# kaegi/adaptive-sph

Hardware: AMD Instinct MI355X
Metric: particle-steps/sec (whole node), 2D dam-break N=1M DFSPH; 1/2/4/8 GPUs (higher is better)
Workload: dtype f32; 1 GPU; dam_break_1m: 2D dam-break, 1024x1024 = 1 048 576 uniform-h particles, HybridDFSPH; particles=1048576, solver=HybridDFSPH, parallelism=single GPU

## Files before the change

adaptive_sph_amd/csrc/sph_api.hip:

```cpp
#include <hip/hip_runtime.h>

#include <algorithm>
#include <chrono>
#include <cmath>
#include <cstdarg>
#include <cstdio>
#include <cstdlib>
#include <cstring>
#include <string>
#include <vector>

#include "sph_context.hpp"
#include "sph_lambda.hpp"

int Profiler::find(const char* name)
{
    for (size_t i = 0; i < recs.size(); i++)
        if (recs[i].name == name) return (int)i;
    recs.push_back(Rec{name, 0, 0, {}});
    return (int)recs.size() - 1;
}
bool Profiler::wants(const char* name) const
{
    return mode == 1 || mode == 3 || mode == 4 || (mode == 2 && (step_index & 7u) == 0u && strncmp(name, "density", 7) == 0);
// ... 43 lines not shown
}
void Profiler::end(hipStream_t s)
{
    if (--depth > 0) return;
    if (ext_open) {
        if (ext_slot >= 0) pending.push_back(Pending{cur, nullptr, nullptr, ext_slot});
        ext_open = false;
        cur = -1;
        return;
    }
    if (kev_open) {
        kev_open = false;
        if (kev_taken) pending.push_back(Pending{cur, cur_a, cur_b, -1});
        else pool.push_back(cur_a);
        cur = -1;
        return;
    }
    hipEvent_t b = get_event();
    (void)hipEventRecord(b, s);
    pending.push_back(Pending{cur, cur_a, b, -1});
    cur = -1;
}
void Profiler::collect()
{
    std::vector<unsigned long long> ts;
    if (ts_next) {
        ts.resize(2 * (size_t)ts_next);
        (void)hipMemcpy(ts.data(), ts_dev, (size_t)ts_next * sizeof(unsigned long long), hipMemcpyDeviceToHost);
        (void)hipMemcpy(ts.data() + ts_next, ts_dev + TS_RING, (size_t)ts_next * sizeof(unsigned long long), hipMemcpyDeviceToHost);
        (void)hipMemset(ts_dev, 0xff, (size_t)ts_next * sizeof(unsigned long long));
        (void)hipMemset(ts_dev + TS_RING, 0, (size_t)ts_next * sizeof(unsigned long long));
    }
    static FILE* dump = getenv("SPH_TS_DUMP") ? fopen(getenv("SPH_TS_DUMP"), "w") : nullptr;
    std::vector<Pending> later;
    for (auto& p : pending) {
        if (p.slot >= 0) {
            const unsigned long long t0 = ts[(size_t)p.slot], t1 = ts[(size_t)ts_next + (size_t)p.slot];
            if (dump) fprintf(dump, "%s %llu %llu\n", recs[p.rec].name.c_str(), t0, t1);
            if (t1 >= t0 && t0 != ~0ull) {
                const float ms = (float)((double)(t1 - t0) * 1e-5);
                recs[p.rec].launches++;
                recs[p.rec].total_ms += ms;
                recs[p.rec].samples.push_back(ms);
            }
            continue;
        }
        float ms = 0.f;
        const hipError_t e = hipEventElapsedTime(&ms, p.a, p.b);
        if (e == hipErrorNotReady) {
            later.push_back(p);
            continue;
        }
        if (e == hipSuccess) {
            recs[p.rec].launches++;
            recs[p.rec].total_ms += ms;
            recs[p.rec].samples.push_back(ms);
        }
        pool.push_back(p.a);
        pool.push_back(p.b);
    }
    pending.swap(later);
    ts_next = 0;
    if (dump) fflush(dump);
}
void Profiler::reset()
{
    collect();
    recs.clear();
}
Profiler::~Profiler()
{
    for (auto& p : pending) {
        if (p.a) (void)hipEventDestroy(p.a);
        if (p.b) (void)hipEventDestroy(p.b);
    }
    for (auto e : pool) (void)hipEventDestroy(e);
    if (ts_dev) (void)hipFree(ts_dev);
}

#define HDR_BLOCKS 256

__global__ __launch_bounds__(256) void k_header(float4* __restrict__ pm, const float2* __restrict__ vel, uint32_t n, float rest_density,
                                                 int from_mass, float* __restrict__ h2_next, HeaderOut* __restrict__ partials,
                                                 const uint8_t* __restrict__ owned)
{
    const float INF = __uint_as_float(0x7f800000u);
    float mnx = INF, mny = INF, mxx = -INF, mxy = -INF, hmx = 0.f, hmn = INF, cfl = INF;
    for (uint32_t i = blockIdx.x * 256 + threadIdx.x; i < n; i += gridDim.x * 256) {
        if (owned && !owned[i]) continue;
        float4 p = pm[i];
        if (from_mass == 1) {
            p.w = h_from_mass(p.z, rest_density);
            pm[i] = p;
        } else if (from_mass == 2) {
            const float t = p.w;
            p.w = h2_next[i];
            h2_next[i] = t;
            pm[i] = p;
        }
        float2 v = vel[i];
        mnx = fminf(mnx, p.x); mxx = fmaxf(mxx, p.x);
        mny = fminf(mny, p.y); mxy = fmaxf(mxy, p.y);
        hmx = fmaxf(hmx, p.w); hmn = fminf(hmn, p.w);
        float sr = p.w * 2.f;
        float c = sr * sr / ((v.x * v.x + v.y * v.y) + 0.01f);
        cfl = c < cfl ? c : cfl;
    }
    mnx = wave_min(mnx); mny = wave_min(mny); mxx = wave_max(mxx); mxy = wave_max(mxy);
    hmx = wave_max(hmx); hmn = wave_min(hmn); cfl = wave_min(cfl);
    __shared__ HeaderOut s[4];
    const int lane = threadIdx.x & 63, w = threadIdx.x >> 6;
    if (lane == 0) s[w] = HeaderOut{mnx, mny, mxx, mxy, hmx, hmn, cfl, 0};
    __syncthreads();
    if (threadIdx.x == 0) {
        HeaderOut o = s[0];
        for (int k = 1; k < 4; k++) {
            o.min_x = fminf(o.min_x, s[k].min_x); o.min_y = fminf(o.min_y, s[k].min_y);
            o.max_x = fmaxf(o.max_x, s[k].max_x); o.max_y = fmaxf(o.max_y, s[k].max_y);
            o.h_max = fmaxf(o.h_max, s[k].h_max); o.h_min = fminf(o.h_min, s[k].h_min);
            o.min_cfl = fminf(o.min_cfl, s[k].min_cfl);
        }
        partials[blockIdx.x] = o;
    }
}

__global__ __launch_bounds__(256) void k_header_final(const HeaderOut* __restrict__ partials, int nparts, HeaderOut* __restrict__ out, uint32_t seq)
{
    const float INF = __uint_as_float(0x7f800000u);
    HeaderOut o{INF, INF, -INF, -INF, 0.f, INF, INF, 0};
    if ((int)threadIdx.x < nparts) o = partials[threadIdx.x];
    o.min_x = wave_min(o.min_x); o.min_y = wave_min(o.min_y); o.max_x = wave_max(o.max_x); o.max_y = wave_max(o.max_y);
    o.h_max = wave_max(o.h_max); o.h_min = wave_min(o.h_min); o.min_cfl = wave_min(o.min_cfl);
    __shared__ HeaderOut s[4];
    const int lane = threadIdx.x & 63, w = threadIdx.x >> 6;
    if (lane == 0) s[w] = o;
    __syncthreads();
    if (threadIdx.x == 0) {
        HeaderOut r = s[0];
        for (int k = 1; k < 4; k++) {
            r.min_x = fminf(r.min_x, s[k].min_x); r.min_y = fminf(r.min_y, s[k].min_y);
            r.max_x = fmaxf(r.max_x, s[k].max_x); r.max_y = fmaxf(r.max_y, s[k].max_y);
            r.h_max = fmaxf(r.h_max, s[k].h_max); r.h_min = fminf(r.h_min, s[k].h_min);
            r.min_cfl = fminf(r.min_cfl, s[k].min_cfl);
        }
        r.pad = seq - 1u;
        *out = r;
        if (seq) {
            __threadfence_system();
            ((volatile HeaderOut*)out)->pad = seq;
        }
    }
}

__global__ __launch_bounds__(1024) void k_header_ahead(const HeaderOut* __restrict__ partials, uint32_t nparts, const SolverCtrl* __restrict__ ctrl,
                                                       HeaderOut* __restrict__ out, const DeviceStatus* __restrict__ status, SolverCtrl* __restrict__ h_ctrl,
                                                       DeviceStatus* __restrict__ h_status, uint32_t seq)
{
    if (ctrl->done == 0u) {
        if (h_ctrl && threadIdx.x == 0) {
            SolverCtrl v = *ctrl;
            v.seq = seq - 1u;
            *h_ctrl = v;
            *h_status = *status;
            __threadfence_system();
            ((volatile SolverCtrl*)h_ctrl)->seq = seq;
        }
        return;
    }
    const float INF = __uint_as_float(0x7f800000u);
    HeaderOut o{INF, INF, -INF, -INF, 0.f, INF, INF, 0};
    for (uint32_t k0 = threadIdx.x; k0 < nparts; k0 += 4096u) {
        HeaderOut q[4];
#pragma unroll
        for (uint32_t u = 0; u < 4u; u++) q[u] = partials[min(k0 + 1024u * u, nparts - 1u)];
#pragma unroll
        for (uint32_t u = 0; u < 4u; u++) {
            o.min_x = fminf(o.min_x, q[u].min_x); o.min_y = fminf(o.min_y, q[u].min_y);
            o.max_x = fmaxf(o.max_x, q[u].max_x); o.max_y = fmaxf(o.max_y, q[u].max_y);
            o.h_max = fmaxf(o.h_max, q[u].h_max); o.h_min = fminf(o.h_min, q[u].h_min);
            o.min_cfl = fminf(o.min_cfl, q[u].min_cfl);
        }
    }
    o.min_x = wave_min(o.min_x); o.min_y = wave_min(o.min_y); o.max_x = wave_max(o.max_x); o.max_y = wave_max(o.max_y);
    o.h_max = wave_max(o.h_max); o.h_min = wave_min(o.h_min); o.min_cfl = wave_min(o.min_cfl);
    __shared__ HeaderOut s[16];
    const int lane = threadIdx.x & 63, w = threadIdx.x >> 6;
    if (lane == 0) s[w] = o;
    __syncthreads();
    if (threadIdx.x == 0) {
        HeaderOut r = s[0];
        for (int k = 1; k < 16; k++) {
            r.min_x = fminf(r.min_x, s[k].min_x); r.min_y = fminf(r.min_y, s[k].min_y);
            r.max_x = fmaxf(r.max_x, s[k].max_x); r.max_y = fmaxf(r.max_y, s[k].max_y);
            r.h_max = fmaxf(r.h_max, s[k].h_max); r.h_min = fminf(r.h_min, s[k].h_min);
            r.min_cfl = fminf(r.min_cfl, s[k].min_cfl);
        }
        *out = r;
        if (h_ctrl) {
            SolverCtrl v = *ctrl;
            v.seq = seq - 1u;
            *h_ctrl = v;
            *h_status = *status;
            __threadfence_system();
            ((volatile SolverCtrl*)h_ctrl)->seq = seq;
        }
    }
}

__global__ __launch_bounds__(256) void k_pack_upload(uint32_t n, const float* __restrict__ mass, const float2* __restrict__ pos,
                                                      const float2* __restrict__ velin, float4* __restrict__ pm, float2* __restrict__ vel,
                                                      uint32_t* __restrict__ orig, float* __restrict__ lvl, float* __restrict__ lvlold,
                                                      float* __restrict__ h2_next)
{
    uint32_t i = blockIdx.x * 256 + threadIdx.x;
    if (i >= n) return;
    float2 p = pos[i];
    pm[i] = make_float4(p.x, p.y, mass[i], 0.f);
    h2_next[i] = h_from_mass(mass[i], 1.f);
    vel[i] = velin[i];
    orig[i] = i;
    lvl[i] = __uint_as_float(0x7fc00000u);
    lvlold[i] = 0.f;
}

__global__ void k_publish(const SolverCtrl* __restrict__ ctrl, const DeviceStatus* __restrict__ status, SolverCtrl* __restrict__ h_ctrl,
                          DeviceStatus* __restrict__ h_status, uint32_t seq)
{
    if (threadIdx.x == 0 && blockIdx.x == 0) {
        SolverCtrl v = *ctrl;
        v.seq = seq - 1u;
        *h_ctrl = v;
        *h_status = *status;
        __threadfence_system();
        ((volatile SolverCtrl*)h_ctrl)->seq = seq;
    }
}

enum { G_F32 = 0, G_F32X2 = 1, G_PM_X = 2, G_PM_M = 3, G_PM_H = 4, G_U32 = 5, G_H2NEXT = 6, G_U8 = 7, G_F32X4_ZW = 8 };

__global__ __launch_bounds__(256) void k_to_host_order(uint32_t n, int kind, const uint32_t* __restrict__ orig, const void* __restrict__ src,
                                                        void* __restrict__ dst)
{
    uint32_t i = blockIdx.x * 256 + threadIdx.x;
    if (i >= n) return;
    uint32_t o = orig ? orig[i] : i;
    switch (kind) {
    case G_F32: ((float*)dst)[o] = ((const float*)src)[i]; break;
    case G_U32: ((uint32_t*)dst)[o] = ((const uint32_t*)src)[i]; break;
    case G_U8: ((uint8_t*)dst)[o] = ((const uint8_t*)src)[i]; break;
    case G_F32X2: ((float2*)dst)[o] = ((const float2*)src)[i]; break;
    case G_PM_X: { float4 p = ((const float4*)src)[i]; ((float2*)dst)[o] = make_float2(p.x, p.y); } break;
    case G_F32X4_ZW: { float4 p = ((const float4*)src)[i]; ((float2*)dst)[o] = make_float2(p.z, p.w); } break;
    case G_PM_M: ((float*)dst)[o] = ((const float4*)src)[i].z; break;
    case G_PM_H: ((float*)dst)[o] = ((const float4*)src)[i].w; break;
    case G_H2NEXT: ((float*)dst)[o] = h_from_mass(((const float4*)src)[i].z, 1.f); break;
    }
}

__global__ __launch_bounds__(256) void k_from_host_order(uint32_t n, int kind, const uint32_t* __restrict__ orig, const void* __restrict__ src,
                                                          void* __restrict__ dst)
{
    uint32_t i = blockIdx.x * 256 + threadIdx.x;
    if (i >= n) return;
    uint32_t o = orig ? orig[i] : i;
    switch (kind) {
    case G_F32: ((float*)dst)[i] = ((const float*)src)[o]; break;
    case G_U32: ((uint32_t*)dst)[i] = ((const uint32_t*)src)[o]; break;
    case G_F32X2: ((float2*)dst)[i] = ((const float2*)src)[o]; break;
    case G_U8: ((uint8_t*)dst)[i] = ((const uint8_t*)src)[o]; break;
    case G_PM_X: { float2 p = ((const float2*)src)[o]; float4 q = ((float4*)dst)[i]; q.x = p.x; q.y = p.y; ((float4*)dst)[i] = q; } break;
    case G_PM_M: { float4 q = ((float4*)dst)[i]; q.z = ((const float*)src)[o]; ((float4*)dst)[i] = q; } break;
    case G_PM_H: { float4 q = ((float4*)dst)[i]; q.w = ((const float*)src)[o]; ((float4*)dst)[i] = q; } break;
    default: break;
    }
}

__global__ __launch_bounds__(256) void k_rows_to_slots(uint32_t n, int kind, const uint32_t* __restrict__ slot, const void* __restrict__ src, void* __restrict__ dst)
{
    const uint32_t r = blockIdx.x * 256 + threadIdx.x;
    if (r >= n) return;
    const uint32_t i = slot[r];
    switch (kind) {
    case G_F32: ((float*)dst)[i] = ((const float*)src)[r]; break;
    case G_U32: ((uint32_t*)dst)[i] = ((const uint32_t*)src)[r]; break;
    case G_F32X2: ((float2*)dst)[i] = ((const float2*)src)[r]; break;
    case G_U8: ((uint8_t*)dst)[i] = ((const uint8_t*)src)[r]; break;
    case G_PM_X: { float2 p = ((const float2*)src)[r]; float4 q = ((float4*)dst)[i]; q.x = p.x; q.y = p.y; ((float4*)dst)[i] = q; } break;
    case G_PM_M: { float4 q = ((float4*)dst)[i]; q.z = ((const float*)src)[r]; ((float4*)dst)[i] = q; } break;
    case G_PM_H: { float4 q = ((float4*)dst)[i]; q.w = ((const float*)src)[r]; ((float4*)dst)[i] = q; } break;
    default: break;
    }
}

__global__ __launch_bounds__(256) void k_cell_index_host(uint32_t n, GridP g, const uint32_t* __restrict__ orig, const float4* __restrict__ pm,
                                                          uint32_t* __restrict__ dst)
{
    uint32_t i = blockIdx.x * 256 + threadIdx.x;
    if (i >= n) return;
    float4 p = pm[i];
    int cx = (int)floorf(p.x / g.cs) - g.minx, cy = (int)floorf(p.y / g.cs) - g.miny;
    dst[orig[i]] = (uint32_t)cx + (uint32_t)cy * (uint32_t)g.sx;
}

__global__ __launch_bounds__(256) void k_ext_counts(uint32_t n, const uint4* __restrict__ nl_ext, const uint32_t* __restrict__ orig, uint32_t* __restrict__ dst)
{
    uint32_t i = blockIdx.x * 256 + threadIdx.x;
    if (i < n) dst[orig[i]] = nl_ext[i].w & 0xffffu;
}

__global__ __launch_bounds__(256) void k_fill_neighbors(uint32_t n, GridP g, TileP t, const uint32_t* __restrict__ cell_start,
                                                         const uint32_t* __restrict__ cxy, const uint32_t* __restrict__ orig,
                                                         const float4* __restrict__ pm, const uint32_t* __restrict__ offsets_host,
                                                         uint32_t* __restrict__ indices, float k, const uint32_t* __restrict__ rowmap)
{
    uint32_t i = blockIdx.x * 256 + threadIdx.x;
    if (i >= n) return;
    const uint32_t row = rowmap ? rowmap[i] : orig[i];
    if (row == 0xffffffffu) return;
    const float4 Ai = pm[i];
    const uint32_t c = cxy[i];
    const int cx = c & 0xffffu, cy = c >> 16;
    uint32_t w = offsets_host[row];
    const int R = stencil_radius(g, t, Ai.w, cx, cy, k);
    for (int dy = -R; dy <= R; dy++) {
        int yy = cy + dy;
        if (yy < 0 || yy >= g.sy) continue;
        uint32_t b = cell_start[(uint32_t)yy * g.sx + max(cx - R, 0)];
        uint32_t e = cell_start[(uint32_t)yy * g.sx + min(cx + R + 1, g.sx)];
        for (uint32_t j = b; j < e; j++) {
            const float4 Aj = pm[j];
            const float dx = Ai.x - Aj.x, dyy = Ai.y - Aj.y;
            const float r2 = dx * dx + dyy * dyy;
            const float s = ((Ai.w + Aj.w) * 0.5f) * k;
            if (r2 < s * s) indices[w++] = orig[j];
        }
    }
}

__global__ __launch_bounds__(256) void k_check_neighborhood(uint32_t n, const float4* __restrict__ pm, const uint32_t* __restrict__ ncount,
                                                             const uint32_t* __restrict__ orig, DeviceStatus* status, const uint8_t* __restrict__ owned)
{
    uint32_t i = blockIdx.x * 256 + threadIdx.x;
    if (i >= n) return;
    if (owned && !owned[i]) return;
    const float4 Ai = pm[i];
    uint32_t cnt = 0;
    for (uint32_t j = 0; j < n; j++) {
        const float4 Aj = pm[j];
        const float dx = Ai.x - Aj.x, dy = Ai.y - Aj.y;
        const float s = ((Ai.w + Aj.w) * 0.5f) * 2.f;
        cnt += (dx * dx + dy * dy < s * s) ? 1u : 0u;
    }
    if (cnt != ncount[i] && atomicCAS(&status->error, 0u, (uint32_t)SPH_ERR_CHECK_NEIGHBORHOOD) == 0u) status->info = orig[i];
}

static int alloc_particle_buffers(sph_ctx* c)
{
    const size_t n = c->cap ? c->cap : 1;
    for (int k = 0; k < 2; k++) {
        HIPCHK(c, c->pm[k].ensure(n * sizeof(float4)));
        HIPCHK(c, c->vel[k].ensure(n * sizeof(float2)));
        HIPCHK(c, c->orig[k].ensure(n * sizeof(uint32_t)));
        HIPCHK(c, c->lvl[k].ensure(n * sizeof(float)));
        HIPCHK(c, c->lvlold[k].ensure(n * sizeof(float)));
        HIPCHK(c, c->h2n[k].ensure(n * sizeof(float)));
        HIPCHK(c, c->szc[k].ensure(n));
        HIPCHK(c, c->key[k].ensure(n * sizeof(uint32_t)));
        HIPCHK(c, c->val[k].ensure(n * sizeof(uint32_t)));
    }
    HIPCHK(c, c->vel_tmp.ensure(n * sizeof(float2)));
    HIPCHK(c, c->sort_scratch.ensure(radix_sort_scratch_elems((uint32_t)n) * sizeof(uint32_t)));
    HIPCHK(c, c->cxy.ensure(n * sizeof(uint32_t)));
    DevBuf* f1[] = {&c->rho, &c->lam_sum, &c->constf, &c->aii, &c->src, &c->p0, &c->p1, &c->dens_err, &c->stat, &c->ncount,
                    &c->mrho, &c->pt0, &c->pt1};
    for (auto b : f1) HIPCHK(c, b->ensure(n * sizeof(float)));
    HIPCHK(c, c->lam_grad.ensure(n * sizeof(float2)));
    if (c->exact) {
        HIPCHK(c, c->wall_pl.ensure(n * sizeof(float2) * SPH_MAX_PLANES));
        HIPCHK(c, c->wall_cnt.ensure(n));
    }
    HIPCHK(c, c->lam_prev.ensure(n * sizeof(float)));
    HIPCHK(c, c->omega.ensure(n * sizeof(float)));
    HIPCHK(c, c->pacc.ensure(n * sizeof(float4)));
    HIPCHK(c, c->prec0.ensure(n * sizeof(float4)));
    HIPCHK(c, c->prec1.ensure(n * sizeof(float4)));
    HIPCHK(c, c->xv.ensure(n * sizeof(float4)));
    HIPCHK(c, c->scratch.ensure(n * sizeof(float4)));
    HIPCHK(c, c->nl.ensure(sweep_list_bytes((uint32_t)n)));
    HIPCHK(c, c->nl_ok.ensure(n));
    HIPCHK(c, c->red_partials.ensure(sizeof(SolverPartial) * (size_t)solver_reduce_blocks((uint32_t)n)));
    HIPCHK(c, c->hdr_ahead_partials.ensure(sizeof(HeaderOut) * (((size_t)n + 255) / 256)));
    return SPH_OK;
}

Options options_from_env()
{
    Options o;
    auto num = [](const char* name, int dflt) {
        const char* e = getenv(name);
        return e && e[0] ? atoi(e) : dflt;
    };
    auto flag = [](const char* name) { return getenv(name) != nullptr ? 1 : 0; };
    o.exact = num("SPH_HIP_EXACT", 0) == 1 ? 1 : 0;
    o.overlap = num("SPH_OVERLAP", -1);
    o.loopback_sync = num("SPH_LOOPBACK_SYNC", 0) != 0 ? 1 : 0;
    o.force_slab_mode = flag("SPH_FORCE_SLAB_MODE");
    o.event_wait = flag("SPH_EVENT_WAIT");
    o.debug_sync = num("SPH_DEBUG_SYNC", 0);
    o.debug_counts = flag("SPH_DEBUG_COUNTS");
    o.comm_delay_us = num("SPH_DEBUG_COMM_DELAY_US", 0);
    o.hip_trace = num("SPH_HIP_TRACE", 0) == 1 ? 1 : 0;
#ifdef SPH_LAB
    o.paced = num("SPH_PACED", 1) != 0 ? 1 : 0;
    o.pace_lead = num("SPH_PACE_LEAD", 0);
    o.pace_pred = num("SPH_PACE_PRED", 0xffff);
    o.chain = num("SPH_CHAIN", -1);
    o.accel_generic = flag("SPH_ACCEL_GENERIC");
    o.jacobi_generic = flag("SPH_JACOBI_GENERIC");
    o.source_generic = flag("SPH_SOURCE_GENERIC");
    o.slab_general = flag("SPH_SLAB_GENERAL");
    o.slab_level_plain = flag("SPH_SLAB_LEVEL_PLAIN");
    o.level_serial = flag("SPH_LEVEL_SERIAL");
    o.level_batch8 = flag("SPH_LEVEL_BATCH8");
    o.level_queue = num("SPH_LEVEL_QUEUE", 1) != 0 ? 1 : 0;
    o.offset_lists = num("SPH_OFFSET_LISTS", 1) != 0 ? 1 : 0;
    o.no_fuse = flag("SPH_NO_FUSE");
    o.side_stream_normal = flag("SPH_SIDE_STREAM_NORMAL");
    o.tile = num("SPH_TILE", 0);
    o.ahead_build = num("SPH_AHEAD_BUILD", 1) != 0 ? 1 : 0;
    o.inc_sort = num("SPH_INC_SORT", 1);
    o.slab_paced = num("SPH_SLAB_PACED", 1) != 0 ? 1 : 0;
    o.slab_records = num("SPH_SLAB_RECORDS", 1) != 0 ? 1 : 0;
    o.side_cus = num("SPH_SIDE_CUS", 0);
    o.main_exclude = num("SPH_MAIN_EXCLUDE", 0) != 0 ? 1 : 0;
    o.ipc_fuse_max_bytes = std::max(num("SPH_IPC_FUSE_MAX_BYTES", 64 << 10), 0);
    o.ipc_copy_min_bytes = std::max(num("SPH_IPC_COPY_MIN_BYTES", 256 << 10), 0);
    o.search_block = std::min(std::max(num("SPH_SEARCH_BLOCK", 1024) / 64 * 64, 64), 1024);
#else
    static const char* const lab_only[] = {"SPH_PACED", "SPH_PACE_LEAD", "SPH_PACE_PRED", "SPH_CHAIN", "SPH_ACCEL_GENERIC", "SPH_JACOBI_GENERIC", "SPH_SOURCE_GENERIC",
                                           "SPH_SLAB_GENERAL", "SPH_SLAB_LEVEL_PLAIN", "SPH_LEVEL_SERIAL", "SPH_LEVEL_BATCH8", "SPH_LEVEL_QUEUE", "SPH_OFFSET_LISTS",
                                           "SPH_NO_FUSE", "SPH_SIDE_STREAM_NORMAL", "SPH_TILE", "SPH_AHEAD_BUILD", "SPH_INC_SORT", "SPH_SLAB_PACED", "SPH_SLAB_RECORDS",
                                           "SPH_SIDE_CUS", "SPH_MAIN_EXCLUDE", "SPH_IPC_FUSE_MAX_BYTES", "SPH_IPC_COPY_MIN_BYTES"};
    static bool warned = false;
    if (!warned)
        for (const char* name : lab_only)
            if (getenv(name)) {
                fprintf(stderr, "libsph_hip: %s is a laboratory switch and is IGNORED by the product library (use SPH_HIP_LIBRARY=libsph_lab.so, scripts/README.md)\n", name);
                warned = true;
            }
#endif
    return o;
}

extern "C" int sph_create(uint64_t n_capacity, int device_id, const sph_plane* planes, int n_planes, sph_ctx** out)
{
    if (!out || n_planes < 0 || n_planes > SPH_MAX_PLANES || (n_planes > 0 && !planes)) return SPH_ERR_INVALID_ARGUMENT;
    if (n_capacity >= (1ull << 31)) return SPH_ERR_CAPACITY;
    int ndev = 0;
    if (hipGetDeviceCount(&ndev) != hipSuccess || ndev <= 0 || device_id < 0 || device_id >= ndev) return SPH_ERR_DEVICE;
    if (hipSetDevice(device_id) != hipSuccess) return SPH_ERR_DEVICE;
    sph_ctx* c = new sph_ctx();
    c->device = device_id;
    c->cap = n_capacity;
    c->n_planes = n_planes;
    for (int k = 0; k < n_planes; k++) c->bnd_h.planes[k] = PlaneP{planes[k].dir_x, planes[k].dir_y, planes[k].delta};
    c->opt = options_from_env();
    c->exact = c->opt.exact;
    auto bail = [&](int code) {
        sph_destroy(c);
        return code;
    };
    uint32_t side_mask[8] = {0, 0, 0, 0, 0, 0, 0, 0}, main_mask[8];
    for (int b = 0; b < 8 * c->opt.side_cus && b < 256; b++) side_mask[b >> 5] |= 1u << (b & 31);
    for (int w = 0; w < 8; w++) main_mask[w] = ~side_mask[w];
    if (c->opt.side_cus > 0 && c->opt.main_exclude) {
        if (hipExtStreamCreateWithCUMask(&c->stream, 8, main_mask) != hipSuccess) return bail(SPH_ERR_DEVICE);
    } else if (hipStreamCreateWithFlags(&c->stream, hipStreamNonBlocking) != hipSuccess) return bail(SPH_ERR_DEVICE);
    if (c->opt.side_cus > 0) {
        if (hipExtStreamCreateWithCUMask(&c->stream2, 8, side_mask) != hipSuccess) return bail(SPH_ERR_DEVICE);
    } else
    {
        int lo = 0, hi = 0;
        (void)hipDeviceGetStreamPriorityRange(&lo, &hi);
        if (c->opt.side_stream_normal || hipStreamCreateWithPriority(&c->stream2, hipStreamNonBlocking, hi) != hipSuccess)
            if (hipStreamCreateWithFlags(&c->stream2, hipStreamNonBlocking) != hipSuccess) return bail(SPH_ERR_DEVICE);
    }
    if (hipEventCreateWithFlags(&c->ev_fork, hipEventDisableTiming) != hipSuccess) return bail(SPH_ERR_DEVICE);
    for (auto& e : c->ev)
        if (hipEventCreate(&e) != hipSuccess) return bail(SPH_ERR_DEVICE);
    if (alloc_particle_buffers(c) != SPH_OK) return bail(SPH_ERR_DEVICE);
    bool ok = c->planes_d.ensure(sizeof(BoundaryP)) == hipSuccess && c->lam_lut.ensure(10001 * 4) == hipSuccess &&
              c->dlam_lut.ensure(10001 * 4) == hipSuccess && c->hdr_partials.ensure(sizeof(HeaderOut) * HDR_BLOCKS) == hipSuccess &&
              c->hdr_out.ensure(sizeof(HeaderOut)) == hipSuccess && c->ctrl.ensure(3 * sizeof(SolverCtrl)) == hipSuccess &&
              c->status.ensure(sizeof(DeviceStatus)) == hipSuccess && c->n_tiles.ensure(16) == hipSuccess;
    if (!ok) return bail(SPH_ERR_DEVICE);
    if (hipHostMalloc((void**)&c->hdr_host, sizeof(HeaderOut), hipHostMallocMapped) != hipSuccess) return bail(SPH_ERR_DEVICE);
    if (hipHostMalloc((void**)&c->ctrl_host, 3 * sizeof(SolverCtrl), hipHostMallocMapped) != hipSuccess) return bail(SPH_ERR_DEVICE);
    if (hipHostMalloc((void**)&c->status_host, sizeof(DeviceStatus), hipHostMallocMapped) != hipSuccess) return bail(SPH_ERR_DEVICE);
    if (hipHostMalloc((void**)&c->lvl_changed, 64 * sizeof(uint32_t), hipHostMallocMapped) != hipSuccess) return bail(SPH_ERR_DEVICE);
    if (hipHostGetDevicePointer((void**)&c->lvl_changed_dev, c->lvl_changed, 0) != hipSuccess) return bail(SPH_ERR_DEVICE);
    memset(c->lvl_changed, 0, 64 * sizeof(uint32_t));
    if (hipHostGetDevicePointer((void**)&c->hdr_host_dev, c->hdr_host, 0) != hipSuccess) return bail(SPH_ERR_DEVICE);
    if (hipHostGetDevicePointer((void**)&c->ctrl_host_dev, c->ctrl_host, 0) != hipSuccess) return bail(SPH_ERR_DEVICE);
    if (hipHostGetDevicePointer((void**)&c->status_host_dev, c->status_host, 0) != hipSuccess) return bail(SPH_ERR_DEVICE);
    if (hipEventCreateWithFlags(&c->ev_sync, hipEventDisableTiming) != hipSuccess) return bail(SPH_ERR_DEVICE);
    memset(c->status_host, 0, sizeof(DeviceStatus));
    memset((void*)c->ctrl_host, 0, 3 * sizeof(SolverCtrl));
    c->prog_host = (volatile uint32_t*)(c->ctrl_host + 2);
    c->prog_host_dev = (uint32_t*)(c->ctrl_host_dev + 2);
    c->movers_host = c->prog_host + 1;
    std::vector<float> lam, dlam;
    sph_lambda::build_luts(lam, dlam);
    if (hipMemcpy(c->lam_lut.p, lam.data(), lam.size() * 4, hipMemcpyHostToDevice) != hipSuccess ||
        hipMemcpy(c->dlam_lut.p, dlam.data(), dlam.size() * 4, hipMemcpyHostToDevice) != hipSuccess ||
        hipMemcpy(c->planes_d.p, &c->bnd_h, sizeof(BoundaryP), hipMemcpyHostToDevice) != hipSuccess ||
        hipMemset(c->status.p, 0, sizeof(DeviceStatus)) != hipSuccess || hipMemset(c->ctrl.p, 0, sizeof(SolverCtrl)) != hipSuccess ||
        hipDeviceSynchronize() != hipSuccess)
        return bail(SPH_ERR_DEVICE);
    *out = c;
    return SPH_OK;
}

extern "C" int sph_set_boundary_polygon(sph_ctx* c, const float* pts, int n)
{
    if (!c || !pts || n < 3 || n > SPH_MAX_POLYGON_POINTS) return SPH_ERR_INVALID_ARGUMENT;
    HIPCHK(c, hipSetDevice(c->device));
    BoundaryP b = c->bnd_h;
    for (int i = 0; i < n; i++) {
        b.px[i] = pts[2 * i];
        b.py[i] = pts[2 * i + 1];
    }
    for (int i = 0; i < n; i++) {
        const int i1 = (i + 1) % n;
        const float dx = b.px[i1] - b.px[i], dy = b.py[i1] - b.py[i];
        const float n2 = dx * dx + dy * dy;
        if (!(n2 > 0.00001f)) return c->fail(SPH_ERR_INVALID_ARGUMENT, "assertion failed: line_dir.norm_squared() > 0.00001");
        const float nn = sqrtf(n2);
        b.dx[i] = dx / nn;
        b.dy[i] = dy / nn;
    }
    for (int i = 0; i < n; i++) {
        const int pi = i == 0 ? n - 1 : i - 1;
        const float px = -b.dy[pi] + -b.dy[i], py = b.dx[pi] + b.dx[i];
        if (!(px * px + py * py > 0.00001f)) return c->fail(SPH_ERR_INVALID_ARGUMENT, "assertion failed: pseudo_normal.norm_squared() > 0.00001");
        b.nx[i] = px;
        b.ny[i] = py;
    }
    b.poly_n = n;
    c->bnd_h = b;
    c->n_planes = 1;
    HIPCHK(c, hipStreamSynchronize(c->stream));
    HIPCHK(c, hipMemcpy(c->planes_d.p, &c->bnd_h, sizeof(BoundaryP), hipMemcpyHostToDevice));
    return SPH_OK;
}

extern "C" void sph_destroy(sph_ctx* c)
{
    if (!c) return;
    (void)hipSetDevice(c->device);
    if (c->stream) (void)hipStreamSynchronize(c->stream);
    if (c->stream2) (void)hipStreamSynchronize(c->stream2);
    dist_release(c);
    DevBuf* all[] = {&c->pm[0], &c->pm[1], &c->vel[0], &c->vel[1], &c->orig[0], &c->orig[1], &c->lvl[0], &c->lvl[1], &c->lvlold[0],
                     &c->lvlold[1], &c->vel_tmp, &c->key[0], &c->key[1], &c->val[0], &c->val[1], &c->sort_scratch, &c->cxy, &c->cell_start,
                     &c->cs_scratch, &c->hdr_ahead_partials, &c->h2n[0], &c->h2n[1], &c->lam_prev, &c->nl, &c->nlx, &c->tile_raw, &c->tile_h, &c->tile_h_ext, &c->lvl_changed_d, &c->lvl_tmp, &c->lvl_nrm, &c->lvl_state, &c->lvl_when, &c->lvl_mark, &c->lvl_queue, &c->nloff, &c->nlh, &c->flag_surface,
                     &c->flag_insufficient, &c->con_thr, &c->con_consumed, &c->con_h, &c->flag_reduced, &c->szc[0], &c->szc[1], &c->omega, &c->stash, &c->nl_ext, &c->nlx_ext, &c->nl_ok, &c->mrho, &c->pt0, &c->pt1, &c->prec0, &c->prec1, &c->xv, &c->rho, &c->lam_sum, &c->lam_grad, &c->wall_pl, &c->wall_cnt, &c->constf, &c->aii, &c->src, &c->p0, &c->p1, &c->pacc, &c->dens_err,
                     &c->stat, &c->ncount, &c->planes_d, &c->lam_lut, &c->dlam_lut, &c->hdr_partials, &c->hdr_out, &c->ctrl, &c->status,
                     &c->n_tiles, &c->red_partials, &c->scratch, &c->split_patterns, &c->akey[0], &c->akey[1], &c->aval[0], &c->aval[1], &c->acxy, &c->acell_start, &c->pm2,
                     &c->atile_raw, &c->atile_h, &c->inc_head, &c->inc_next, &c->inc_bsum, &c->inc_movers, &c->cand_red, &c->rnd_rec, &c->rnd_keys, &c->rnd_out, &c->rnd_max, &c->rnd_prev, &c->rnd_layer, &c->rnd_band, &c->rnd_words, &c->rnd_stage};
    for (auto b : all) b->release();
    for (DevBuf* b : c->export_bufs()) b->release();
    for (DevBuf* b : c->prob_bufs()) b->release();
    for (DevBuf* b : c->slab_bufs()) b->release();
    if (c->hdr_host) (void)hipHostFree(c->hdr_host);
    if (c->ctrl_host) (void)hipHostFree(c->ctrl_host);
    if (c->status_host) (void)hipHostFree(c->status_host);
    if (c->lvl_changed) (void)hipHostFree(c->lvl_changed);
    for (auto& e : c->ev)
        if (e) (void)hipEventDestroy(e);
    if (c->ev_sync) (void)hipEventDestroy(c->ev_sync);
    if (c->stream) (void)hipStreamDestroy(c->stream);
    if (c->stream2) (void)hipStreamDestroy(c->stream2);
    if (c->ev_fork) (void)hipEventDestroy(c->ev_fork);
    delete c;
}

extern "C" const char* sph_last_error(const sph_ctx* c) { return c ? c->err.c_str() : "null context"; }
extern "C" uint64_t sph_num_particles(const sph_ctx* c) { return c ? c->n : 0; }
extern "C" float sph_time(const sph_ctx* c) { return c ? c->time : 0.f; }
extern "C" int sph_set_time(sph_ctx* c, float t, uint64_t step)
{
    if (!c) return SPH_ERR_INVALID_ARGUMENT;
    c->time = t;
    c->step_number = step;
    return SPH_OK;
}

extern "C" int sph_set_math_policy(sph_ctx* c, int policy)
{
    if (!c || (policy != SPH_MATH_FAST && policy != SPH_MATH_EXACT)) return SPH_ERR_INVALID_ARGUMENT;
    if (c->poisoned) return c->fail(SPH_ERR_POISONED, "sph_set_math_policy: the context is poisoned until sph_upload");
    if (policy == c->exact) return SPH_OK;
    HIPCHK(c, hipSetDevice(c->device));
    if (int rc = wait_stream(c)) return rc;
    c->exact = policy;
    if (c->exact) {
        size_t n = c->cap ? c->cap : 1;
        HIPCHK(c, c->wall_pl.ensure(n * sizeof(float2) * SPH_MAX_PLANES));
        HIPCHK(c, c->wall_cnt.ensure(n));
    }
    c->drop(DROPS_POLICY);
    return SPH_OK;
}
extern "C" int sph_get_math_policy(const sph_ctx* c) { return c ? c->exact : -1; }

extern "C" int sph_upload(sph_ctx* c, uint64_t n, const float* mass, const float* pos, const float* vel)
{
    if (!c || (n && (!mass || !pos || !vel))) return SPH_ERR_INVALID_ARGUMENT;
    if (n > c->cap) return c->fail(SPH_ERR_CAPACITY, "n=%llu exceeds capacity %llu", (unsigned long long)n, (unsigned long long)c->cap);
    HIPCHK(c, hipSetDevice(c->device));
    hipStream_t s = c->stream;
    c->n = n;
    c->cur = 0;
    c->pcur = 0;
    c->poisoned = false;
    c->dist.n_tot = (uint32_t)n;
    c->drop(DROPS_UPLOAD);
    for (DevBuf* b : c->export_bufs()) b->release();
    for (DevBuf* b : c->slab_bufs()) b->release();
    for (DevBuf* b : c->prob_bufs()) b->release();
    if (n == 0) return SPH_OK;
    HIPCHK(c, hipMemcpyAsync(c->key[1].p, mass, n * sizeof(float), hipMemcpyHostToDevice, s));
    HIPCHK(c, hipMemcpyAsync(c->scratch.p, pos, n * sizeof(float2), hipMemcpyHostToDevice, s));
    HIPCHK(c, hipMemcpyAsync(c->vel_tmp.p, vel, n * sizeof(float2), hipMemcpyHostToDevice, s));
    hipLaunchKernelGGL(k_pack_upload, dim3((n + 255) / 256), dim3(256), 0, s, (uint32_t)n, c->key[1].as<float>(), c->scratch.as<float2>(),
                       c->vel_tmp.as<float2>(), c->pm[0].as<float4>(), c->vel[0].as<float2>(), c->orig[0].as<uint32_t>(),
                       c->lvl[0].as<float>(), c->lvlold[0].as<float>(), c->h2n[0].as<float>());
    HIPCHK(c, hipMemsetAsync(c->szc[0].p, 2, n, s));
    DevBuf* zero[] = {&c->rho, &c->lam_sum, &c->constf, &c->aii, &c->src, &c->p0, &c->p1, &c->dens_err, &c->ncount};
    for (auto b : zero) HIPCHK(c, hipMemsetAsync(b->p, 0, n * sizeof(float), s));
    HIPCHK(c, hipMemsetAsync(c->lam_grad.p, 0, n * sizeof(float2), s));
    HIPCHK(c, hipMemsetAsync(c->pacc.p, 0, n * sizeof(float4), s));
    c->pressure_cur = 0;
    HIPCHK(c, hipStreamSynchronize(s));
    return SPH_OK;
}

struct FieldRef {
    int kind;
    const void* src;
    size_t elem;
    bool uploadable;
};

static bool field_ref(sph_ctx* c, int field, FieldRef* r)
{
    const int k = c->cur;
    switch (field) {
    case SPH_F_MASS: *r = {G_PM_M, c->pm[c->pcur].p, 4, true}; return true;
    case SPH_F_POSITION: *r = {G_PM_X, c->pm[c->pcur].p, 8, true}; return true;
    case SPH_F_VELOCITY: *r = {G_F32X2, c->vel[k].p, 8, true}; return true;
    case SPH_F_PRESSURE_ACCEL: *r = {G_F32X4_ZW, c->pacc.p, 8, false}; return true;
    case SPH_F_DENSITY: *r = {G_F32, c->rho.p, 4, false}; return true;
    case SPH_F_PPE_SOURCE_TERM: *r = {G_F32, c->src.p, 4, false}; return true;
    case SPH_F_PRESSURE: *r = {G_F32, c->pressure_cur ? c->p1.p : c->p0.p, 4, false}; return true;
    case SPH_F_AII: *r = {G_F32, c->aii.p, 4, false}; return true;
    case SPH_F_DENSITY_ERROR: *r = {G_F32, c->dens_err.p, 4, false}; return true;
    case SPH_F_H2: *r = {G_PM_H, c->pm[c->pcur].p, 4, true}; return true;
    case SPH_F_H2_NEXT: *r = {G_F32, c->h2n[k].p, 4, true}; return true;
    case SPH_F_CONSTANT_FIELD: *r = {G_F32, c->constf.p, 4, false}; return true;
    case SPH_F_NEIGHBOR_COUNT: *r = {G_U32, c->ncount.p, 4, false}; return true;
    case SPH_F_LEVEL_ESTIMATION: *r = {G_F32, c->lvl[k].p, 4, true}; return true;
    case SPH_F_LEVEL_OLD: *r = {G_F32, c->lvlold[k].p, 4, true}; return true;
    case SPH_F_PARTICLE_SIZE_CLASS: *r = {G_U8, c->szc[k].p, 1, true}; return true;
    case SPH_F_LAMBDA_SUM: *r = {G_F32, c->lam_sum.p, 4, false}; return true;
    case SPH_F_LAMBDA_GRAD_SUM: *r = {G_F32X2, c->lam_grad.p, 8, false}; return true;
    default: return false;
    }
}

static int download_slab(sph_ctx* c, int kind, const void* src, size_t elem, void* dst, uint64_t bytes)
{
    hipStream_t s = c->stream;
    const uint32_t nt = c->have_flags ? c->dist.n_tot : (uint32_t)c->n;
    if (bytes != (uint64_t)c->n * elem) return c->fail(SPH_ERR_INVALID_ARGUMENT, "size mismatch (slab holds %llu particles)", (unsigned long long)c->n);
    if (nt == 0) return SPH_OK;
    std::vector<uint8_t> raw((size_t)nt * elem), flags(nt, 1);
    hipLaunchKernelGGL(k_to_host_order, dim3((nt + 255) / 256), dim3(256), 0, s, nt, kind, (const uint32_t*)nullptr, src, c->scratch.p);
    HIPCHK(c, hipMemcpyAsync(raw.data(), c->scratch.p, raw.size(), hipMemcpyDeviceToHost, s));
    if (c->have_flags) HIPCHK(c, hipMemcpyAsync(flags.data(), c->dist.owned.p, nt, hipMemcpyDeviceToHost, s));
    HIPCHK(c, hipStreamSynchronize(s));
    size_t w = 0;
    for (uint32_t i = 0; i < nt; i++)
        if (flags[i]) {
            if (w >= c->n) return c->fail(SPH_ERR_DEVICE, "owned-particle count mismatch");
            memcpy((uint8_t*)dst + w * elem, raw.data() + (size_t)i * elem, elem);
            w++;
        }
    return SPH_OK;
}

extern "C" int sph_download(sph_ctx* c, int field, void* dst, uint64_t bytes)
{
    if (!c || !dst) return SPH_ERR_INVALID_ARGUMENT;
    HIPCHK(c, hipSetDevice(c->device));
    hipStream_t s = c->stream;
    const uint32_t n = (uint32_t)c->n;
    const int k = c->cur;
    if (field == SPH_F_PARTICLE_ID) {
        if (c->dist.on) return download_slab(c, G_U32, c->orig[k].p, 4, dst, bytes);
        if (bytes != (uint64_t)n * 4) return c->fail(SPH_ERR_INVALID_ARGUMENT, "field %d: size mismatch", field);
        for (uint32_t i = 0; i < n; i++) ((uint32_t*)dst)[i] = i;
        return SPH_OK;
    }
    if (field == SPH_F_CELL_INDEX) {
        if (!c->grid_valid) return c->fail(SPH_ERR_INVALID_ARGUMENT, "no grid yet: run a step first");
        if (c->dist.on) return download_slab(c, G_U32, c->key[0].p, 4, dst, bytes);
        if (bytes != (uint64_t)n * 4) return c->fail(SPH_ERR_INVALID_ARGUMENT, "field %d: size mismatch", field);
        if (n == 0) return SPH_OK;
        const bool same_grid = c->fgrid.minx == c->grid.minx && c->fgrid.miny == c->grid.miny && c->fgrid.sx == c->grid.sx && c->fgrid.sy == c->grid.sy;
        if (c->uniform_h && same_grid) {
            hipLaunchKernelGGL(k_to_host_order, dim3((n + 255) / 256), dim3(256), 0, s, n, (int)G_U32, c->orig[k].as<uint32_t>(),
// ... 597 lines not shown
    if (!ext)
        hipLaunchKernelGGL(k_fill_neighbors, dim3((n + 255) / 256), dim3(256), 0, s, n, c->fgrid,
                           TileP{c->tile_ts, c->tile_tsx, c->tile_tsy, c->tile_h.as<uint32_t>(), 0.f}, c->cell_start.as<uint32_t>(), c->cxy.as<uint32_t>(),
                           c->orig[c->cur].as<uint32_t>(), c->pm[c->pcur ^ 1].as<float4>(), d_off.as<uint32_t>(), d_idx.as<uint32_t>(), 2.f, (const uint32_t*)nullptr);
    else
        hipLaunchKernelGGL(k_fill_neighbors, dim3((n + 255) / 256), dim3(256), 0, s, n, c->fgrid,
                           TileP{c->tile_ts, c->tile_tsx, c->tile_tsy, c->tile_h_ext.as<uint32_t>(), c->lists_after_slack}, c->cell_start.as<uint32_t>(),
                           c->cxy.as<uint32_t>(), c->orig[c->cur].as<uint32_t>(), c->pm[c->pcur].as<float4>(), d_off.as<uint32_t>(), d_idx.as<uint32_t>(),
                           c->lists_after_k, (const uint32_t*)nullptr);
    HIPCHK(c, hipMemcpyAsync(indices, d_idx.p, (size_t)tot * 4, hipMemcpyDeviceToHost, s));
    HIPCHK(c, hipStreamSynchronize(s));
    c->export_built();
    c->export_tot = tot;
    return SPH_OK;
}

int export_lists_on_device(sph_ctx* c)
{
    const uint32_t n = (uint32_t)c->n;
    hipStream_t s = c->stream;
    DevBuf &d_off = c->export_d_off, &d_idx = c->export_d_idx;
    c->drop(CARRY_EXPORT);
    HIPCHK(c, d_off.ensure(((size_t)n + 1) * 4));
    HIPCHK(c, c->scratch.ensure((size_t)n * 4 + 4));
    HIPCHK(c, c->cand_scan.ensure(((size_t)n / 2048 + 4) * 4));
    const bool ext = c->lists_after;
    const dim3 grid((n + 255) / 256), blk(256);
    if (n) {
        if (!ext) hipLaunchKernelGGL(k_to_host_order, grid, blk, 0, s, n, (int)G_U32, c->orig[c->cur].as<uint32_t>(), (const void*)c->ncount.p, c->scratch.p);
        else hipLaunchKernelGGL(k_ext_counts, grid, blk, 0, s, n, c->nl_ext.as<uint4>(), c->orig[c->cur].as<uint32_t>(), c->scratch.as<uint32_t>());
    }
    device_exclusive_scan_u32(s, c->scratch.as<uint32_t>(), d_off.as<uint32_t>(), n, c->cand_scan.as<uint32_t>(), d_off.as<uint32_t>() + n);
    uint32_t tot = 0;
    HIPCHK(c, hipMemcpyAsync(&tot, d_off.as<uint32_t>() + n, 4, hipMemcpyDeviceToHost, s));
    HIPCHK(c, hipStreamSynchronize(s));
    HIPCHK(c, d_idx.ensure((size_t)tot * 4));
    if (n && tot) {
        if (!ext)
            hipLaunchKernelGGL(k_fill_neighbors, grid, blk, 0, s, n, c->fgrid, TileP{c->tile_ts, c->tile_tsx, c->tile_tsy, c->tile_h.as<uint32_t>(), 0.f},
                               c->cell_start.as<uint32_t>(), c->cxy.as<uint32_t>(), c->orig[c->cur].as<uint32_t>(), c->pm[c->pcur ^ 1].as<float4>(),
                               d_off.as<uint32_t>(), d_idx.as<uint32_t>(), 2.f, (const uint32_t*)nullptr);
        else
            hipLaunchKernelGGL(k_fill_neighbors, grid, blk, 0, s, n, c->fgrid,
                               TileP{c->tile_ts, c->tile_tsx, c->tile_tsy, c->tile_h_ext.as<uint32_t>(), c->lists_after_slack}, c->cell_start.as<uint32_t>(),
                               c->cxy.as<uint32_t>(), c->orig[c->cur].as<uint32_t>(), c->pm[c->pcur].as<float4>(), d_off.as<uint32_t>(), d_idx.as<uint32_t>(),
                               c->lists_after_k, (const uint32_t*)nullptr);
    }
    c->export_built();
    c->export_tot = tot;
    return SPH_OK;
}

__global__ __launch_bounds__(256) void k_slab_owned_flags(uint32_t nt, const uint8_t* __restrict__ owned, uint32_t* __restrict__ flag, uint32_t* __restrict__ iota)
{
    const uint32_t s = blockIdx.x * 256 + threadIdx.x;
    if (s >= nt) return;
    flag[s] = owned[s] ? 1u : 0u;
    iota[s] = s;
}
__global__ __launch_bounds__(256) void k_slab_rowmap(uint32_t nt, uint32_t n_rows, const uint8_t* __restrict__ owned, uint32_t* __restrict__ pos,
                                                      const uint32_t* __restrict__ ncount, const uint4* __restrict__ nl_ext, uint32_t* __restrict__ row_slot,
                                                      uint32_t* __restrict__ cnt, unsigned long long* __restrict__ total64)
{
    const uint32_t s = blockIdx.x * 256 + threadIdx.x;
    unsigned long long c = 0;
    if (s < nt) {
        const uint32_t r = pos[s];
        if (!owned[s] || r >= n_rows) pos[s] = 0xffffffffu;
        else {
            row_slot[r] = s;
            c = nl_ext ? (nl_ext[s].w & 0xffffu) : ncount[s];
            cnt[r] = (uint32_t)c;
        }
    }
    for (int o = 32; o > 0; o >>= 1) c += __shfl_down(c, o, 64);
    if ((threadIdx.x & 63) == 0 && c) atomicAdd(total64, c);
}
int slab_lists_on_device(sph_ctx* c)
{
    const uint32_t n = (uint32_t)c->n, nt = c->dist.n_tot;
    hipStream_t s = c->stream;
    c->drop(CARRY_SLAB_LISTS);
    TmpBuf d_iota, d_cnt, d_tot64;
    HIPCHK(c, d_tot64.ensure(8));
    HIPCHK(c, hipMemsetAsync(d_tot64.p, 0, 8, s));
    DevBuf& d_map = c->slab_slot_row;
    HIPCHK(c, d_map.ensure((size_t)nt * 4 + 4));
    HIPCHK(c, d_iota.ensure((size_t)nt * 4 + 4));
    HIPCHK(c, d_cnt.ensure((size_t)n * 4 + 4));
    HIPCHK(c, c->slab_row_slot.ensure((size_t)n * 4 + 4));
    HIPCHK(c, c->slab_off.ensure(((size_t)n + 1) * 4));
    HIPCHK(c, c->scratch.ensure((size_t)nt * 4 + 4));
    HIPCHK(c, c->cand_scan.ensure(((size_t)nt / 2048 + 4) * 4));
    const bool ext = c->lists_after;
    uint32_t* off = c->slab_off.as<uint32_t>();
    uint32_t tot[2] = {0, 0};
    if (nt) {
        const dim3 grid((nt + 255) / 256), blk(256);
        hipLaunchKernelGGL(k_slab_owned_flags, grid, blk, 0, s, nt, c->dist.owned.as<uint8_t>(), c->scratch.as<uint32_t>(), d_iota.as<uint32_t>());
        device_exclusive_scan_u32(s, c->scratch.as<uint32_t>(), d_map.as<uint32_t>(), nt, c->cand_scan.as<uint32_t>(), d_map.as<uint32_t>() + nt);
        HIPCHK(c, hipMemcpyAsync(&tot[0], d_map.as<uint32_t>() + nt, 4, hipMemcpyDeviceToHost, s));
        hipLaunchKernelGGL(k_slab_rowmap, grid, blk, 0, s, nt, n, c->dist.owned.as<uint8_t>(), d_map.as<uint32_t>(), c->ncount.as<uint32_t>(),
                           ext ? c->nl_ext.as<uint4>() : (const uint4*)nullptr, c->slab_row_slot.as<uint32_t>(), d_cnt.as<uint32_t>(), d_tot64.as<unsigned long long>());
    }
    unsigned long long tot64 = 0;
    HIPCHK(c, hipMemcpyAsync(&tot64, d_tot64.p, 8, hipMemcpyDeviceToHost, s));
    device_exclusive_scan_u32(s, d_cnt.as<uint32_t>(), off, n, c->cand_scan.as<uint32_t>(), off + n);
    HIPCHK(c, hipMemcpyAsync(&tot[1], off + n, 4, hipMemcpyDeviceToHost, s));
    HIPCHK(c, hipStreamSynchronize(s));
    if (tot[0] != n) return c->fail(SPH_ERR_DEVICE, "owned-particle count mismatch");
    if (tot64 >= (1ull << 32) || tot64 != tot[1])
        return c->fail(SPH_ERR_CAPACITY, "%llu neighbour-list entries on rank %d do not fit the 32-bit CSR offsets", tot64, c->dist.rank);
    HIPCHK(c, c->slab_idx.ensure((size_t)tot[1] * 4 + 4));
    if (nt && tot[1]) {
        const dim3 grid((nt + 255) / 256), blk(256);
        if (!ext)
            hipLaunchKernelGGL(k_fill_neighbors, grid, blk, 0, s, nt, c->fgrid, TileP{c->tile_ts, c->tile_tsx, c->tile_tsy, c->tile_h.as<uint32_t>(), 0.f},
                               c->cell_start.as<uint32_t>(), c->cxy.as<uint32_t>(), (const uint32_t*)d_iota.as<uint32_t>(), c->pm[c->pcur ^ 1].as<float4>(), off,
                               c->slab_idx.as<uint32_t>(), 2.f, (const uint32_t*)d_map.as<uint32_t>());
        else
            hipLaunchKernelGGL(k_fill_neighbors, grid, blk, 0, s, nt, c->fgrid,
                               TileP{c->tile_ts, c->tile_tsx, c->tile_tsy, c->tile_h_ext.as<uint32_t>(), c->lists_after_slack}, c->cell_start.as<uint32_t>(),
                               c->cxy.as<uint32_t>(), (const uint32_t*)d_iota.as<uint32_t>(), c->pm[c->pcur].as<float4>(), off, c->slab_idx.as<uint32_t>(),
                               c->lists_after_k, (const uint32_t*)d_map.as<uint32_t>());
        HIPCHK(c, hipStreamSynchronize(s));
    }
    c->slab_lists_valid = true;
    c->slab_lists_rows = n;
    c->slab_lists_tot = tot[1];
    return SPH_OK;
}


void launch_header(sph_ctx* c, uint32_t n, float rest_density, int from_mass , HeaderOut* out_dev,
                   const uint8_t* owned)
{
    hipStream_t s = c->stream;
    ProfScope ps(&c->prof, "header", s);
    int nb = (int)((n + 255) / 256);
    if (nb > HDR_BLOCKS) nb = HDR_BLOCKS;
    if (nb < 1) nb = 1;
    hipLaunchKernelGGL(k_header, dim3(nb), dim3(256), 0, s, c->pm[c->pcur].as<float4>(), c->vel[c->cur].as<float2>(), n, rest_density, from_mass,
                       c->h2n[c->cur].as<float>(), c->hdr_partials.as<HeaderOut>(), owned);
    c->publish_seq++;
    if (c->publish_seq == 0u) c->publish_seq = 1u;
    const bool mapped = out_dev == c->hdr_host_dev;
    hipLaunchKernelGGL(k_header_final, dim3(1), dim3(256), 0, s, c->hdr_partials.as<HeaderOut>(), nb, out_dev, mapped ? c->publish_seq : 0u);
    if (mapped) {
        c->hint_word = &((volatile HeaderOut*)c->hdr_host)->pad;
        c->hint_seq = c->publish_seq;
    }
}

void launch_header_ahead(sph_ctx* c, uint32_t nblocks, HeaderOut* out_dev, bool publish)
{
    ProfScope ps(&c->prof, "header_ahead", c->stream);
    uint32_t seq = 0;
    if (publish) {
        c->publish_seq++;
        if (c->publish_seq == 0u) c->publish_seq = 1u;
        seq = c->publish_seq;
        c->publish_folded = true;
    }
    hipLaunchKernelGGL(k_header_ahead, dim3(1), dim3(1024), 0, c->stream, c->hdr_ahead_partials.as<HeaderOut>(), nblocks, c->ctrl.as<SolverCtrl>(), out_dev,
                       c->status.as<DeviceStatus>(), publish ? c->ctrl_host_dev : (SolverCtrl*)nullptr, publish ? c->status_host_dev : (DeviceStatus*)nullptr, seq);
}

void launch_publish(sph_ctx* c)
{
    if (c->publish_folded) {
        c->publish_folded = false;
        return;
    }
    c->publish_seq++;
    if (c->publish_seq == 0u) c->publish_seq = 1u;
    hipLaunchKernelGGL(k_publish, dim3(1), dim3(64), 0, c->stream, c->ctrl.as<SolverCtrl>(), c->status.as<DeviceStatus>(), c->ctrl_host_dev,
                       c->status_host_dev, c->publish_seq);
}

void launch_check_neighborhood(sph_ctx* c, const SweepArgs& a)
{
    ProfScope ps(&c->prof, "check_neighborhood", c->stream);
    hipLaunchKernelGGL(k_check_neighborhood, dim3((a.n + 255) / 256), dim3(256), 0, c->stream, a.n, a.pm, a.ncount, a.orig, a.status, a.owned);
}
```

adaptive_sph_amd/csrc/sph_context.hpp:

```cpp
#pragma once

#include <hip/hip_runtime.h>

#include <array>
#include <chrono>
#include <cstdarg>
#include <cstdio>
#include <string>
#include <vector>

#include "sph_carry.hpp"
#include "sph_internal.hpp"

struct DevBuf {
    void* p = nullptr;
    size_t bytes = 0;
    hipError_t ensure(size_t need)
    {
        if (need <= bytes) return hipSuccess;
        if (p) (void)hipFree(p);
        p = nullptr;
        bytes = 0;
        size_t grow = need + need / 4 + 256;
        hipError_t e = hipMalloc(&p, grow);
        if (e == hipSuccess) bytes = grow;
        return e;
    }
    void release()
    {
        if (p) (void)hipFree(p);
        p = nullptr;
        bytes = 0;
    }
    template <class T>
    T* as() const { return (T*)p; }
};

struct TmpBuf : DevBuf {
    TmpBuf() = default;
    TmpBuf(const TmpBuf&) = delete;
    TmpBuf& operator=(const TmpBuf&) = delete;
    ~TmpBuf() { release(); }
};

struct Options {
    int exact = 0;
    int paced = 1;
    int pace_lead = 0;
    int pace_pred = 0xffff;
    int chain = -1;
    int overlap = -1;
    int accel_generic = 0;
    int jacobi_generic = 0;
    int source_generic = 0;
    int slab_general = 0;
    int slab_level_plain = 0;
    int level_serial = 0;
    int level_batch8 = 0;
    int offset_lists = 1;
    int level_queue = 1;
    int no_fuse = 0;
    int event_wait = 0;
    int loopback_sync = 0;
    int side_stream_normal = 0;
    int force_slab_mode = 0;
    int tile = 0;
    int ahead_build = 1;
    int inc_sort = 1;
    int slab_paced = 1;
    int slab_records = 1;
    int debug_sync = 0;
    int debug_counts = 0;
    int comm_delay_us = 0;
    int hip_trace = 0;
    int side_cus = 0;
    int main_exclude = 0;
    int ipc_fuse_max_bytes = 64 << 10;
    int ipc_copy_min_bytes = 256 << 10;
    int search_block = 1024;
};
Options options_from_env();

struct sph_ctx : Carry {
    int device = 0;
    Options opt;
    uint64_t cap = 0, n = 0;
    hipStream_t stream = nullptr;
    hipStream_t stream2 = nullptr;
    hipEvent_t ev_fork = nullptr;
    uint32_t level_seq = 0;
    int n_planes = 0;
    BoundaryP bnd_h{};
    float time = 0.f;
    uint64_t step_number = 0;
    uint64_t n_waits = 0;
    bool poisoned = false;
    std::string err;
    Profiler prof;
    int exact = 0;
    std::vector<uint32_t> export_cnt, export_off;
    DevBuf export_d_off, export_d_idx;

    uint64_t export_tot = 0;
    DevBuf cand_rec, cand_cls, cand_cnt, cand_off, cand_idx, cand_scan, cand_red;
    std::array<DevBuf*, 8> export_bufs() { return {&export_d_off, &export_d_idx, &cand_rec, &cand_cls, &cand_cnt, &cand_off, &cand_idx, &cand_scan}; }
    int prob_kind = 0;
    uint32_t prob_k = 0;
    DevBuf prob_flag, prob_rank, prob_lvl, prob_ids, prob_cls, prob_mass, prob_level, prob_pos, prob_h2, prob_off, prob_idx;
    uint64_t prob_serial = 0, sol_serial = 0;
    DevBuf sol_partner, sol_counter, ps_w, ps_words, ps_state, ps_rec;
    std::array<DevBuf*, 17> prob_bufs() { return {&prob_flag, &prob_rank, &prob_lvl, &prob_ids, &prob_cls, &prob_mass, &prob_level, &prob_pos, &prob_h2, &prob_off, &prob_idx,
                                                  &sol_partner, &sol_counter, &ps_w, &ps_words, &ps_state, &ps_rec}; }
    uint32_t slab_lists_rows = 0, slab_rows_n = 0;
    uint64_t slab_lists_tot = 0, slab_rows_tot = 0;
    DevBuf slab_row_slot, slab_slot_row, slab_off, slab_idx;
    uint32_t slab_prob_k = 0, slab_prob_ko = 0;
    DevBuf slab_prob_flag, slab_prob_rank, slab_prob_ids, slab_prob_cls, slab_prob_mass, slab_prob_level, slab_prob_pos, slab_prob_h2, slab_prob_off;
    std::array<DevBuf*, 13> slab_bufs() { return {&slab_row_slot, &slab_slot_row, &slab_off, &slab_idx, &slab_prob_flag, &slab_prob_rank, &slab_prob_ids, &slab_prob_cls,
                                                  &slab_prob_mass, &slab_prob_level, &slab_prob_pos, &slab_prob_h2, &slab_prob_off}; }

    DevBuf pm[2], vel[2], orig[2], lvl[2], lvlold[2];
    int cur = 0;
    int pcur = 0;
    DevBuf vel_tmp;
    DevBuf key[2], val[2], sort_scratch, cxy, cell_start, cs_scratch, nl, nl_ok, mrho, pt0, pt1, prec0, prec1, xv;
    bool uniform_h = false;
    float h_uniform = 0.f;
    DevBuf wall_pl, wall_cnt;
    DevBuf rho, lam_sum, lam_grad, constf, aii, src, p0, p1, pacc, dens_err, stat, ncount;
    DevBuf planes_d, lam_lut, dlam_lut, hdr_partials, hdr_out, ctrl, status, n_tiles, red_partials, scratch;
    HeaderOut* hdr_host = nullptr;
    volatile uint32_t* hint_word = nullptr;
    uint32_t hint_seq = 0;
    uint32_t publish_seq = 0;
    bool publish_folded = false;
    SolverCtrl* ctrl_host = nullptr;
    DeviceStatus* status_host = nullptr;
    HeaderOut* hdr_host_dev = nullptr;
    SolverCtrl* ctrl_host_dev = nullptr;
    DeviceStatus* status_host_dev = nullptr;
    volatile uint32_t* prog_host = nullptr;
    uint32_t* prog_host_dev = nullptr;
    uint32_t solve_epoch = 0;
    bool paced_step = false;
    hipEvent_t ev_sync = nullptr;

    struct Dist {
        bool on = false;
        int rank = 0, nranks = 1;
        float cut_lo = 0.f, cut_hi = 0.f;
        uint32_t n_tot = 0;
        uint32_t n_halo[2] = {0, 0}, n_ghost[2] = {0, 0};
        float hcut[2] = {0.f, 0.f};
        float halo_w[2] = {0.f, 0.f};
        DevBuf owned;
        DevBuf cls, blk;
        int overlap_env = -1;
        bool pre = false;
        uint32_t pre_n = 0;
        uint32_t pre_cls_n = 0;
        uint32_t pre_own = 0;
        DevBuf tot_table;
        DevBuf ring1, ring1_src;
        DevBuf halo_idx, halo_pos, halo_src, ghost_dst;
        DevBuf send[2], recv[2];
        DevBuf counts;
        DevBuf solver_tot;
        uint32_t* counts_host = nullptr;
        uint32_t* counts_host_dev = nullptr;
        void* nccl = nullptr;
        DevBuf edge;
        hipStream_t xstream = nullptr;
        hipEvent_t ev_x[3] = {nullptr, nullptr, nullptr};
        hipEvent_t ev_pack = nullptr, ev_copied = nullptr, ev_tot = nullptr;
        double* gtot = nullptr;
        uint32_t gtot_seq = 0;
        bool ghosts_ok = true;
        void* tgroup = nullptr;
        void* ipc = nullptr;
        void* shm = nullptr;
        size_t shm_bytes = 0;
        std::string shm_name;
        int rebalance_every = 0;
        DevBuf hist;
        uint32_t rebalances = 0;
        uint64_t stat_exchanges = 0, stat_bytes_sent = 0, stat_bytes_recv = 0, stat_allreduces = 0, stat_step0 = 0;
    } dist;

    GridP grid{};
    GridP fgrid{};
    int tile_ts = 0, tile_tsx = 0, tile_tsy = 0;
    DevBuf tile_raw, tile_h, tile_h_ext, nlx;
    DevBuf nloff, nlh;
    DevBuf akey[2], aval[2], acxy, acell_start, pm2;
    DevBuf atile_raw, atile_h;
    DevBuf inc_head, inc_next, inc_bsum, inc_movers;
    uint32_t inc_epoch = 0;
    int inc_radix_streak = 0;
    struct Ahead {
        GridP g{};
        float h_max = 0.f, h_min = 0.f, rest_density = 0.f;
        int tile_ts = 0, tile_tsx = 0, tile_tsy = 0;
        uint64_t n = 0;
    } ahead;
    DevBuf hdr_ahead_partials;
    float hdr_ahead_rest_density = 0.f;
    DevBuf h2n[2];
    DevBuf lam_prev;
    DevBuf lvl_queue;
    DevBuf lvl_tmp, lvl_nrm, lvl_state, lvl_when, lvl_mark, flag_surface, flag_insufficient, stash, nl_ext, nlx_ext;
    DevBuf con_thr, con_consumed, con_h, flag_reduced;
    float lists_after_k = 0.f, lists_after_slack = 0.f;
    float h_max_step = 0.f;
    float last_dmax = 0.f;
    float slab_slack_w = 0.f;
    DevBuf szc[2];
    DevBuf omega;
    DevBuf split_patterns;
    uint32_t n_split_patterns = 0;
    DevBuf lvl_changed_d;
    uint32_t* lvl_changed = nullptr;
    uint32_t last_level_sweeps = 0;
    uint32_t* lvl_changed_dev = nullptr;
    uint32_t pressure_cur = 0;
    uint32_t last_div_iters = 2, last_dens_iters = 2;
    uint32_t prev_dens_iters = 0;
    uint32_t prev_div_iters = 0;
    DevBuf rnd_rec, rnd_keys, rnd_out, rnd_max, rnd_prev;
    uint64_t rnd_prev_n = 0;
    DevBuf rnd_layer, rnd_band, rnd_words, rnd_stage;
    bool rnd_have_layer = false;
    int rnd_layer_sx0 = 0, rnd_layer_sx1 = 0, rnd_layer_hs = 0;
    hipEvent_t ev[8];

    int fail(int code, const char* fmt, ...)
    {
        char buf[512];
        va_list ap;
        va_start(ap, fmt);
        vsnprintf(buf, sizeof buf, fmt, ap);
        va_end(ap);
        err = buf;
        return code;
    }
    int refuse_poisoned() { return fail(SPH_ERR_POISONED, "an earlier step failed inside the step: the particle state is undefined until sph_upload"); }
};

#define HIPCHK(ctx, call)                                                                                  \
    do {                                                                                                   \
        hipError_t e_ = (call);                                                                            \
        if (e_ != hipSuccess) return (ctx)->fail(SPH_ERR_DEVICE, "%s failed: %s", #call, hipGetErrorString(e_)); \
    } while (0)


int wait_stream(sph_ctx* c);
const char* status_message(uint32_t code);
SweepArgs make_args(sph_ctx* c, const StepP& sp);

void launch_header(sph_ctx* c, uint32_t n, float rest_density, int from_mass, HeaderOut* out_dev, const uint8_t* owned = nullptr);
void launch_publish(sph_ctx* c);
void launch_profile_calibration(sph_ctx* c);
void launch_check_neighborhood(sph_ctx* c, const SweepArgs& a);
int export_lists_on_device(sph_ctx* c);
int slab_lists_on_device(sph_ctx* c);
void dist_release(sph_ctx* c);
```

adaptive_sph_amd/csrc/sph_internal.hpp:

```cpp
#pragma once

#include <hip/hip_runtime.h>
#include <hip/hip_ext.h>
#include <stdint.h>

#include <string>
#include <vector>

#include "sph_device.h"
#include "sph_ffi.h"

struct Profiler {
    int mode = 0;
    uint64_t step_index = 0;
    struct Rec {
        std::string name;
        uint64_t launches = 0;
        double total_ms = 0;
        std::vector<float> samples;
    };
    struct Pending {
        int rec;
        hipEvent_t a, b;
        int slot;
    };
    std::vector<Rec> recs;
    std::vector<Pending> pending;
    std::vector<hipEvent_t> pool;

    int find(const char* name);
    bool wants(const char* name) const;
    hipEvent_t get_event();
    void begin(const char* name, hipStream_t s, bool single_launch = false);
    void end(hipStream_t s);
    unsigned long long* take_slot();
    bool take_events(hipEvent_t* a, hipEvent_t* b);
    enum { TS_RING = 1 << 16 };
    unsigned long long* ts_dev = nullptr;
    uint32_t ts_next = 0;
    void collect();
    void reset();
    ~Profiler();
    int cur = -1;
    int depth = 0;
    hipEvent_t cur_a = nullptr, cur_b = nullptr;
    bool ext_open = false;
    int ext_slot = -1;
    bool kev_open = false, kev_taken = false;
};

struct ProfScope {
    Profiler* p;
    hipStream_t s;
    bool on;
    ProfScope(Profiler* p_, const char* name, hipStream_t s_, bool single_launch = false)
        : p(p_), s(s_), on(p_ && p_->mode && p_->wants(name) && (p_->mode != 3 || single_launch))
    {
        if (on) p->begin(name, s, single_launch);
    }
    ~ProfScope()
    {
        if (on) p->end(s);
    }
};

struct HeaderOut {
    float min_x, min_y, max_x, max_y, h_max, h_min, min_cfl;
    uint32_t pad;
};

struct SolverCtrl {
    uint32_t done;
    uint32_t iters;
    uint32_t cur;
    uint32_t peer_error;
    uint32_t normal, singular, negative;
    float sum_err, max_err;
    uint32_t slot_done[2];
    uint32_t seq;
};

struct DeviceStatus {
    uint32_t error;
    uint32_t info;
};

struct CellKeyGen {
    const float4* pm;
    GridP g;
    const uint8_t* gone;
    uint32_t n_gone, gone_from;
    int clamp = 0;
};
int radix_sort_pairs(hipStream_t s, Profiler* prof, uint32_t* keyA, uint32_t* valA, uint32_t* keyB, uint32_t* valB,
                     uint32_t n, int bits, uint32_t* hist_scratch , const CellKeyGen* keygen = nullptr);
size_t radix_sort_scratch_elems(uint32_t n);
struct ReorderIO {
    const float4* pm_in;
    const float2* vel_in;
    const uint32_t* orig_in;
    const float *lvl_in, *lvlold_in;
    float4* pm_out;
    float2* vel_out;
    uint32_t* orig_out;
    float *lvl_out, *lvlold_out;
    uint32_t* cxy_out;
    const float* h2n_in;
    float* h2n_out;
    const float* lam_in;
    float* lam_prev_out;
    const uint8_t* szc_in;
    uint8_t* szc_out;
};
size_t incremental_sort_block_sums(uint32_t ncells);
void incremental_cell_sort_reorder(hipStream_t s, Profiler* prof, uint32_t n, const float4* pm_new, const IncClassifyP& q, bool classified,
                                   const uint32_t* cell_start_cur, uint32_t* key_out, uint32_t* cell_start_out, const ReorderIO& io, uint32_t* bsum, uint32_t* movers,
                                   uint32_t* movers_host);

void incremental_cell_sort_perm(hipStream_t s, Profiler* prof, uint32_t n, uint32_t n_prev, const CellKeyGen& kg, const IncClassifyP& q, const uint32_t* cell_start_cur,
                                uint32_t* key_out, uint32_t* perm_out, uint32_t* cell_start_out, uint32_t* bsum, uint32_t* movers, uint32_t* movers_host);

void launch_reorder(hipStream_t s, Profiler* prof, uint32_t n, GridP g, const uint32_t* sorted_key, const uint32_t* perm, const ReorderIO& io,
                    void* cell_start_scratch);
size_t cell_start_scratch_bytes();
void launch_cell_start(hipStream_t s, Profiler* prof, const uint32_t* sorted_key, uint32_t n, uint32_t ncells,
                       uint32_t* cell_start , void* scratch ,
                       bool count_zeroed = false );
void launch_tile_hmax(hipStream_t s, Profiler* prof, uint32_t n, const float4* pm, GridP g, int ts, int tsx, int tsy, uint32_t* raw,
                      uint32_t* out , uint32_t* out_ext = nullptr , int d_ext = 2);

struct SweepArgs {
    GridP g;
    StepP sp;
    uint32_t n;
    int exact;
    int uniform_h;
    float h_uniform;
    const uint32_t* cell_start;
    const uint32_t* orig;
    const float4* pm;
    float2* vel;
    float2* vel_tmp;
    float* rho;
    float* lam_sum;
    float2* lam_grad;
    float2* wall_pl = nullptr;
    uint8_t* wall_cnt = nullptr;
    float* constf;
    float* aii;
    float* src;
    float* p0;
    float* p1;
    float4* pacc;
    float* dens_err;
    float* stat;
    uint32_t* ncount;
    uint4* nl;
    uint4* nlx;
    HeaderOut* hdr_partials;
    IncClassifyP inc;
    int h_mode;
    int sp_check_aii;
    float* h2_next;
    float* omega;
    const uint8_t* size_class;
    const float* lam_prev;
    const uint2* nloff = nullptr;
    const uint8_t* nlh = nullptr;
    uint2* nloff_out = nullptr;
    uint8_t* nlh_out = nullptr;
    uint4* nl_ext;
    uint4* nlx_ext;
    TileP t;
    TileP t_ext;
    float* partials;
    const uint8_t* owned;
    const uint8_t* ring1;
    const uint8_t* edge = nullptr;
    const uint32_t* elist_a = nullptr;
    const uint32_t* elist_b = nullptr;
    uint32_t n_ea = 0, n_eb = 0;
    int part = 0;
    double* solver_tot;
    const double* tot_table = nullptr;
    int tot_nr = 0, tot_self = 0;
    float* mrho;
    float* pt0;
    float* pt1;
    float4* rec0 = nullptr;
    float4* rec1 = nullptr;
    float4* xv = nullptr;
    bool xv_ok = false;
    const BoundaryP* planes;
    const float* lam_lut;
    const float* dlam_lut;
    SolverCtrl* ctrl;
    const uint32_t* gate = nullptr;
    DeviceStatus* status;
    uint32_t* prog_host = nullptr;
    uint32_t prog_epoch = 0;
    int opt_tile = 0, opt_jacobi_generic = 0;
    Profiler* prof = nullptr;
};

bool sweep_a_on_records(const SweepArgs& a);
bool source_term_on_records(const SweepArgs& a);
size_t sweep_list_bytes(uint32_t n);
size_t sweep_index_list_bytes(uint32_t n);
size_t sweep_offset_list_bytes(uint32_t n);
bool sweeps_want_offset_lists(const SweepArgs& a);
bool sweep_forces_index_lists();
uint32_t solver_reduce_blocks(uint32_t n);
void launch_density(hipStream_t s, Profiler* prof, const SweepArgs& a);
void launch_density_replay(hipStream_t s, Profiler* prof, const SweepArgs& a);
void launch_constrain_init(hipStream_t s, Profiler* prof, const SweepArgs& a, uint32_t target, float* thr, uint32_t* consumed, float* h_new, uint8_t* flag);
void launch_constrain_pass(hipStream_t s, Profiler* prof, const SweepArgs& a, uint32_t target, float* thr, uint32_t* consumed, float* h_new, uint32_t* pending);
void launch_constrain_apply(hipStream_t s, Profiler* prof, const SweepArgs& a, float4* pm, const float* h_new, float* h2_next);
void launch_aii_const(hipStream_t s, Profiler* prof, const SweepArgs& a);
void launch_aii_const_non_pressure(hipStream_t s, Profiler* prof, const SweepArgs& a);
void launch_non_pressure(hipStream_t s, Profiler* prof, const SweepArgs& a);
void launch_source_term(hipStream_t s, Profiler* prof, const SweepArgs& a, int kind, int residual_density);
void launch_pressure_accel(hipStream_t s, Profiler* prof, const SweepArgs& a, int iter, int residual_density, float max_avg_error, uint32_t max_iters, int multi,
                           int part = 0);
void launch_solver_totals(hipStream_t s, Profiler* prof, const SweepArgs& a, int iter, int residual_density, float max_avg_error, uint32_t max_iters);
void launch_pack_and_totals(hipStream_t s, Profiler* prof, const SweepArgs& a, int iter, int residual_density, float max_avg_error, uint32_t max_iters,
                            const uint32_t* src_idx, uint32_t cnt0, uint32_t cnt1, int words, int stride, int off, const float* field, float* out0, float* out1);
void launch_ctrl_reset(hipStream_t s, SolverCtrl* ctrl, const uint32_t* gate);
void launch_solver_progress(hipStream_t s, Profiler* prof, const SweepArgs& a, int iter, int residual_density, float max_avg_error, uint32_t max_iters);
void launch_solver_handoff(hipStream_t s, Profiler* prof, SolverCtrl* ctrl, SolverCtrl* saved_host, uint32_t* gate);
void launch_solver_tail(hipStream_t s, Profiler* prof, const SweepArgs& a, int tail, float4* pm_out, int decide_iter = -1, int residual_density = 0,
                        float max_avg_error = 0.f, uint32_t max_iters = 0, SolverCtrl* handoff_host = nullptr, uint32_t* gate_out = nullptr);
void launch_jacobi_update(hipStream_t s, Profiler* prof, const SweepArgs& a, int iter, int residual_density, float max_avg_error, uint32_t max_iters, int multi);
void launch_solver_decide(hipStream_t s, Profiler* prof, const SweepArgs& a, int iter, int residual_density, float max_avg_error,
                          uint32_t max_iters);
struct LevelArgs {
    float k;
    float threshold;
    float max_surface_distance;
    int boundary_is_fluid_surface;
    float2* nrm;
    uint8_t* state;
    uint8_t* flag_surface;
    uint8_t* flag_insufficient;
    float maximum_range;
    uint8_t* size_class;
    float* level;
    uint32_t* when;
    uint32_t* mark;
    uint8_t* fmap = nullptr;
    uint32_t fmap_lg_s = 0;
    float* level_old;
    float* stash_first;
    int center_diff;
    int plain_propagate;
    const uint8_t* edge;
    int replay_step_lists;
    const float4* pm_cell;
};
void launch_max_disp(hipStream_t s, Profiler* prof, uint32_t n, const float4* pm_old, const float4* pm_new, uint32_t* out);
void launch_tile_redilate(hipStream_t s, Profiler* prof, int tsx, int tsy, int d, const uint32_t* raw, uint32_t* out);
void launch_level_detect(hipStream_t s, Profiler* prof, const SweepArgs& a, const LevelArgs& l);
void launch_level_propagate(hipStream_t s, Profiler* prof, const SweepArgs& a, const LevelArgs& l, uint32_t t, uint32_t* changed);
void launch_fill_stash(hipStream_t s, Profiler* prof, const SweepArgs& a, const LevelArgs& l, float* stash);
void launch_level_smooth(hipStream_t s, Profiler* prof, const SweepArgs& a, const LevelArgs& l, const float4* pm_new, const float* in, float* out);
void launch_classify(hipStream_t s, Profiler* prof, uint32_t n, const float4* pm, const float* level, uint8_t* size_class, const uint8_t* owned,
                     const uint32_t* orig, DeviceStatus* status, const sph_params* p);
void launch_header_ahead(sph_ctx* c, uint32_t nblocks, HeaderOut* out_dev, bool publish = false);
void launch_iisph2_scale(hipStream_t s, Profiler* prof, const SweepArgs& a);
void launch_check_aii(hipStream_t s, Profiler* prof, const SweepArgs& a);
void launch_vel_add_pacc(hipStream_t s, Profiler* prof, const SweepArgs& a);
void launch_integrate(hipStream_t s, Profiler* prof, const SweepArgs& a, float4* pm_out, int mode);

struct EditSrc {
    uint32_t obj;
    uint32_t set_idx;
};
struct EditSet {
    uint32_t fields;
    float mass, px, py, vx, vy, h2, h2_next, lvl, lvlold;
};
struct sph_ctx;
int regather_host_order(sph_ctx* c, uint32_t n_new, const EditSrc* d_src, const EditSet* d_sets);
void device_exclusive_scan_u32(hipStream_t s, const uint32_t* in, uint32_t* out, uint32_t n, uint32_t* scratch, uint32_t* total);
int transfer_on_device(struct sph_ctx* c, const struct sph_params* p, const struct sph_adapt_params* ap, const uint32_t* d_partner, const uint16_t* d_counter,
                       int merging);
```

adaptive_sph_amd/csrc/sph_sort.hip:

```cpp
#include "sph_internal.hpp"

#define RS_ITEMS 32
#define RS_TILE (64 * RS_ITEMS)

template <int NB>
__device__ __forceinline__ uint64_t rs_peers(uint32_t d, bool valid)
{
    uint64_t peers = __ballot(valid);
#pragma unroll
    for (int b = 0; b < NB; b++) {
        const bool bit = (d >> b) & 1u;
        const uint64_t m = __ballot(bit);
        peers &= bit ? m : ~m;
    }
    return peers;
}

__device__ __forceinline__ uint32_t cell_key_of(const CellKeyGen& kg, uint32_t i)
{
    if (kg.gone && i < kg.n_gone && kg.gone[i] >= kg.gone_from) return kg.g.ncells;
    const float4 p = kg.pm[i];
    if (kg.clamp) return cell_key_clamped(kg.g, p.x, p.y);
    const int cx = (int)floorf(p.x / kg.g.cs) - kg.g.minx;
    const int cy = (int)floorf(p.y / kg.g.cs) - kg.g.miny;
// ... 77 lines not shown
    constexpr int DIG = 1 << NB, PER = DIG / 256;
    __shared__ uint32_t wcount[4][DIG];
    __shared__ uint32_t gbase[DIG];
    __shared__ uint32_t wsum[4];
    const int tid = threadIdx.x, lane = tid & 63, w = tid >> 6;
    for (int k = 0; k < 4; k++)
        for (int q = 0; q < PER; q++) wcount[k][tid * PER + q] = 0;
    {
        uint32_t t[PER], sum = 0;
        for (int q = 0; q < PER; q++) {
            t[q] = totals[tid * PER + q];
            sum += t[q];
        }
        uint32_t x = sum;
#pragma unroll
        for (int o = 1; o < 64; o <<= 1) {
            const uint32_t y = __shfl_up(x, o, 64);
            if (lane >= o) x += y;
        }
        if (lane == 63) wsum[w] = x;
        __syncthreads();
        uint32_t off = x - sum;
        for (int k = 0; k < w; k++) off += wsum[k];
        for (int q = 0; q < PER; q++) {
            gbase[tid * PER + q] = off + hist[(size_t)(tid * PER + q) * nblocks + blockIdx.x];
            off += t[q];
        }
    }
    const uint32_t base = blockIdx.x * RS_TILE + w * (RS_TILE / 4);
    const uint64_t lt = (1ull << lane) - 1ull;
    uint32_t k_[RS_ITEMS / 4], v_[RS_ITEMS / 4], d_[RS_ITEMS / 4], rank_[RS_ITEMS / 4];
    bool ok_[RS_ITEMS / 4];
    __syncthreads();
#pragma unroll
    for (int r = 0; r < RS_ITEMS / 4; r++) {
        const uint32_t idx = base + r * 64 + lane;
        ok_[r] = idx < n;
        k_[r] = ok_[r] ? key_in[idx] : 0u;
        v_[r] = ok_[r] ? val_in[idx] : 0u;
        d_[r] = (k_[r] >> shift) & (uint32_t)(DIG - 1);
        const uint64_t peers = rs_peers<NB>(d_[r], ok_[r]);
        const uint32_t before = wcount[w][d_[r]];
        rank_[r] = before + (uint32_t)__popcll(peers & lt);
        __builtin_amdgcn_wave_barrier();
        if (ok_[r] && (peers & lt) == 0ull) wcount[w][d_[r]] = before + (uint32_t)__popcll(peers);
        __builtin_amdgcn_wave_barrier();
    }
    __syncthreads();
    for (int q = 0; q < PER; q++) {
        const int d = tid * PER + q;
        uint32_t run = gbase[d];
        for (int k = 0; k < 4; k++) {
            const uint32_t c = wcount[k][d];
            wcount[k][d] = run;
            run += c;
        }
    }
    __syncthreads();
#pragma unroll
    for (int r = 0; r < RS_ITEMS / 4; r++) {
        if (ok_[r]) {
            const uint32_t dst = wcount[w][d_[r]] + rank_[r];
            key_out[dst] = k_[r];
            val_out[dst] = v_[r];
        }
    }
}

#define RS_MAX_DIGITS 1024

size_t radix_sort_scratch_elems(uint32_t n)
{
    size_t nblocks = ((size_t)n + RS_TILE - 1) / RS_TILE;
    return RS_MAX_DIGITS * (nblocks ? nblocks : 1) + RS_MAX_DIGITS;
}

template <int NB>
static void radix_pass(hipStream_t s, Profiler* prof, uint32_t* ki, uint32_t* vi, uint32_t* ko, uint32_t* vo, uint32_t n, int shift,
                       uint32_t nblocks, uint32_t* hist, uint32_t* totals, const CellKeyGen* kg)
{
    {
        ProfScope ps(prof, "sort_hist", s);
        if (kg) hipLaunchKernelGGL((k_rs_hist<NB, true>), dim3(nblocks), dim3(256), 0, s, ki, vi, n, shift, nblocks, hist, *kg);
        else hipLaunchKernelGGL((k_rs_hist<NB, false>), dim3(nblocks), dim3(256), 0, s, ki, vi, n, shift, nblocks, hist, CellKeyGen{});
    }
    {
        ProfScope ps(prof, "sort_rowscan", s);
        hipLaunchKernelGGL(k_rs_rowscan, dim3(1 << NB), dim3(256), 0, s, hist, nblocks, totals);
    }
    {
        ProfScope ps(prof, "sort_scatter", s);
        hipLaunchKernelGGL(k_rs_scatter<NB>, dim3(nblocks), dim3(256), 0, s, ki, vi, ko, vo, n, shift, nblocks, hist, totals);
    }
}

int radix_sort_pairs(hipStream_t s, Profiler* prof, uint32_t* keyA, uint32_t* valA, uint32_t* keyB, uint32_t* valB, uint32_t n,
                     int bits, uint32_t* scratch, const CellKeyGen* keygen)
{
    if (n == 0) return 0;
    uint32_t nblocks = (n + RS_TILE - 1) / RS_TILE;
    uint32_t* hist = scratch;
    uint32_t* totals = scratch + (size_t)RS_MAX_DIGITS * nblocks;
    if (bits < 1) bits = 1;
    const int passes = (bits + 9) / 10;
    int nb = (bits + passes - 1) / passes;
    if (nb < 8) nb = 8;
    int cur = 0;
    for (int p = 0; p < passes; p++) {
        uint32_t *ki = cur ? keyB : keyA, *vi = cur ? valB : valA, *ko = cur ? keyA : keyB, *vo = cur ? valA : valB;
        const CellKeyGen* kg = p == 0 ? keygen : nullptr;
        if (nb == 8) radix_pass<8>(s, prof, ki, vi, ko, vo, n, p * nb, nblocks, hist, totals, kg);
        else if (nb == 9) radix_pass<9>(s, prof, ki, vi, ko, vo, n, p * nb, nblocks, hist, totals, kg);
        else radix_pass<10>(s, prof, ki, vi, ko, vo, n, p * nb, nblocks, hist, totals, kg);
        cur ^= 1;
    }
    return cur;
}

struct IncGrid {
    GridP cur, nxt;
};
__device__ __forceinline__ void inc_cur_range(const IncGrid& G, uint32_t c, const uint32_t* __restrict__ cell_start_cur, uint32_t& b, uint32_t& e)
{
    const uint32_t cy = c / (uint32_t)G.nxt.sx, cx = c - cy * (uint32_t)G.nxt.sx;
    const int ox = (int)cx + G.nxt.minx - G.cur.minx, oy = (int)cy + G.nxt.miny - G.cur.miny;
    b = e = 0u;
    if (ox >= 0 && ox < G.cur.sx && oy >= 0 && oy < G.cur.sy) {
        const uint32_t k = (uint32_t)ox + (uint32_t)oy * (uint32_t)G.cur.sx;
        b = cell_start_cur[k];
        e = cell_start_cur[k + 1];
    }
}

__global__ __launch_bounds__(256) void k_inc_classify(uint32_t n, const float4* __restrict__ pm, IncClassifyP q)
{
    const uint32_t i = blockIdx.x * 256 + threadIdx.x;
    if (i >= n) return;
    const float4 p = pm[i];
    inc_classify_particle(q, i, p.x, p.y);
}

__global__ __launch_bounds__(256) void k_inc_classify_slab(uint32_t n, uint32_t n_prev, CellKeyGen kg, IncClassifyP q)
{
    const uint32_t i = blockIdx.x * 256 + threadIdx.x;
    if (i >= n) return;
    if (kg.gone && i < kg.n_gone && kg.gone[i] >= kg.gone_from) {
        q.mv[i] = 2;
        return;
    }
    const uint32_t k = cell_key_of(kg, i);
    inc_register(q, i, k, i >= n_prev || k != inc_key_of_cur_cell(q.cur, q.nxt, q.cxy_cur[i]));
}

#define INC_CELLS 1024
__global__ __launch_bounds__(INC_CELLS) void k_inc_count(IncGrid G, const uint32_t* __restrict__ cell_start_cur, const uint8_t* __restrict__ mv,
                                                          const uint32_t* __restrict__ next, const unsigned long long* __restrict__ head, uint32_t epoch,
                                                          uint32_t* __restrict__ count , uint32_t* __restrict__ bsum,
                                                          uint32_t* __restrict__ movers)
{
    __shared__ uint32_t ws[INC_CELLS / 64], wm[INC_CELLS / 64];
    const uint32_t c = blockIdx.x * (uint32_t)INC_CELLS + threadIdx.x;
    uint32_t cnt = 0, listed = 0;
    if (c < G.nxt.ncells) {
        uint32_t b, e;
        inc_cur_range(G, c, cell_start_cur, b, e);
        const unsigned long long h = head[c];
        for (uint32_t j = b; j < e; j++) cnt += mv[j] ? 0u : 1u;
        if ((uint32_t)(h >> 32) == epoch)
            for (uint32_t m = (uint32_t)h; m; m = next[m - 1u]) listed++;
        cnt += listed;
        count[c] = cnt;
    }
    uint32_t x = cnt, y = listed;
    for (int o = 32; o > 0; o >>= 1) {
        x += (uint32_t)__shfl_xor((int)x, o, 64);
        y += (uint32_t)__shfl_xor((int)y, o, 64);
    }
    if ((threadIdx.x & 63) == 0) {
        ws[threadIdx.x >> 6] = x;
        wm[threadIdx.x >> 6] = y;
    }
    __syncthreads();
    if (threadIdx.x == 0) {
        uint32_t t = 0, m = 0;
        for (int k = 0; k < INC_CELLS / 64; k++) {
            t += ws[k];
            m += wm[k];
        }
        bsum[blockIdx.x] = t;
        if (m) atomicAdd(movers, m);
    }
}

__global__ __launch_bounds__(256) void k_inc_scan(uint32_t ncells, uint32_t* __restrict__ cell_start, const uint32_t* __restrict__ bsum, uint32_t* __restrict__ movers,
                                                   uint32_t* __restrict__ movers_host)
{
    __shared__ uint32_t ws[4], base_s;
    const int tid = threadIdx.x, lane = tid & 63, w = tid >> 6;
    uint32_t pre = 0;
    for (uint32_t k = tid; k < blockIdx.x; k += 256) pre += bsum[k];
    for (int o = 32; o > 0; o >>= 1) pre += (uint32_t)__shfl_xor((int)pre, o, 64);
    if (lane == 0) ws[w] = pre;
    __syncthreads();
    if (tid == 0) base_s = ws[0] + ws[1] + ws[2] + ws[3];
    __syncthreads();
    const uint32_t c0 = blockIdx.x * (uint32_t)INC_CELLS + 4u * (uint32_t)tid;
    uint32_t v[4];
#pragma unroll
    for (uint32_t u = 0; u < 4u; u++) v[u] = c0 + u < ncells ? cell_start[c0 + u] : 0u;
    const uint32_t own = v[0] + v[1] + v[2] + v[3];
    uint32_t x = own;
#pragma unroll
    for (int o = 1; o < 64; o <<= 1) {
        const uint32_t y = __shfl_up(x, o, 64);
        if (lane >= o) x += y;
    }
    if (lane == 63) ws[w] = x;
    __syncthreads();
    uint32_t run = base_s + x - own;
    for (int k = 0; k < w; k++) run += ws[k];
#pragma unroll
    for (uint32_t u = 0; u < 4u; u++) {
        if (c0 + u < ncells) cell_start[c0 + u] = run;
        run += v[u];
        if (c0 + u + 1u == ncells) cell_start[ncells] = run;
    }
    if (blockIdx.x == 0 && tid == 0) {
        *movers_host = *movers;
        *movers = 0u;
    }
}

template <bool PERM>
__global__ __launch_bounds__(256) void k_inc_place_reorder(uint32_t n, IncGrid G, const uint32_t* __restrict__ cell_start_cur, const uint32_t* __restrict__ cell_start_nxt,
                                                            const uint32_t* __restrict__ nk, const uint8_t* __restrict__ mv, const uint32_t* __restrict__ next,
                                                            const unsigned long long* __restrict__ head, uint32_t epoch, const uint32_t* __restrict__ cxy_cur,
                                                            uint32_t* __restrict__ key_out, ReorderIO io, uint32_t* __restrict__ perm_out)
{
    const uint32_t i = blockIdx.x * 256 + threadIdx.x;
    if (i >= n) return;
    const uint32_t flag = mv[i];
    if (PERM && flag == 2u) return;
    const uint32_t c = nk[i];
    const bool mover = flag != 0u;
    const uint32_t own = mover ? 0u : cxy_cur[i];
    float4 pm;
    float2 vel;
    uint32_t orig = 0;
    float lvl = 0.f, lvlold = 0.f;
    if (!PERM) {
        pm = io.pm_in[i];
        vel = io.vel_in[i];
        orig = io.orig_in[i];
        lvl = io.lvl_in[i];
        lvlold = io.lvlold_in[i];
    }
    const unsigned long long h = head[c];
    const uint32_t first = cell_start_nxt[c];
    uint32_t b, e, r = 0;
    if (!mover) {
        const uint32_t k = (own & 0xffffu) + (own >> 16) * (uint32_t)G.cur.sx;
        b = cell_start_cur[k];
        e = i;
    } else {
        uint32_t eb;
        inc_cur_range(G, c, cell_start_cur, b, eb);
        e = i >= eb ? eb : b;
    }
    for (uint32_t j = b; j < e; j++) r += mv[j] ? 0u : 1u;
    if ((uint32_t)(h >> 32) == epoch)
        for (uint32_t m = (uint32_t)h; m; m = next[m - 1u]) r += (m - 1u < i) ? 1u : 0u;
    const uint32_t dst = first + r;
    key_out[dst] = c;
    if (PERM) {
        perm_out[dst] = i;
        return;
    }
    io.pm_out[dst] = pm;
    io.vel_out[dst] = vel;
    io.orig_out[dst] = orig;
    io.lvl_out[dst] = lvl;
    io.lvlold_out[dst] = lvlold;
    if (io.h2n_in) io.h2n_out[dst] = io.h2n_in[i];
    if (io.lam_in) io.lam_prev_out[dst] = io.lam_in[i];
    if (io.szc_in) io.szc_out[dst] = io.szc_in[i];
    const uint32_t cy = c / (uint32_t)G.nxt.sx;
    io.cxy_out[dst] = (c - cy * (uint32_t)G.nxt.sx) | (cy << 16);
}

size_t incremental_sort_block_sums(uint32_t ncells) { return ((size_t)ncells + INC_CELLS - 1) / INC_CELLS; }

void incremental_cell_sort_reorder(hipStream_t s, Profiler* prof, uint32_t n, const float4* pm_new, const IncClassifyP& q, bool classified,
                                   const uint32_t* cell_start_cur, uint32_t* key_out, uint32_t* cell_start_out, const ReorderIO& io, uint32_t* bsum, uint32_t* movers,
                                   uint32_t* movers_host)
{
    const IncGrid G{q.cur, q.nxt};
    const uint32_t ncells = q.nxt.ncells, cblocks = (uint32_t)incremental_sort_block_sums(ncells);
    if (!classified) {
        ProfScope ps(prof, "inc_classify", s);
        hipLaunchKernelGGL(k_inc_classify, dim3((n + 255) / 256), dim3(256), 0, s, n, pm_new, q);
    }
    {
        ProfScope ps(prof, "inc_count", s);
        hipLaunchKernelGGL(k_inc_count, dim3(cblocks), dim3(INC_CELLS), 0, s, G, cell_start_cur, q.mv, q.next, q.head, q.epoch, cell_start_out, bsum, movers);
    }
    {
        ProfScope ps(prof, "inc_scan", s);
        hipLaunchKernelGGL(k_inc_scan, dim3(cblocks), dim3(256), 0, s, ncells, cell_start_out, bsum, movers, movers_host);
    }
    {
        ProfScope ps(prof, "inc_reorder", s);
        hipLaunchKernelGGL(k_inc_place_reorder<false>, dim3((n + 255) / 256), dim3(256), 0, s, n, G, cell_start_cur, cell_start_out, q.nk, q.mv, q.next, q.head,
                           q.epoch, q.cxy_cur, key_out, io, (uint32_t*)nullptr);
    }
}

void incremental_cell_sort_perm(hipStream_t s, Profiler* prof, uint32_t n, uint32_t n_prev, const CellKeyGen& kg, const IncClassifyP& q, const uint32_t* cell_start_cur,
                                uint32_t* key_out, uint32_t* perm_out, uint32_t* cell_start_out, uint32_t* bsum, uint32_t* movers, uint32_t* movers_host)
{
    const IncGrid G{q.cur, q.nxt};
    const uint32_t ncells = q.nxt.ncells, cblocks = (uint32_t)incremental_sort_block_sums(ncells);
    {
        ProfScope ps(prof, "inc_classify", s);
        hipLaunchKernelGGL(k_inc_classify_slab, dim3((n + 255) / 256), dim3(256), 0, s, n, n_prev, kg, q);
    }
    {
        ProfScope ps(prof, "inc_count", s);
        hipLaunchKernelGGL(k_inc_count, dim3(cblocks), dim3(INC_CELLS), 0, s, G, cell_start_cur, q.mv, q.next, q.head, q.epoch, cell_start_out, bsum, movers);
    }
    {
        ProfScope ps(prof, "inc_scan", s);
        hipLaunchKernelGGL(k_inc_scan, dim3(cblocks), dim3(256), 0, s, ncells, cell_start_out, bsum, movers, movers_host);
    }
    {
        ProfScope ps(prof, "inc_place", s);
        hipLaunchKernelGGL(k_inc_place_reorder<true>, dim3((n + 255) / 256), dim3(256), 0, s, n, G, cell_start_cur, cell_start_out, q.nk, q.mv, q.next, q.head, q.epoch,
                           q.cxy_cur, key_out, ReorderIO{}, perm_out);
    }
}

__global__ __launch_bounds__(256) void k_reorder(uint32_t n, GridP g, const uint32_t* __restrict__ sorted_key,
                                                  const uint32_t* __restrict__ perm, const float4* __restrict__ pm_in,
                                                  const float2* __restrict__ vel_in, const uint32_t* __restrict__ orig_in,
                                                  const float* __restrict__ lvl_in, const float* __restrict__ lvlold_in,
                                                  float4* __restrict__ pm_out, float2* __restrict__ vel_out,
                                                  uint32_t* __restrict__ orig_out, float* __restrict__ lvl_out,
                                                  float* __restrict__ lvlold_out, uint32_t* __restrict__ cxy,
                                                  const float* __restrict__ h2n_in, float* __restrict__ h2n_out,
                                                  const float* __restrict__ lam_in, float* __restrict__ lam_prev_out,
                                                  uint32_t* __restrict__ zero_word, const uint8_t* __restrict__ szc_in,
                                                  uint8_t* __restrict__ szc_out)
{
    uint32_t i = blockIdx.x * 256 + threadIdx.x;
    if (i == 0 && zero_word) *zero_word = 0u;
    if (i >= n) return;
    uint32_t src = perm[i];
    if (h2n_in) h2n_out[i] = h2n_in[src];
    if (lam_in) lam_prev_out[i] = lam_in[src];
    if (szc_in) szc_out[i] = szc_in[src];
    pm_out[i] = pm_in[src];
    vel_out[i] = vel_in[src];
    orig_out[i] = orig_in[src];
    lvl_out[i] = lvl_in[src];
    lvlold_out[i] = lvlold_in[src];
    uint32_t k = sorted_key[i];
    uint32_t cy = k / (uint32_t)g.sx;
    uint32_t cx = k - cy * (uint32_t)g.sx;
    cxy[i] = cx | (cy << 16);
}

void launch_reorder(hipStream_t s, Profiler* prof, uint32_t n, GridP g, const uint32_t* sorted_key, const uint32_t* perm, const ReorderIO& io,
                    void* cell_start_scratch)
{
    ProfScope ps(prof, "reorder", s);
    hipLaunchKernelGGL(k_reorder, dim3((n + 255) / 256), dim3(256), 0, s, n, g, sorted_key, perm, io.pm_in, io.vel_in, io.orig_in, io.lvl_in,
                       io.lvlold_in, io.pm_out, io.vel_out, io.orig_out, io.lvl_out, io.lvlold_out, io.cxy_out, io.h2n_in, io.h2n_out, io.lam_in,
                       io.lam_prev_out, (uint32_t*)cell_start_scratch, io.szc_in, io.szc_out);
}

#define CS_INLINE 64u
#define CS_WORK_CAP 65536u

struct CellGap {
    uint32_t lo, hi, val;
};

__global__ __launch_bounds__(256) void k_cell_start(const uint32_t* __restrict__ key, uint32_t n, uint32_t ncells,
                                                     uint32_t* __restrict__ cell_start, CellGap* __restrict__ work,
                                                     uint32_t* __restrict__ work_count)
{
    uint32_t i = blockIdx.x * 256 + threadIdx.x;
    if (i > n) return;
    uint32_t lo, hi;
    if (i == 0) {
        lo = 0;
        hi = n ? key[0] : ncells;
    } else if (i == n) {
        lo = key[n - 1] + 1;
        hi = ncells;
    } else {
        uint32_t a = key[i - 1], b = key[i];
        if (a == b) return;
        lo = a + 1;
        hi = b;
    }
    if (hi - lo >= CS_INLINE) {
        uint32_t slot = atomicAdd(work_count, 1u);
        if (slot < CS_WORK_CAP) {
            work[slot] = CellGap{lo, hi, i};
            return;
        }
    }
    for (uint32_t c = lo; c <= hi; c++) cell_start[c] = i;
}

__global__ __launch_bounds__(256) void k_cell_fill(const CellGap* __restrict__ work, const uint32_t* __restrict__ work_count,
                                                    uint32_t* __restrict__ cell_start)
{
    const uint32_t cnt = min(*work_count, CS_WORK_CAP);
    for (uint32_t e = blockIdx.x; e < cnt; e += gridDim.x) {
        const CellGap g = work[e];
        for (uint32_t c = g.lo + threadIdx.x; c <= g.hi; c += 256) cell_start[c] = g.val;
    }
}

size_t cell_start_scratch_bytes() { return (size_t)CS_WORK_CAP * sizeof(CellGap) + 16; }

void launch_cell_start(hipStream_t s, Profiler* prof, const uint32_t* sorted_key, uint32_t n, uint32_t ncells, uint32_t* cell_start,
                       void* scratch, bool count_zeroed)
{
    ProfScope ps(prof, "cell_start", s);
    uint32_t* count = (uint32_t*)scratch;
    CellGap* work = (CellGap*)((char*)scratch + 16);
    if (!count_zeroed) (void)hipMemsetAsync(count, 0, sizeof(uint32_t), s);
    hipLaunchKernelGGL(k_cell_start, dim3((n + 1 + 255) / 256), dim3(256), 0, s, sorted_key, n, ncells, cell_start, work, count);
    hipLaunchKernelGGL(k_cell_fill, dim3(512), dim3(256), 0, s, work, count, cell_start);
}

__global__ __launch_bounds__(256) void k_tile_hmax(uint32_t n, const float4* __restrict__ pm, GridP g, int ts, int tsx, uint32_t* __restrict__ raw)
{
    const uint32_t i = blockIdx.x * 256 + threadIdx.x;
    uint32_t tile = 0xffffffffu, hb = 0u;
    if (i < n) {
        const float4 p = pm[i];
        int cx = (int)floorf(p.x / g.cs) - g.minx, cy = (int)floorf(p.y / g.cs) - g.miny;
        cx = min(max(cx, 0), g.sx - 1);
        cy = min(max(cy, 0), g.sy - 1);
        tile = (uint32_t)(cy / ts) * (uint32_t)tsx + (uint32_t)(cx / ts);
        hb = __float_as_uint(p.w);
    }
    const int lane = threadIdx.x & 63;
    for (int o = 1; o < 64; o <<= 1) {
        const uint32_t ot = (uint32_t)__shfl_down((int)tile, o, 64), oh = (uint32_t)__shfl_down((int)hb, o, 64);
        if (lane + o < 64 && ot == tile) hb = max(hb, oh);
    }
    const uint32_t prev = (uint32_t)__shfl_up((int)tile, 1, 64);
    if (i < n && (lane == 0 || prev != tile)) atomicMax(&raw[tile], hb);
}
__global__ __launch_bounds__(256) void k_tile_dilate(int tsx, int tsy, int D, const uint32_t* __restrict__ raw, uint32_t* __restrict__ out)
{
    const uint32_t t = blockIdx.x * 256 + threadIdx.x;
    if (t >= (uint32_t)tsx * (uint32_t)tsy) return;
    const int tx = (int)(t % (uint32_t)tsx), ty = (int)(t / (uint32_t)tsx);
    uint32_t m = 0;
    for (int dy = -D; dy <= D; dy++)
        for (int dx = -D; dx <= D; dx++) {
            const int x = tx + dx, y = ty + dy;
            if (x >= 0 && x < tsx && y >= 0 && y < tsy) m = max(m, raw[(uint32_t)y * (uint32_t)tsx + (uint32_t)x]);
        }
    out[t] = m;
}

void launch_tile_hmax(hipStream_t s, Profiler* prof, uint32_t n, const float4* pm, GridP g, int ts, int tsx, int tsy, uint32_t* raw, uint32_t* out,
                      uint32_t* out_ext, int d_ext)
{
    ProfScope ps(prof, "tile_hmax", s);
    const uint32_t nt = (uint32_t)tsx * (uint32_t)tsy;
    (void)hipMemsetAsync(raw, 0, (size_t)nt * 4, s);
    if (n) hipLaunchKernelGGL(k_tile_hmax, dim3((n + 255) / 256), dim3(256), 0, s, n, pm, g, ts, tsx, raw);
    hipLaunchKernelGGL(k_tile_dilate, dim3((nt + 255) / 256), dim3(256), 0, s, tsx, tsy, 1, raw, out);
    if (out_ext) hipLaunchKernelGGL(k_tile_dilate, dim3((nt + 255) / 256), dim3(256), 0, s, tsx, tsy, d_ext, raw, out_ext);
}

void launch_tile_redilate(hipStream_t s, Profiler* prof, int tsx, int tsy, int d, const uint32_t* raw, uint32_t* out)
{
    ProfScope ps(prof, "tile_hmax", s);
    const uint32_t nt = (uint32_t)tsx * (uint32_t)tsy;
    hipLaunchKernelGGL(k_tile_dilate, dim3((nt + 255) / 256), dim3(256), 0, s, tsx, tsy, d, raw, out);
}
```

adaptive_sph_amd/csrc/sph_step.hip:

```cpp
#include <atomic>
#include <hip/hip_runtime.h>
#include <rccl/rccl.h>

#include <array>
#include <cmath>
#include <cstdlib>
#include <cstring>
#include <condition_variable>
#include <functional>
#include <memory>
#include <mutex>
#include <vector>

#include "sph_dist.hpp"

SweepArgs make_args(sph_ctx* c, const StepP& sp)
{
    SweepArgs a{};
    const int k = c->cur;
    a.g = c->fgrid;
    a.sp = sp;
    a.n = c->dist.on ? c->dist.n_tot : (uint32_t)c->n;
    a.exact = c->exact;
    a.cell_start = c->cell_start.as<uint32_t>();
// ... 131 lines not shown
{
    c->hint_word = nullptr;
    return wait_word(c, &((volatile SolverCtrl*)c->ctrl_host)->seq, c->publish_seq);
}

__global__ void k_publish_words(const uint32_t* __restrict__ src, uint32_t n, uint32_t* __restrict__ dst_host, uint32_t* __restrict__ seq_host,
                                uint32_t seq)
{
    if (threadIdx.x == 0 && blockIdx.x == 0) {
        for (uint32_t k = 0; k < n; k++) dst_host[k] = src[k];
        __threadfence_system();
        *(volatile uint32_t*)seq_host = seq;
    }
}
int publish_and_wait(sph_ctx* c, const void* dev_words, uint32_t n_words)
{
    c->publish_seq++;
    if (c->publish_seq == 0u) c->publish_seq = 1u;
    hipLaunchKernelGGL(k_publish_words, dim3(1), dim3(64), 0, c->stream, (const uint32_t*)dev_words, n_words, c->dist.counts_host_dev + 16,
                       c->dist.counts_host_dev + 63, c->publish_seq);
    return wait_word(c, (volatile uint32_t*)c->dist.counts_host + 63, c->publish_seq);
}

__global__ void k_publish_count(const uint32_t* __restrict__ flags, uint32_t n, uint32_t* __restrict__ dst_host, uint32_t seq_slot, uint32_t seq)
{
    uint32_t v = 0;
    for (uint32_t k = threadIdx.x; k < n; k += 64) v += flags[k] ? 1u : 0u;
    v = wave_sum_u32(v);
    if (threadIdx.x == 0 && blockIdx.x == 0) {
        dst_host[0] = v;
        __threadfence_system();
        ((volatile uint32_t*)dst_host)[seq_slot] = seq;
    }
}

static int ilog2_ceil(uint32_t v)
{
    int b = 0;
    while ((1ull << b) < (uint64_t)v) b++;
    return b;
}

struct HostTrace {
    bool on = false;
    std::chrono::steady_clock::time_point t0;
    double acc[8] = {0};
    int steps = 0;
    void start(bool enabled)
    {
        on = enabled;
        if (on) t0 = std::chrono::steady_clock::now();
    }
    void mark(int k)
    {
        if (!on) return;
        auto t1 = std::chrono::steady_clock::now();
        acc[k] += std::chrono::duration<double, std::micro>(t1 - t0).count();
        t0 = t1;
    }
    void end_step()
    {
        if (!on) return;
        if (++steps % 20 == 0)
            fprintf(stderr, "[sph trace] per step us: decomposition %.1f | header %.1f | neighbourhood launches %.1f | first sweeps %.1f | div solve %.1f | dens solve %.1f\n",
                    acc[0] / steps, acc[1] / steps, acc[2] / steps, acc[3] / steps, acc[4] / steps, acc[5] / steps);
    }
};
static thread_local HostTrace g_trace;

void dbg_sync(sph_ctx* c, const char* what, int id)
{
    if (!(c->opt.debug_sync & (1 << id))) return;
    (void)hipSetDevice(c->device);
    const hipError_t e = hipStreamSynchronize(c->stream);
    fprintf(stderr, "[sph debug] rank %d step %llu: %s -> %s\n", c->dist.rank, (unsigned long long)c->step_number, what, hipGetErrorString(e));
}

int wait_all_hinted(Group& G)
{
    for (auto c : G.m) {
        int rc = wait_hinted(c);
        if (rc) return rc;
    }
    return SPH_OK;
}
int wait_all(Group& G)
{
    for (auto c : G.m) {
        int rc = wait_stream(c);
        if (rc) return rc;
    }
    return SPH_OK;
}

int agree(Group& G, int local_rc)
{
    if (!G.multi()) return local_rc;
    std::vector<int> v(G.m.size(), local_rc);
    int rc = G.comm->allreduce_max_i32(G, v);
    if (rc) return rc;
    if (local_rc) return local_rc;
    if (v[0]) return G.m[0]->fail(v[0], "another rank of the slab decomposition reported status %d", v[0]);
    return SPH_OK;
}

int sync_ctrl(Group& G, int mode)
{
    int rc = SPH_OK;
    if (!G.multi()) mode = SYNC_AGREE;
    for (auto c : G.m) {
        (void)hipSetDevice(c->device);
        launch_publish(c);
    }
    uint32_t peer = 0;
    for (auto c : G.m) {
        int r = wait_publish(c);
        if (r && !rc) rc = r;
        if (mode == SYNC_DEFER) continue;
        if (!r && c->status_host->error) {
            uint32_t code = c->status_host->error, info = c->status_host->info;
            (void)hipMemsetAsync(c->status.p, 0, sizeof(DeviceStatus), c->stream);
            c->status_host->error = 0;
            r = c->fail((int)code, "%s (particle i=%u)", status_message(code), info);
            if (!rc) rc = r;
        }
        if (!r && c->ctrl_host->peer_error > peer) peer = c->ctrl_host->peer_error;
    }
    if (mode == SYNC_FINAL) {
        if (!rc && peer) rc = G.m[0]->fail(peer > 1 ? (int)peer : SPH_ERR_DEVICE, "another rank of the slab decomposition reported status %u", peer);
        return rc;
    }
    if (mode == SYNC_DEFER) return rc;
    return agree(G, rc);
}

static float* sel_rho(Member& m) { return m.a.rho; }
static float* sel_vel(Member& m) { return (float*)m.a.vel; }
static float* sel_pt0(Member& m) { return m.a.pt0; }
static float* sel_pt1(Member& m) { return m.a.pt1; }
static float* sel_rec0(Member& m) { return (float*)m.a.rec0; }
static float* sel_rec1(Member& m) { return (float*)m.a.rec1; }
static float* sel_lv_level(Member& m) { return m.lv_level; }
static float* sel_lv_when(Member& m) { return m.lv_when; }
static float* sel_lv_pmnew(Member& m) { return m.lv_pmnew; }

struct SolveQ {
    float max_avg_error;
    int residual_density;
    uint32_t max_iters;
    int tail;
    bool density_solver;
    int tot_slot = 0;
    uint32_t k = 1, upto = 2;
    void extend() { upto = k + std::max(1u, k / 4u); }
};
static int solve_sweep_a(Group& G, std::vector<Member>& M, const SolveQ& q, uint32_t k)
{
    const int multi = G.multi() ? 1 : 0;
    for (auto& m : M) {
        (void)hipSetDevice(m.c->device);
        if (m.n) launch_pressure_accel(m.c->stream, &m.c->prof, m.a, (int)k, q.residual_density, q.max_avg_error, q.max_iters, multi);
        else if (!multi) {
            SolverCtrl z{};
            z.done = 1u;
            z.slot_done[0] = z.slot_done[1] = 1u;
            z.cur = k & 1u;
            (void)hipMemcpyAsync(m.c->ctrl.p, &z, sizeof z, hipMemcpyHostToDevice, m.c->stream);
        } else (void)hipMemsetAsync(m.c->dist.solver_tot.as<double>() + 8 * q.tot_slot, 0, 48, m.c->stream);
    }
    if (multi) return G.comm->allreduce_solver(G, q.tot_slot);
    return SPH_OK;
}
#ifndef SPLIT_MIN_PARTICLES
#define SPLIT_MIN_PARTICLES 786432u
#endif
static bool split_sweep_a(const Group& G, const std::vector<Member>& M)
{
    const int env = G.m[0]->dist.overlap_env;
    if (env == 0 || G.comm == nullptr || G.m[0]->dist.nranks <= 1 || G.m[0]->dist.xstream == nullptr) return false;
    if (env > 0) return true;
    uint32_t n_max = 0;
    for (auto& m : M) n_max = std::max(n_max, m.n);
    return n_max >= SPLIT_MIN_PARTICLES;
}
static int exchange_and_sweep_a(Group& G, std::vector<Member>& M, const SolveQ& q, uint32_t ka)
{
    int rc;
    const bool recs = sweep_a_on_records(M[0].a);
    float* (*sel)(Member&) = recs ? ((ka & 1u) ? sel_rec1 : sel_rec0) : ((ka & 1u) ? sel_pt1 : sel_pt0);
    const int stride = recs ? 4 : 1, off = recs ? 2 : 0;
    const TotalsJob job{(int)ka - 1, q.residual_density, q.max_avg_error, q.max_iters};
    if (!split_sweep_a(G, M)) {
        if (!G.multi()) return solve_sweep_a(G, M, q, ka);
        for (auto& m : M) {
            sph_ctx* c = m.c;
            (void)hipSetDevice(c->device);
            if (!m.n) HIPCHK(c, hipMemsetAsync(c->dist.solver_tot.as<double>() + 8 * q.tot_slot, 0, 48, c->stream));
        }
        if ((rc = refresh_ghosts(G, M, sel, 1, "pt", q.tot_slot, nullptr, stride, off, &job))) return rc;
        for (auto& m : M) {
            (void)hipSetDevice(m.c->device);
            if (m.n) launch_pressure_accel(m.c->stream, &m.c->prof, m.a, (int)ka, q.residual_density, q.max_avg_error, q.max_iters, 2);
            else launch_solver_progress(m.c->stream, &m.c->prof, m.a, (int)ka - 1, q.residual_density, q.max_avg_error, q.max_iters);
        }
        return SPH_OK;
    }
    for (auto& m : M) {
        sph_ctx* c = m.c;
        auto& d = c->dist;
        (void)hipSetDevice(c->device);
        HIPCHK(c, hipEventRecord(d.ev_x[0], c->stream));
        HIPCHK(c, hipStreamWaitEvent(d.xstream, d.ev_x[0], 0));
        if (m.n) launch_pressure_accel(d.xstream, &c->prof, m.a, (int)ka, q.residual_density, q.max_avg_error, q.max_iters, 1, 1);
        HIPCHK(c, hipEventRecord(d.ev_x[1], d.xstream));
        if (!m.n) HIPCHK(c, hipMemsetAsync(c->dist.solver_tot.as<double>() + 8 * q.tot_slot, 0, 48, c->stream));
    }
    if ((rc = refresh_ghosts(G, M, sel, 1, "pt", q.tot_slot, nullptr, stride, off, &job))) return rc;
    for (auto& m : M) {
        sph_ctx* c = m.c;
        (void)hipSetDevice(c->device);
        launch_solver_progress(c->stream, &c->prof, m.a, (int)ka - 1, q.residual_density, q.max_avg_error, q.max_iters);
        HIPCHK(c, hipStreamWaitEvent(c->stream, c->dist.ev_x[1], 0));
        if (m.n) launch_pressure_accel(c->stream, &c->prof, m.a, (int)ka, q.residual_density, q.max_avg_error, q.max_iters, 1, 2);
    }
    return SPH_OK;
}
static int solve_begin(Group& G, std::vector<Member>& M, SolveQ& q, uint32_t predicted_iters)
{
    int rc;
    if ((rc = exchange_and_sweep_a(G, M, q, 1))) return rc;
    q.k = 1;
    q.upto = predicted_iters > 2 ? predicted_iters : 2;
    return SPH_OK;
}
static int solve_queue(Group& G, std::vector<Member>& M, SolveQ& q, bool handoff = false, bool publish_next = false)
{
    int rc;
    const int multi = G.multi() ? 1 : 0;
    for (; q.k <= q.upto && q.k <= q.max_iters; q.k++) {
        const uint32_t k = q.k;
        for (auto& m : M) {
            (void)hipSetDevice(m.c->device);
            if (m.n) launch_jacobi_update(m.c->stream, &m.c->prof, m.a, (int)k, q.residual_density, q.max_avg_error, q.max_iters, multi);
        }
        if ((rc = exchange_and_sweep_a(G, M, q, k + 1))) return rc;
    }
    for (auto& m : M) {
        (void)hipSetDevice(m.c->device);
        SolverCtrl* hand_host = handoff ? m.c->ctrl_host_dev + 1 : nullptr;
        uint32_t* gate_out = handoff ? (uint32_t*)(m.c->ctrl.as<SolverCtrl>() + 2) : nullptr;
        if (!m.n || q.tail == 0 ) {
            if (handoff) launch_solver_handoff(m.c->stream, &m.c->prof, m.c->ctrl.as<SolverCtrl>(), hand_host, gate_out);
            continue;
        }
        launch_solver_tail(m.c->stream, &m.c->prof, m.a, q.tail, m.c->pm[m.c->pcur ^ 1].as<float4>(), -1, q.residual_density,
                           q.max_avg_error, q.max_iters, hand_host, gate_out);
        if (q.tail == 1  && source_term_on_records(m.a)) m.a.xv_ok = true;
        if (q.tail >= 2  && m.a.hdr_partials) launch_header_ahead(m.c, (m.n + 255u) / 256u, m.c->hdr_host_dev, publish_next && !multi);
    }
    return SPH_OK;
}
static void solve_stats(Member& m, const SolveQ& q, const SolverCtrl& h)
{
    m.c->pressure_cur = h.cur;
    sph_solver_stats* st = q.density_solver ? &m.st.density_solver : &m.st.div_solver;
    st->iters = h.iters;
    st->converged = 1;
    st->normal_count = h.normal;
    st->singular_count = h.singular;
    st->negative_count = h.negative;
    st->avg_error = h.normal > 0 ? h.sum_err / (float)h.normal : NAN;
    st->max_error = h.max_err;
}


static uint32_t pace_lead(const sph_ctx* c, uint32_t n)
{
    if (c->opt.pace_lead > 0) return (uint32_t)c->opt.pace_lead;
    return std::min(8u, std::max(1u, (450000u + n - 1u) / std::max(n, 1u)));
}
static uint32_t pace_prediction(const sph_ctx* c, uint32_t n, uint32_t last, uint32_t prev)
{
    const int mode = c->opt.pace_pred;
    const int md = mode == 0xffff ? (n >= 450000u ? 0 : 1) : mode;
    if (md == 0) return 2u;
    if (md == 2 || prev == 0u) return last;
    return std::min(last, prev);
}
static int solve_paced(Group& G, std::vector<Member>& M, SolveQ& q, uint32_t predicted_iters)
{
    const bool multi = G.multi();
    size_t lead_member = 0;
    while (lead_member + 1 < M.size() && M[lead_member].n == 0) lead_member++;
    Member& m = M[lead_member];
    sph_ctx* c = m.c;
    const uint32_t lead = multi ? 1u : pace_lead(c, m.n);
    int rc;
    sph_ctx* c0 = M[0].c;
    c0->solve_epoch = c0->solve_epoch >= 0xffffu ? 1u : c0->solve_epoch + 1u;
    const uint32_t epoch = c0->solve_epoch;
    for (auto& mm : M) {
        mm.c->solve_epoch = epoch;
        mm.a.prog_host = mm.c->prog_host_dev;
        mm.a.prog_epoch = epoch;
    }
    if ((rc = solve_begin(G, M, q, multi ? 2u : predicted_iters))) return rc;
    auto iteration = [&](uint32_t k) -> int {
        for (auto& mm : M) {
            (void)hipSetDevice(mm.c->device);
            if (mm.n) launch_jacobi_update(mm.c->stream, &mm.c->prof, mm.a, (int)k, q.residual_density, q.max_avg_error, q.max_iters, multi ? 1 : 0);
        }
        return exchange_and_sweep_a(G, M, q, k + 1);
    };
    for (; q.k <= q.upto && q.k <= q.max_iters; q.k++)
        if ((rc = iteration(q.k))) return rc;
    auto t0 = std::chrono::steady_clock::now();
    int last_seen = -2;
    for (uint64_t spins = 0;; spins++) {
        const uint32_t w = *c->prog_host;
        const bool seen = (w >> 16) == epoch;
        if (seen && (w & 0x8000u)) break;
        const int decided = seen ? (int)(w & 0x7fffu) : -1;
        if (q.k <= q.max_iters && (int)q.k - 1 - decided < (int)lead) {
            if ((rc = iteration(q.k))) return rc;
            q.k++;
            continue;
        }
        if (decided != last_seen) {
            last_seen = decided;
            t0 = std::chrono::steady_clock::now();
        } else if ((spins & 0xffffu) == 0xffffu && std::chrono::duration<double>(std::chrono::steady_clock::now() - t0).count() > 2.0) {
            if ((rc = wait_stream(c))) return rc;
            const uint32_t w2 = *c->prog_host;
            if ((w2 >> 16) == epoch && (w2 & 0x8000u)) break;
            if ((w2 >> 16) == epoch && (int)(w2 & 0x7fffu) != decided) continue;
            return c->fail(SPH_ERR_DEVICE, "pressure solve: the device finished its queue without a stop decision (iteration %u queued)", q.k - 1);
        }
    }
    q.upto = q.k - 1;
    for (auto& mm : M) mm.a.prog_host = nullptr;
    return SPH_OK;
}

static int pressure_iterations(Group& G, std::vector<Member>& M, float max_avg_error, int residual_density, uint32_t max_iters,
                               uint32_t predicted_iters, int tail, bool density_solver, bool final_solve,
                               const std::function<int()>* behind_tail = nullptr )
{
    int rc;
    const int multi = G.multi() ? 1 : 0;
    SolveQ q{max_avg_error, residual_density, max_iters, tail, density_solver};
    if ((multi || M[0].n > 0) && M[0].c->paced_step) {
        sph_ctx* c0 = M[0].c;
        const uint32_t head = density_solver ? pace_prediction(c0, M[0].n, c0->last_dens_iters, c0->prev_dens_iters) : pace_prediction(c0, M[0].n, c0->last_div_iters, c0->prev_div_iters);
        if ((rc = solve_paced(G, M, q, head))) return rc;
        if ((rc = solve_queue(G, M, q, false, true))) return rc;
        if (behind_tail && (rc = (*behind_tail)())) return rc;
        if (multi && final_solve && (rc = G.comm->agree_guards_queued(G))) return rc;
        if ((rc = sync_ctrl(G, multi ? (final_solve ? SYNC_FINAL : SYNC_DEFER) : SYNC_AGREE))) return rc;
        for (auto& m : M) solve_stats(m, q, *m.c->ctrl_host);
        return SPH_OK;
    }
    if ((rc = solve_begin(G, M, q, predicted_iters))) return rc;
    for (;;) {
        if ((rc = solve_queue(G, M, q, false, true))) return rc;
        if (multi && final_solve && (rc = G.comm->agree_guards_queued(G))) return rc;
        if ((rc = sync_ctrl(G, multi ? (final_solve ? SYNC_FINAL : SYNC_DEFER) : SYNC_AGREE))) return rc;
        if (M[0].c->ctrl_host->done) break;
        if (q.k > max_iters) break;
        q.extend();
    }
    for (auto& m : M) solve_stats(m, q, *m.c->ctrl_host);
    return SPH_OK;
}

ReorderIO reorder_io(sph_ctx* c, const float4* pm_in, float4* pm_out, uint32_t* cxy, bool lam)
{
    const int k = c->cur;
    return ReorderIO{pm_in, c->vel[k].as<float2>(), c->orig[k].as<uint32_t>(), c->lvl[k].as<float>(), c->lvlold[k].as<float>(), pm_out, c->vel[k ^ 1].as<float2>(),
                     c->orig[k ^ 1].as<uint32_t>(), c->lvl[k ^ 1].as<float>(), c->lvlold[k ^ 1].as<float>(), cxy, c->h2n[k].as<float>(), c->h2n[k ^ 1].as<float>(),
                     lam ? c->lam_sum.as<float>() : nullptr, lam ? c->lam_prev.as<float>() : nullptr, c->szc[k].as<uint8_t>(), c->szc[k ^ 1].as<uint8_t>()};
}

struct CellSortBufs {
    DevBuf *key, *val;
    DevBuf* cell_start;
};
static void radix_cell_build(sph_ctx* c, const CellSortBufs& v, const CellKeyGen& kg, uint32_t n_sort, int bits, uint32_t n, const ReorderIO& io)
{
    if (n_sort && radix_sort_pairs(c->stream, &c->prof, v.key[0].as<uint32_t>(), v.val[0].as<uint32_t>(), v.key[1].as<uint32_t>(), v.val[1].as<uint32_t>(), n_sort, bits,
                                   c->sort_scratch.as<uint32_t>(), &kg) == 1) {
        std::swap(v.key[0], v.key[1]);
        std::swap(v.val[0], v.val[1]);
    }
    if (n) launch_reorder(c->stream, &c->prof, n, kg.g, v.key[0].as<uint32_t>(), v.val[0].as<uint32_t>(), io, c->cs_scratch.p);
    launch_cell_start(c->stream, &c->prof, v.key[0].as<uint32_t>(), n, kg.g.ncells, v.cell_start->as<uint32_t>(), c->cs_scratch.p, n > 0);
}

static int ensure_inc_sort_scratch(sph_ctx* c, uint32_t ncells)
{
    const size_t head_before = c->inc_head.bytes;
    HIPCHK(c, c->inc_head.ensure((size_t)ncells * 8));
    if (c->inc_head.bytes != head_before) HIPCHK(c, hipMemsetAsync(c->inc_head.p, 0, c->inc_head.bytes, c->stream));
    HIPCHK(c, c->inc_next.ensure((size_t)c->cap * 4));
    HIPCHK(c, c->inc_bsum.ensure(incremental_sort_block_sums(ncells) * 4));
    if (!c->inc_movers.p) {
        HIPCHK(c, c->inc_movers.ensure(4));
        HIPCHK(c, hipMemsetAsync(c->inc_movers.p, 0, 4, c->stream));
    }
    if (++c->inc_epoch == 0u) c->inc_epoch = 1u;
    return SPH_OK;
}

static int level_setup(Member& m, const sph_params* p, bool after, LevelArgs& l)
{
    sph_ctx* c = m.c;
    const size_t n = m.n ? m.n : 1;
    HIPCHK(c, c->lvl_tmp.ensure((c->cap ? c->cap : 1) * 4));
    HIPCHK(c, c->lvl_nrm.ensure(n * 8));
    HIPCHK(c, c->lvl_when.ensure(n * 4));
    HIPCHK(c, c->lvl_mark.ensure(n * 8));
    HIPCHK(c, c->stash.ensure(n * 4));
    for (DevBuf* b : {&c->lvl_state, &c->flag_surface, &c->flag_insufficient}) HIPCHK(c, b->ensure(n));
    HIPCHK(c, c->nl_ext.ensure(sweep_list_bytes((uint32_t)n)));
    HIPCHK(c, c->nlx_ext.ensure(sweep_index_list_bytes((uint32_t)n)));
    HIPCHK(c, c->lvl_changed_d.ensure(1024 * sizeof(uint32_t)));
    if (!after) {
        m.a = make_args(c, m.sp);
        m.a.h_mode = p->support_length_estimation;
        m.a.sp_check_aii = p->check_aii;
    }
    l = LevelArgs{};
    l.k = p->level_estimation_range / SPH_ETA;
    l.threshold = cosf(50.f * (SPH_PI_F / 180.f));
    l.max_surface_distance = p->maximum_surface_distance;
    l.boundary_is_fluid_surface = p->boundary_is_fluid_surface;
    l.maximum_range = (p->support_length_estimation == SPH_H_FROM_DISTRIBUTION || p->support_length_estimation == SPH_H_FROM_DISTRIBUTION2)
                          ? p->maximum_range : -1.f;
    l.nrm = c->lvl_nrm.as<float2>();
    l.state = c->lvl_state.as<uint8_t>();
    l.flag_surface = c->flag_surface.as<uint8_t>();
    l.flag_insufficient = c->flag_insufficient.as<uint8_t>();
    l.size_class = c->szc[c->cur].as<uint8_t>();
    l.level = c->lvl[c->cur].as<float>();
    l.when = c->lvl_when.as<uint32_t>();
    l.mark = c->lvl_mark.as<uint32_t>();
    l.level_old = c->lvlold[c->cur].as<float>();
    l.stash_first = p->fill_stash_with == SPH_STASH_SURFACE_DISTANCE_FIRST ? c->stash.as<float>() : nullptr;
    l.center_diff = p->level_estimation_method == SPH_LEVEL_CENTER_DIFF;
    l.replay_step_lists = after && !p->use_extended_range_for_level_estimation;
    m.a.nl_ext = l.replay_step_lists ? m.a.nl : c->nl_ext.as<uint4>();
    m.a.nlx_ext = l.replay_step_lists ? m.a.nlx : c->nlx_ext.as<uint4>();
    return SPH_OK;
}

static void redilate_tiles_for_slack(sph_ctx* c, hipStream_t s, float k, float slack)
{
    const float tile_side = (float)c->tile_ts * c->fgrid.cs;
    const int d = (int)ceilf((k * c->h_max_step + slack) / tile_side);
    launch_tile_redilate(s, &c->prof, c->tile_tsx, c->tile_tsy, d < 1 ? 1 : d, c->tile_raw.as<uint32_t>(), c->tile_h_ext.as<uint32_t>());
}

struct LevelBatches {
    uint32_t t = 1, effective = 0;
    int B = 8;
};
static void level_queue_batch(sph_ctx* c, hipStream_t ls, const SweepArgs& al, const LevelArgs& lv, bool stash_middle, LevelBatches& st)
{
    uint32_t* chg = c->lvl_changed_d.as<uint32_t>();
    (void)hipMemsetAsync(chg, 0, (size_t)st.B * sizeof(uint32_t), ls);
    for (int b = 0; b < st.B; b++, st.t++) {
        launch_level_propagate(ls, &c->prof, al, lv, st.t, chg + b);
        if (st.t == 1u && stash_middle) launch_fill_stash(ls, &c->prof, al, lv, c->stash.as<float>());
    }
    c->level_seq++;
    if (c->level_seq == 0u) c->level_seq = 1u;
    hipLaunchKernelGGL(k_publish_count, dim3(1), dim3(64), 0, ls, chg, (uint32_t)st.B, c->lvl_changed_dev, 63u, c->level_seq);
}
static int level_collect_batches(sph_ctx* c, hipStream_t ls, const SweepArgs& al, const LevelArgs& lv, bool stash_middle, LevelBatches& st)
{
    for (;; level_queue_batch(c, ls, al, lv, stash_middle, st)) {
        if (int rc = wait_word(c, (volatile uint32_t*)c->lvl_changed + 63, c->level_seq)) return rc;
        const uint32_t changed = c->lvl_changed[0];
        st.effective += changed;
        if (changed < (uint32_t)st.B) break;
        st.B = 8;
    }
    c->last_level_sweeps = st.effective;
    return SPH_OK;
}

static int group_step_inner(Group& G, const sph_params* p, sph_step_stats* outs, bool* started)
{
    int rc = SPH_OK;
    g_trace.start(G.m[0]->opt.hip_trace != 0);
    std::vector<Member> M(G.m.size());
    for (size_t i = 0; i < G.m.size(); i++) {
        M[i].c = G.m[i];
        M[i].n = (uint32_t)G.m[i]->n;
        memset(&M[i].st, 0, sizeof(sph_step_stats));
        M[i].wall0 = std::chrono::steady_clock::now();
    }
    sph_ctx* c0 = G.m[0];
    if (c0->n_planes == 0) return c0->fail(SPH_ERR_NO_BOUNDARY, "not implemented: NoBoundaryHandler::iisph_aii");
    const bool h_from_mass_mode = p->support_length_estimation == SPH_H_FROM_MASS;
    const bool level_on = p->level_estimation_method != SPH_LEVEL_NONE;
    const bool level_after = level_on && p->level_estimation_after_advection;
    if (level_on && !level_after && p->level_estimation_method == SPH_LEVEL_CENTER_DIFF)
        return c0->fail(SPH_ERR_INVALID_ARGUMENT, "center diff level estimation method needs density values");
    if (!p->level_estimation_after_advection && !p->use_extended_range_for_level_estimation)
        return c0->fail(SPH_ERR_INVALID_ARGUMENT, "assertion failed: simulation_params.use_extended_range_for_level_estimation");
    if (!G.multi() && c0->n == 0) return c0->fail(SPH_ERR_INVALID_ARGUMENT, "called `Option::unwrap()` on a `None` value (no particles)");
    if (!p->level_estimation_after_advection && !(p->level_estimation_range / SPH_ETA >= 2.f))
        return c0->fail(SPH_ERR_UNSUPPORTED, "level_estimation_range / 1.9 = %g < 2: the reference then steps on lists narrower than the SPH support, which this build does not cover",
                        (double)(p->level_estimation_range / SPH_ETA));
    for (auto c : G.m)
        if (c->poisoned) return c->refuse_poisoned();
    *started = true;
    const bool no_records = c0->opt.accel_generic != 0;
    const bool paced = c0->opt.paced != 0 && p->max_iters <= 0x7fffu && (!G.multi() || c0->opt.slab_paced != 0);
    for (auto c : G.m) c->paced_step = paced;
    for (auto c : G.m) c->dist.overlap_env = c0->opt.overlap;
    for (auto c : G.m) c->publish_folded = false;

    const bool tev = c0->prof.mode == 1;
    for (auto& m : M) {
        (void)hipSetDevice(m.c->device);
        if (tev) (void)hipEventRecord(m.c->ev[0], m.c->stream);
    }

    std::vector<std::vector<float>> red(M.size(), std::vector<float>(8));
    int hdr_rc = SPH_OK, setup_rc = SPH_OK;
    bool slab_fused = false;
    const float slab_slack_k = (level_on && p->level_estimation_after_advection && G.multi())
                                   ? fmaxf(2.f, c0->h_max_step > 0.f ? 4.f * c0->last_dmax / c0->h_max_step : 0.f) : 0.f;
    const float halo_base_k = fmaxf(4.f, level_on ? p->level_estimation_range / SPH_ETA : 0.f);
    auto header_ready = [&](sph_ctx* c) { return h_from_mass_mode && c->hdr_ahead && c->hdr_ahead_rest_density == p->rest_density; };
    const bool ahead_usable = !G.multi() && header_ready(c0);
    auto fill_red = [&]() {
        for (size_t i = 0; i < M.size(); i++) {
            const HeaderOut h = *M[i].c->hdr_host;
            const bool any = M[i].c->n > 0;
            red[i][0] = any ? -h.h_max : 0.f;
            red[i][1] = any ? h.h_min : INFINITY;
            red[i][2] = any ? h.min_cfl : INFINITY;
            red[i][3] = -(float)hdr_rc;
            red[i][4] = any ? h.min_x : INFINITY;
            red[i][5] = any ? -h.max_x : INFINITY;
            red[i][6] = any ? h.min_y : INFINITY;
            red[i][7] = any ? -h.max_y : INFINITY;
            M[i].c->hdr_ahead = false;
        }
    };
    if (G.multi()) {
        bool rebalanced = false;
        const int every = c0->dist.rebalance_every;
        if (every > 0 && c0->step_number > 0 && c0->step_number % (uint64_t)every == 0 && c0->h_max_step > 0.f)
            if ((rc = rebalance_cuts(G, M, &rebalanced))) return rc;
        bool launched = false;
        for (auto& m : M) {
            sph_ctx* c = m.c;
// ... 375 lines not shown
            done = last[0] < B;
        }
        for (auto& m : M) {
            m.c->have_level = true;
            m.st.ms_level_estimation += std::chrono::duration<double, std::milli>(std::chrono::steady_clock::now() - t_lvl0).count();
        }
        return SPH_OK;
    };
    if (level_on && G.multi() && !level_after) {
        if ((rc = level_estimation_slabs(false))) return rc;
        for (auto& m : M) dbg_sync(m.c, "level estimation (slabs)", 4);
    } else if (level_on && !level_after) {
        if ((rc = level_estimation(nullptr, nullptr, !c0->opt.level_serial))) return rc;
    } else if (!level_on) {
        for (auto& m : M) m.c->have_level = false;
    }

    for (auto& m : M) {
        (void)hipSetDevice(m.c->device);
        m.a.nloff = nullptr;
        m.a.nlh = nullptr;
        const bool offsets = m.n && m.c->opt.offset_lists && sweeps_want_offset_lists(m.a);
        if (offsets) {
            HIPCHK(m.c, m.c->nloff.ensure(sweep_offset_list_bytes(m.a.n ? m.a.n : 1u)));
            HIPCHK(m.c, m.c->nlh.ensure((size_t)(m.a.n ? m.a.n : 1u)));
            m.a.nloff_out = m.c->nloff.as<uint2>();
            m.a.nlh_out = m.c->nlh.as<uint8_t>();
        }
        if (m.n) launch_density(m.c->stream, &m.c->prof, m.a);
        m.a.nloff_out = nullptr;
        m.a.nlh_out = nullptr;
        if (offsets) {
            m.a.nloff = m.c->nloff.as<uint2>();
            m.a.nlh = m.c->nlh.as<uint8_t>();
        }
        if (m.n) launch_profile_calibration(m.c);
        if (p->check_neighborhood && m.n) launch_check_neighborhood(m.c, m.a);
    }
    for (auto& m : M) m.c->have_reduced = false;
    float dt_step = dt;
    if (p->constrain_neighborhood_count) {
        const float onn = (SPH_ETA * 2.f) * (SPH_ETA * 2.f);
        const uint32_t target = (uint32_t)onn + 5u;
        for (auto& m : M) {
            sph_ctx* c = m.c;
            (void)hipSetDevice(c->device);
            const size_t n = m.n ? m.n : 1;
            HIPCHK(c, c->con_thr.ensure(n * 4));
            HIPCHK(c, c->con_consumed.ensure(n * 4));
            HIPCHK(c, c->con_h.ensure(n * 4));
            HIPCHK(c, c->flag_reduced.ensure(n));
            HIPCHK(c, c->lvl_changed_d.ensure(64 * sizeof(uint32_t)));
            launch_constrain_init(c->stream, &c->prof, m.a, target, c->con_thr.as<float>(), c->con_consumed.as<uint32_t>(), c->con_h.as<float>(),
                                  c->flag_reduced.as<uint8_t>());
        }
        bool any = false;
        for (auto& m : M) any = any || m.n > 0;
        for (bool done = !any && !G.multi(); !done;) {
            const int B = 4;
            for (auto& m : M) {
                sph_ctx* c = m.c;
                (void)hipSetDevice(c->device);
                uint32_t* pend = c->lvl_changed_d.as<uint32_t>();
                (void)hipMemsetAsync(pend, 0, B * sizeof(uint32_t), c->stream);
                for (int b = 0; b < B && m.n; b++)
                    launch_constrain_pass(c->stream, &c->prof, m.a, target, c->con_thr.as<float>(), c->con_consumed.as<uint32_t>(), c->con_h.as<float>(), pend + b);
                HIPCHK(c, hipMemcpyAsync(c->lvl_changed, pend, B * sizeof(uint32_t), hipMemcpyDeviceToHost, c->stream));
            }
            if ((rc = sync_ctrl(G))) return rc;
            std::vector<int> pending(M.size(), 0);
            for (size_t i = 0; i < M.size(); i++) pending[i] = M[i].c->lvl_changed[B - 1] ? 1 : 0;
            if (G.multi() && (rc = G.comm->allreduce_max_i32(G, pending))) return rc;
            done = true;
            for (int v : pending) done = done && !v;
        }
        for (auto& m : M) {
            sph_ctx* c = m.c;
            (void)hipSetDevice(c->device);
            if (m.n) launch_constrain_apply(c->stream, &c->prof, m.a, c->pm[c->pcur].as<float4>(), c->con_h.as<float>(), m.a.h2_next);
            m.lv_pmnew = (float*)c->pm[c->pcur].as<float4>();
        }
        if ((rc = refresh_ghosts(G, M, sel_lv_pmnew, 4, "pm"))) return rc;
        std::vector<std::vector<float>> cfl(M.size(), std::vector<float>(1, INFINITY));
        for (auto& m : M) {
            sph_ctx* c = m.c;
            (void)hipSetDevice(c->device);
            if (m.n) launch_header(c, m.n, p->rest_density, 0, c->hdr_host_dev, c->dist.on && c->have_flags ? c->dist.owned.as<uint8_t>() : nullptr);
        }
        if ((rc = sync_ctrl(G))) return rc;
        for (size_t i = 0; i < M.size(); i++)
            if (M[i].n && M[i].c->n > 0) cfl[i][0] = M[i].c->hdr_host->min_cfl;
        if (G.multi() && (rc = G.comm->allreduce_min_f32(G, cfl))) return rc;
        if (!G.multi())
            for (size_t i = 1; i < M.size(); i++) cfl[0][0] = fminf(cfl[0][0], cfl[i][0]);
        dt_step = fminf(p->max_dt, p->cfl_factor * sqrtf(cfl[0][0]));
        for (auto& m : M) {
            sph_ctx* c = m.c;
            (void)hipSetDevice(c->device);
            m.sp.dt = dt_step;
            m.sp.hyb_vfactor = fminf(dt_step * p->hybrid_dfsph_factor, 1.f);
            m.a.sp = m.sp;
            m.st.dt = dt_step;
            if (m.n) launch_density_replay(c->stream, &c->prof, m.a);
            c->have_reduced = true;
        }
    }
    if ((rc = refresh_ghosts(G, M, sel_rho, 1, "rho"))) return rc;
    if (G.multi())
        for (auto& m : M) {
            sph_ctx* c = m.c;
            (void)hipSetDevice(c->device);
            slab_ghost_mrho(c, m.a);
        }
    const bool np_first = p->pressure_solver_method != SPH_SOLVER_HYBRID_DFSPH || p->hybrid_dfsph_non_pressure_accel_before_divergence_free;
    const bool np_fused = np_first && !p->check_aii && !c0->opt.no_fuse;
    for (auto& m : M) {
        (void)hipSetDevice(m.c->device);
        if (m.n && np_fused) {
            launch_aii_const_non_pressure(m.c->stream, &m.c->prof, m.a);
            continue;
        }
        if (m.n) launch_aii_const(m.c->stream, &m.c->prof, m.a);
        if (m.n && p->check_aii) launch_check_aii(m.c->stream, &m.c->prof, m.a);
    }
    auto non_pressure = [&]() -> int {
        for (auto& m : M) {
            sph_ctx* c = m.c;
            (void)hipSetDevice(c->device);
            if (m.n && !np_fused) launch_non_pressure(c->stream, &c->prof, m.a);
            std::swap(c->vel[c->cur], c->vel_tmp);
            m.a.vel = c->vel[c->cur].as<float2>();
            m.a.vel_tmp = c->vel_tmp.as<float2>();
            m.a.xv_ok = m.n && source_term_on_records(m.a);
        }
        return refresh_ghosts(G, M, sel_vel, 2, "vel");
    };
    auto begin_solve = [&](int kind, int residual_density) {
        for (auto& m : M) {
            (void)hipSetDevice(m.c->device);
            if (!m.n) launch_ctrl_reset(m.c->stream, m.c->ctrl.as<SolverCtrl>(), m.a.gate);
            if (m.n) launch_source_term(m.c->stream, &m.c->prof, m.a, kind, residual_density);
        }
    };
    auto rec = [&](int e) {
        if (tev)
            for (auto& m : M) {
                (void)hipSetDevice(m.c->device);
                (void)hipEventRecord(m.c->ev[e], m.c->stream);
            }
    };
    enum { T_NONE = 0, T_VEL = 1, T_VX = 2, T_HYBRID = 3 };
    g_trace.mark(3);
    struct AheadPlan {
        bool on = false, incremental = false;
        GridP g{};
        int tile_ts = 0, tile_tsx = 0, tile_tsy = 0;
        IncClassifyP q{};
    } plan;
    auto plan_ahead_build = [&]() -> int {
        sph_ctx* c = c0;
        plan = AheadPlan{};
        if (G.multi() || !paced || !c->opt.ahead_build || !h_from_mass_mode || p->constrain_neighborhood_count || (!c->uniform_h && c->tile_ts <= 0) ||
            (c->uniform_h && c->tile_ts != 0) || c->exact || M[0].n == 0)
            return SPH_OK;
        const uint32_t n = M[0].n;
        const float cs = c->fgrid.cs;
        const int ts = c->tile_ts, margin = 2 * (ts > 0 ? ts : 1);
        GridP g;
        if (!plan_grid(boxes[0], cs, margin, g)) return SPH_OK;
        if (ts > 0) {
            plan.tile_ts = ts;
            plan.tile_tsx = tiles_across(g.sx, ts);
            plan.tile_tsy = tiles_across(g.sy, ts);
            const size_t nt = (size_t)plan.tile_tsx * (size_t)plan.tile_tsy;
            HIPCHK(c, c->atile_raw.ensure(nt * 4));
            HIPCHK(c, c->atile_h.ensure(nt * 4));
        }
        for (int q = 0; q < 2; q++) {
            HIPCHK(c, c->akey[q].ensure((size_t)c->cap * 4));
            HIPCHK(c, c->aval[q].ensure((size_t)c->cap * 4));
        }
        HIPCHK(c, c->acxy.ensure((size_t)c->cap * 4));
        HIPCHK(c, c->pm2.ensure((size_t)c->cap * sizeof(float4)));
        HIPCHK(c, c->acell_start.ensure(((size_t)g.ncells + 1) * 4));
        plan.on = true;
        plan.g = g;
        if (!(c->opt.inc_sort && c->grid_valid && c->fgrid.cs == cs && c->fgrid.ncells > 0 && inc_sort_fits(g.ncells, n) &&
              inc_sort_worthwhile(c->inc_count_valid, *c->movers_host, inc_sort_mover_limit(n, c->opt.inc_sort), c->inc_radix_streak)))
            return SPH_OK;
        if ((rc = ensure_inc_sort_scratch(c, g.ncells))) return rc;
        plan.incremental = true;
        plan.q = IncClassifyP{c->fgrid, g, c->cxy.as<uint32_t>(), c->akey[1].as<uint32_t>(), c->aval[1].as<uint8_t>(), c->inc_next.as<uint32_t>(),
                              c->inc_head.as<unsigned long long>(), c->inc_epoch};
        M[0].a.inc = plan.q;
        return SPH_OK;
    };
    bool ahead_deferred = level_on;
    const std::function<int()> queue_ahead_build = [&]() -> int {
        sph_ctx* c = c0;
        if (ahead_deferred) return SPH_OK;
        c->ahead_valid = false;
        if (!plan.on) return SPH_OK;
        const uint32_t n = M[0].n;
        const GridP g = plan.g;
        hipStream_t s = c->stream;
        const float4* integrated = c->pm[c->pcur ^ 1].as<float4>();
        if (plan.incremental) {
            incremental_cell_sort_reorder(s, &c->prof, n, integrated, plan.q,  true, c->cell_start.as<uint32_t>(), c->akey[0].as<uint32_t>(),
                                          c->acell_start.as<uint32_t>(), reorder_io(c, integrated, c->pm2.as<float4>(), c->acxy.as<uint32_t>(), false),
                                          c->inc_bsum.as<uint32_t>(), c->inc_movers.as<uint32_t>(), (uint32_t*)(c->ctrl_host_dev + 2) + 1);
            c->inc_count_valid = true;
        } else {
            const CellKeyGen kg{integrated, g, nullptr, 0u, (uint32_t)SC_GONE_FROM, 1};
            radix_cell_build(c, CellSortBufs{c->akey, c->aval, &c->acell_start}, kg, n, ilog2_ceil(g.ncells), n,
                             reorder_io(c, integrated, c->pm2.as<float4>(), c->acxy.as<uint32_t>(), true));
        }
        if (plan.tile_ts > 0)
            launch_tile_hmax(s, &c->prof, n, c->pm2.as<float4>(), g, plan.tile_ts, plan.tile_tsx, plan.tile_tsy, c->atile_raw.as<uint32_t>(), c->atile_h.as<uint32_t>(),
                             nullptr, 1);
        c->ahead_valid = true;
        c->ahead.g = g;
        c->ahead.h_max = h_max_g;
        c->ahead.h_min = h_min_g;
        c->ahead.tile_ts = plan.tile_ts;
        c->ahead.tile_tsx = plan.tile_tsx;
        c->ahead.tile_tsy = plan.tile_tsy;
        c->ahead.rest_density = p->rest_density;
        c->ahead.n = c->n;
        return SPH_OK;
    };

    switch (p->pressure_solver_method) {
    case SPH_SOLVER_IISPH:
        if ((rc = non_pressure())) return rc;
        rec(4);
        begin_solve(1, 1);
        if ((rc = plan_ahead_build())) return rc;
        if ((rc = pressure_iterations(G, M, p->iisph_max_avg_density_error, 1, p->max_iters, c0->last_dens_iters, T_VX, true, !level_on, &queue_ahead_build))) return rc;
        rec(5);
        break;
    case SPH_SOLVER_IISPH2:
        if ((rc = non_pressure())) return rc;
        rec(4);
        begin_solve(3, 1);
        if ((rc = pressure_iterations(G, M, p->iisph_max_avg_density_error, 1, p->max_iters, c0->last_dens_iters, T_NONE, true, false))) return rc;
        for (auto& m : M) {
            (void)hipSetDevice(m.c->device);
            if (m.n) launch_iisph2_scale(m.c->stream, &m.c->prof, m.a);
        }
        if ((rc = refresh_ghosts(G, M, M[0].c->pressure_cur ? sel_pt1 : sel_pt0, 1, "pt"))) return rc;
        for (auto& m : M) {
            (void)hipSetDevice(m.c->device);
            if (!m.n) continue;
            launch_pressure_accel(m.c->stream, &m.c->prof, m.a, -1, 1, 0.f, 0u, G.multi() ? 1 : 0);
            launch_solver_tail(m.c->stream, &m.c->prof, m.a, T_VX, m.c->pm[m.c->pcur ^ 1].as<float4>());
            if (m.a.hdr_partials) launch_header_ahead(m.c, (m.n + 255u) / 256u, m.c->hdr_host_dev);
        }
        if (G.multi() && !level_on && (rc = G.comm->agree_guards_queued(G))) return rc;
        if ((rc = sync_ctrl(G, G.multi() ? (level_on ? SYNC_DEFER : SYNC_FINAL) : SYNC_AGREE))) return rc;
        rec(5);
        break;
    case SPH_SOLVER_ONLY_DIVERGENCE:
        if ((rc = non_pressure())) return rc;
        rec(2);
        begin_solve(0, 0);
        if ((rc = plan_ahead_build())) return rc;
        if ((rc = pressure_iterations(G, M, p->hybrid_dfsph_max_avg_divergence_error, 0, p->max_iters, c0->last_div_iters, T_VX, false, !level_on, &queue_ahead_build))) return rc;
        rec(3);
        break;
    default: {
        if (p->hybrid_dfsph_non_pressure_accel_before_divergence_free)
            if ((rc = non_pressure())) return rc;
        rec(2);
        begin_solve(0, 0);
        if (paced && (G.multi() || M[0].n > 0)) {
            const bool multi = G.multi();
            SolveQ qd{p->hybrid_dfsph_max_avg_divergence_error, 0, p->max_iters, T_VEL, false};
            SolveQ qs{p->hybrid_dfsph_max_avg_density_error, 1, p->max_iters, T_HYBRID, true};
            if ((rc = solve_paced(G, M, qd, pace_prediction(c0, M[0].n, c0->last_div_iters, c0->prev_div_iters)))) return rc;
            if ((rc = solve_queue(G, M, qd, true))) return rc;
            g_trace.mark(4);
            rec(3);
            if (multi && (rc = refresh_ghosts(G, M, sel_vel, 2, "vel"))) return rc;
            if (!p->hybrid_dfsph_non_pressure_accel_before_divergence_free)
                if ((rc = non_pressure())) return rc;
            rec(4);
            begin_solve(p->hybrid_dfsph_density_source_term == SPH_ONLY_DENSITY ? 2 : 1, 1);
            if ((rc = plan_ahead_build())) return rc;
            if ((rc = solve_paced(G, M, qs, pace_prediction(c0, M[0].n, c0->last_dens_iters, c0->prev_dens_iters)))) return rc;
            if ((rc = solve_queue(G, M, qs, false, true))) return rc;
            if ((rc = queue_ahead_build())) return rc;
            const bool final_solve = !level_on;
            if (multi && final_solve && (rc = G.comm->agree_guards_queued(G))) return rc;
            if ((rc = sync_ctrl(G, multi ? (final_solve ? SYNC_FINAL : SYNC_DEFER) : SYNC_AGREE))) return rc;
            for (auto& m : M) {
                solve_stats(m, qd, m.c->ctrl_host[1]);
                solve_stats(m, qs, *m.c->ctrl_host);
            }
            g_trace.mark(5);
            rec(5);
            break;
        }
        const bool chain_wanted = c0->opt.chain >= 0 ? c0->opt.chain == 1 : c0->last_div_iters == c0->prev_div_iters;
        const bool chain = (G.multi() || M[0].n > 0) && p->hybrid_dfsph_non_pressure_accel_before_divergence_free && chain_wanted;
        if (chain) {
            const int multi = G.multi() ? 1 : 0;
            const bool final_solve = !level_on;
            SolveQ qd{p->hybrid_dfsph_max_avg_divergence_error, 0, p->max_iters, T_VEL, false};
            SolveQ qs{p->hybrid_dfsph_max_avg_density_error, 1, p->max_iters, T_HYBRID, true};
            qs.tot_slot = 1;
            const int kind = p->hybrid_dfsph_density_source_term == SPH_ONLY_DENSITY ? 2 : 1;
            auto set_gate = [&](bool on) {
                for (auto& m : M) {
                    m.a.gate = on ? (const uint32_t*)(m.c->ctrl.as<SolverCtrl>() + 2) : nullptr;
                    m.a.solver_tot = m.c->dist.solver_tot.as<double>() + (on && m.c->dist.solver_tot.p ? 8 : 0);
                    if (m.a.tot_table) m.a.tot_table = m.c->dist.tot_table.as<double>() + (on ? (size_t)m.c->dist.nranks * 8 : 0);
                }
            };
            if ((rc = solve_begin(G, M, qd, c0->last_div_iters))) return rc;
            for (bool div_done = false;;) {
                if (!div_done) {
                    set_gate(false);
                    if ((rc = solve_queue(G, M, qd, true))) return rc;
                    g_trace.mark(4);
                    rec(3);
                    if ((rc = refresh_ghosts(G, M, sel_vel, 2, "vel"))) return rc;
                    rec(4);
                    set_gate(true);
                    begin_solve(kind, 1);
                    if ((rc = solve_begin(G, M, qs, c0->last_dens_iters))) return rc;
                }
                if ((rc = solve_queue(G, M, qs, false, true))) return rc;
                if (multi && final_solve && (rc = G.comm->agree_guards_queued(G))) return rc;
                if ((rc = sync_ctrl(G, multi ? (final_solve ? SYNC_FINAL : SYNC_DEFER) : SYNC_AGREE))) return rc;
                if (!div_done) {
                    if (!M[0].c->ctrl_host[1].done) {
                        if (qd.k > p->max_iters) return c0->fail(SPH_ERR_DEVICE, "divergence solve: no decision after max_iters iterations");
                        qd.extend();
                        continue;
                    }
                    div_done = true;
                    for (auto& m : M) solve_stats(m, qd, m.c->ctrl_host[1]);
                }
                if (M[0].c->ctrl_host->done) break;
                if (qs.k > p->max_iters) break;
                qs.extend();
            }
            set_gate(false);
            for (auto& m : M) solve_stats(m, qs, *m.c->ctrl_host);
            g_trace.mark(5);
            rec(5);
            break;
        }
        if ((rc = pressure_iterations(G, M, p->hybrid_dfsph_max_avg_divergence_error, 0, p->max_iters, c0->last_div_iters, T_VEL, false, false))) return rc;
        g_trace.mark(4);
        rec(3);
        if ((rc = refresh_ghosts(G, M, sel_vel, 2, "vel"))) return rc;
        if (!p->hybrid_dfsph_non_pressure_accel_before_divergence_free)
            if ((rc = non_pressure())) return rc;
        rec(4);
        begin_solve(p->hybrid_dfsph_density_source_term == SPH_ONLY_DENSITY ? 2 : 1, 1);
        if ((rc = pressure_iterations(G, M, p->hybrid_dfsph_max_avg_density_error, 1, p->max_iters, c0->last_dens_iters, T_HYBRID, true, !level_on))) return rc;
        g_trace.mark(5);
        rec(5);
        break;
    }
    }
    rec(6);
    if (p->viscosity_type == SPH_VISC_XSPH)
        return c0->fail(SPH_ERR_XSPH_TODO, "not yet implemented (XSPH velocity smoothing)");

    if (level_on && G.multi()) {
        if (level_after && (rc = level_estimation_slabs(true))) return rc;
        const auto t_lvl0 = std::chrono::steady_clock::now();
        for (auto& m : M) {
            m.lv_level = m.c->lvl[m.c->cur].as<float>();
            m.lv_pmnew = (float*)m.c->pm[m.c->pcur ^ 1].as<float4>();
        }
        if ((rc = refresh_ghosts(G, M, sel_lv_level, 1, "level"))) return rc;
        if (!level_after && (rc = refresh_ghosts(G, M, sel_lv_pmnew, 4, "pm_new"))) return rc;
        for (size_t i = 0; i < M.size(); i++) {
            Member& m = M[i];
            sph_ctx* c = m.c;
            (void)hipSetDevice(c->device);
            if (!m.n) continue;
            SweepArgs as = level_after ? AL[i] : m.a;
            as.pm = m.a.pm;
            launch_level_smooth(c->stream, &c->prof, as, LV[i], c->pm[c->pcur ^ 1].as<float4>(), c->lvl[c->cur].as<float>(), c->lvl_tmp.as<float>());
            std::swap(c->lvl[c->cur], c->lvl_tmp);
        }
        if ((rc = G.comm->agree_guards_queued(G))) return rc;
        if ((rc = sync_ctrl(G, SYNC_FINAL))) return rc;
        for (auto& m : M) m.st.ms_level_estimation += std::chrono::duration<double, std::milli>(std::chrono::steady_clock::now() - t_lvl0).count();
    }
    if (level_after && !G.multi()) {
        sph_ctx* c = M[0].c;
        if ((rc = level_estimation(c->pm[c->pcur ^ 1].as<float4>(), c->pm[c->pcur].as<float4>(), false))) return rc;
    }
    if (level_on && !G.multi()) {
        if ((rc = level_estimation_finish())) return rc;
        const auto t_lvl0 = std::chrono::steady_clock::now();
        Member& m = M[0];
        sph_ctx* c = m.c;
        if (m.n) {
            SweepArgs as = m.a;
            as.t_ext.slack = lv_slack;
            launch_level_smooth(c->stream, &c->prof, as, lv, c->pm[c->pcur ^ 1].as<float4>(), c->lvl[c->cur].as<float>(), c->lvl_tmp.as<float>());
            std::swap(c->lvl[c->cur], c->lvl_tmp);
        }
        if ((rc = sync_ctrl(G))) return rc;
        m.st.ms_level_estimation += std::chrono::duration<double, std::milli>(std::chrono::steady_clock::now() - t_lvl0).count();
        ahead_deferred = false;
        if ((rc = queue_ahead_build())) return rc;
    }

    for (size_t i = 0; i < M.size(); i++) {
        Member& m = M[i];
        sph_ctx* c = m.c;
        c->pcur ^= 1;
        c->lists_after = level_after && p->use_extended_range_for_level_estimation;
        c->lists_after_k = G.multi() ? LV[i].k : lv.k;
        c->lists_after_slack = G.multi() ? slab_lv_slack : lv_slack;
        c->hdr_ahead = h_from_mass_mode && m.n > 0 && m.a.hdr_partials != nullptr && !p->constrain_neighborhood_count;
        c->hdr_ahead_rest_density = p->rest_density;
        c->prev_div_iters = c->last_div_iters;
        c->prev_dens_iters = c->last_dens_iters;
        c->last_div_iters = m.st.div_solver.iters;
        c->last_dens_iters = m.st.density_solver.iters;
        c->time += dt_step;
        c->step_number += 1;
        m.st.time = c->time;
        m.st.step_number = c->step_number;
        m.st.ms_simulation_step = std::chrono::duration<double, std::milli>(std::chrono::steady_clock::now() - m.wall0).count();
        if (tev) {
            (void)hipSetDevice(c->device);
            float ms = 0.f;
            (void)hipEventSynchronize(c->ev[6]);
            if (hipEventElapsedTime(&ms, c->ev[0], c->ev[6]) == hipSuccess) m.st.ms_simulation_step = ms;
            if (hipEventElapsedTime(&ms, c->ev[0], c->ev[1]) == hipSuccess) m.st.ms_neighborhood = ms;
            const bool has_div = p->pressure_solver_method == SPH_SOLVER_ONLY_DIVERGENCE || p->pressure_solver_method == SPH_SOLVER_HYBRID_DFSPH;
            const bool has_dens = p->pressure_solver_method != SPH_SOLVER_ONLY_DIVERGENCE;
// ... 169 lines not shown
```

Baseline: 2.432 billion particle-steps/s.

## Fuse header reduction and scan into incremental cell sort kernels

```diff
diff --git a/adaptive_sph_amd/csrc/sph_api.hip b/adaptive_sph_amd/csrc/sph_api.hip
--- a/adaptive_sph_amd/csrc/sph_api.hip
+++ b/adaptive_sph_amd/csrc/sph_api.hip
@@ -219,60 +219,7 @@
     }
 }
 
-__global__ __launch_bounds__(1024) void k_header_ahead(const HeaderOut* __restrict__ partials, uint32_t nparts, const SolverCtrl* __restrict__ ctrl,
-                                                       HeaderOut* __restrict__ out, const DeviceStatus* __restrict__ status, SolverCtrl* __restrict__ h_ctrl,
-                                                       DeviceStatus* __restrict__ h_status, uint32_t seq)
-{
-    if (ctrl->done == 0u) {
-        if (h_ctrl && threadIdx.x == 0) {
-            SolverCtrl v = *ctrl;
-            v.seq = seq - 1u;
-            *h_ctrl = v;
-            *h_status = *status;
-            __threadfence_system();
-            ((volatile SolverCtrl*)h_ctrl)->seq = seq;
-        }
-        return;
-    }
-    const float INF = __uint_as_float(0x7f800000u);
-    HeaderOut o{INF, INF, -INF, -INF, 0.f, INF, INF, 0};
-    for (uint32_t k0 = threadIdx.x; k0 < nparts; k0 += 4096u) {
-        HeaderOut q[4];
-#pragma unroll
-        for (uint32_t u = 0; u < 4u; u++) q[u] = partials[min(k0 + 1024u * u, nparts - 1u)];
-#pragma unroll
-        for (uint32_t u = 0; u < 4u; u++) {
-            o.min_x = fminf(o.min_x, q[u].min_x); o.min_y = fminf(o.min_y, q[u].min_y);
-            o.max_x = fmaxf(o.max_x, q[u].max_x); o.max_y = fmaxf(o.max_y, q[u].max_y);
-            o.h_max = fmaxf(o.h_max, q[u].h_max); o.h_min = fminf(o.h_min, q[u].h_min);
-            o.min_cfl = fminf(o.min_cfl, q[u].min_cfl);
-        }
-    }
-    o.min_x = wave_min(o.min_x); o.min_y = wave_min(o.min_y); o.max_x = wave_max(o.max_x); o.max_y = wave_max(o.max_y);
-    o.h_max = wave_max(o.h_max); o.h_min = wave_min(o.h_min); o.min_cfl = wave_min(o.min_cfl);
-    __shared__ HeaderOut s[16];
-    const int lane = threadIdx.x & 63, w = threadIdx.x >> 6;
-    if (lane == 0) s[w] = o;
-    __syncthreads();
-    if (threadIdx.x == 0) {
-        HeaderOut r = s[0];
-        for (int k = 1; k < 16; k++) {
-            r.min_x = fminf(r.min_x, s[k].min_x); r.min_y = fminf(r.min_y, s[k].min_y);
-            r.max_x = fmaxf(r.max_x, s[k].max_x); r.max_y = fmaxf(r.max_y, s[k].max_y);
-            r.h_max = fmaxf(r.h_max, s[k].h_max); r.h_min = fminf(r.h_min, s[k].h_min);
-            r.min_cfl = fminf(r.min_cfl, s[k].min_cfl);
-        }
-        *out = r;
-        if (h_ctrl) {
-            SolverCtrl v = *ctrl;
-            v.seq = seq - 1u;
-            *h_ctrl = v;
-            *h_status = *status;
-            __threadfence_system();
-            ((volatile SolverCtrl*)h_ctrl)->seq = seq;
-        }
-    }
-}
+__global__ __launch_bounds__(HDR_AHEAD_THREADS) void k_header_ahead(HeaderAheadP a) { header_ahead_block(a); }
 
 __global__ __launch_bounds__(256) void k_pack_upload(uint32_t n, const float* __restrict__ mass, const float2* __restrict__ pos,
                                                       const float2* __restrict__ velin, float4* __restrict__ pm, float2* __restrict__ vel,
@@ -496,6 +443,7 @@
     o.tile = num("SPH_TILE", 0);
     o.ahead_build = num("SPH_AHEAD_BUILD", 1) != 0 ? 1 : 0;
     o.inc_sort = num("SPH_INC_SORT", 1);
+    o.boundary_fused = num("SPH_BOUNDARY_FUSED", 1) != 0 ? 1 : 0;
     o.slab_paced = num("SPH_SLAB_PACED", 1) != 0 ? 1 : 0;
     o.slab_records = num("SPH_SLAB_RECORDS", 1) != 0 ? 1 : 0;
     o.side_cus = num("SPH_SIDE_CUS", 0);
@@ -506,7 +454,7 @@
 #else
     static const char* const lab_only[] = {"SPH_PACED", "SPH_PACE_LEAD", "SPH_PACE_PRED", "SPH_CHAIN", "SPH_ACCEL_GENERIC", "SPH_JACOBI_GENERIC", "SPH_SOURCE_GENERIC",
                                            "SPH_SLAB_GENERAL", "SPH_SLAB_LEVEL_PLAIN", "SPH_LEVEL_SERIAL", "SPH_LEVEL_BATCH8", "SPH_LEVEL_QUEUE", "SPH_OFFSET_LISTS",
-                                           "SPH_NO_FUSE", "SPH_SIDE_STREAM_NORMAL", "SPH_TILE", "SPH_AHEAD_BUILD", "SPH_INC_SORT", "SPH_SLAB_PACED", "SPH_SLAB_RECORDS",
+                                           "SPH_NO_FUSE", "SPH_SIDE_STREAM_NORMAL", "SPH_TILE", "SPH_AHEAD_BUILD", "SPH_INC_SORT", "SPH_BOUNDARY_FUSED", "SPH_SLAB_PACED", "SPH_SLAB_RECORDS",
                                            "SPH_SIDE_CUS", "SPH_MAIN_EXCLUDE", "SPH_IPC_FUSE_MAX_BYTES", "SPH_IPC_COPY_MIN_BYTES"};
     static bool warned = false;
     if (!warned)
@@ -634,7 +582,7 @@
                      &c->flag_insufficient, &c->con_thr, &c->con_consumed, &c->con_h, &c->flag_reduced, &c->szc[0], &c->szc[1], &c->omega, &c->stash, &c->nl_ext, &c->nlx_ext, &c->nl_ok, &c->mrho, &c->pt0, &c->pt1, &c->prec0, &c->prec1, &c->xv, &c->rho, &c->lam_sum, &c->lam_grad, &c->wall_pl, &c->wall_cnt, &c->constf, &c->aii, &c->src, &c->p0, &c->p1, &c->pacc, &c->dens_err,
                      &c->stat, &c->ncount, &c->planes_d, &c->lam_lut, &c->dlam_lut, &c->hdr_partials, &c->hdr_out, &c->ctrl, &c->status,
                      &c->n_tiles, &c->red_partials, &c->scratch, &c->split_patterns, &c->akey[0], &c->akey[1], &c->aval[0], &c->aval[1], &c->acxy, &c->acell_start, &c->pm2,
-                     &c->atile_raw, &c->atile_h, &c->inc_head, &c->inc_next, &c->inc_bsum, &c->inc_movers, &c->cand_red, &c->rnd_rec, &c->rnd_keys, &c->rnd_out, &c->rnd_max, &c->rnd_prev, &c->rnd_layer, &c->rnd_band, &c->rnd_words, &c->rnd_stage};
+                     &c->atile_raw, &c->atile_h, &c->inc_head, &c->inc_next, &c->inc_bsum, &c->inc_movers, &c->inc_local, &c->cand_red, &c->rnd_rec, &c->rnd_keys, &c->rnd_out, &c->rnd_max, &c->rnd_prev, &c->rnd_layer, &c->rnd_band, &c->rnd_words, &c->rnd_stage};
     for (auto b : all) b->release();
     for (DevBuf* b : c->export_bufs()) b->release();
     for (DevBuf* b : c->prob_bufs()) b->release();
@@ -1538,9 +1486,8 @@
     }
 }
 
-void launch_header_ahead(sph_ctx* c, uint32_t nblocks, HeaderOut* out_dev, bool publish)
-{
-    ProfScope ps(&c->prof, "header_ahead", c->stream);
+HeaderAheadP header_ahead_args(sph_ctx* c, uint32_t nblocks, HeaderOut* out_dev, bool publish)
+{
     uint32_t seq = 0;
     if (publish) {
         c->publish_seq++;
@@ -1548,10 +1495,15 @@
         seq = c->publish_seq;
         c->publish_folded = true;
     }
-    hipLaunchKernelGGL(k_header_ahead, dim3(1), dim3(1024), 0, c->stream, c->hdr_ahead_partials.as<HeaderOut>(), nblocks, c->ctrl.as<SolverCtrl>(), out_dev,
-                       c->status.as<DeviceStatus>(), publish ? c->ctrl_host_dev : (SolverCtrl*)nullptr, publish ? c->status_host_dev : (DeviceStatus*)nullptr, seq);
-}
-
+    return HeaderAheadP{c->hdr_ahead_partials.as<HeaderOut>(), nblocks, c->ctrl.as<SolverCtrl>(), out_dev, c->status.as<DeviceStatus>(),
+                        publish ? c->ctrl_host_dev : (SolverCtrl*)nullptr, publish ? c->status_host_dev : (DeviceStatus*)nullptr, seq};
+}
+
+void launch_header_ahead(sph_ctx* c, uint32_t nblocks, HeaderOut* out_dev, bool publish)
+{
+    ProfScope ps(&c->prof, "header_ahead", c->stream);
+    hipLaunchKernelGGL(k_header_ahead, dim3(1), dim3(HDR_AHEAD_THREADS), 0, c->stream, header_ahead_args(c, nblocks, out_dev, publish));
+}
 void launch_publish(sph_ctx* c)
 {
     if (c->publish_folded) {
diff --git a/adaptive_sph_amd/csrc/sph_boundary_fused.hpp b/adaptive_sph_amd/csrc/sph_boundary_fused.hpp
--- /dev/null
+++ b/adaptive_sph_amd/csrc/sph_boundary_fused.hpp
@@ -0,0 +1,39 @@
+#pragma once
+
+#include <math.h>
+#include <stdint.h>
+
+#if defined(__HIPCC__)
+#define SPH_HD __host__ __device__ __forceinline__
+#else
+#define SPH_HD inline
+#endif
+
+struct HeaderOut {
+    float min_x, min_y, max_x, max_y, h_max, h_min, min_cfl;
+    uint32_t pad;
+};
+
+#define HDR_AHEAD_THREADS 1024u
+SPH_HD uint32_t header_ahead_slot(uint32_t k0, uint32_t u, uint32_t nparts)
+{
+    const uint32_t k = k0 + HDR_AHEAD_THREADS * u;
+    return k < nparts - 1u ? k : nparts - 1u;
+}
+SPH_HD HeaderOut header_neutral()
+{
+    const float inf = INFINITY;
+    return HeaderOut{inf, inf, -inf, -inf, 0.f, inf, inf, 0u};
+}
+SPH_HD void header_merge(HeaderOut& o, const HeaderOut& q)
+{
+    o.min_x = fminf(o.min_x, q.min_x); o.min_y = fminf(o.min_y, q.min_y);
+    o.max_x = fmaxf(o.max_x, q.max_x); o.max_y = fmaxf(o.max_y, q.max_y);
+    o.h_max = fmaxf(o.h_max, q.h_max); o.h_min = fminf(o.h_min, q.h_min);
+    o.min_cfl = fminf(o.min_cfl, q.min_cfl);
+}
+
+#define INC_CELLS_LOG2 10
+#define INC_CELLS (1 << INC_CELLS_LOG2)
+SPH_HD uint32_t inc_cell_first(const uint32_t* local, const uint32_t* bpre, uint32_t c) { return local[c] + bpre[c >> INC_CELLS_LOG2]; }
+SPH_HD uint32_t inc_count_blocks(uint32_t ncells) { return (ncells + (uint32_t)INC_CELLS - 1u) >> INC_CELLS_LOG2; }
diff --git a/adaptive_sph_amd/csrc/sph_context.hpp b/adaptive_sph_amd/csrc/sph_context.hpp
--- a/adaptive_sph_amd/csrc/sph_context.hpp
+++ b/adaptive_sph_amd/csrc/sph_context.hpp
@@ -67,6 +67,7 @@
     int tile = 0;
     int ahead_build = 1;
     int inc_sort = 1;
+    int boundary_fused = 1;
     int slab_paced = 1;
     int slab_records = 1;
     int debug_sync = 0;
@@ -195,6 +196,7 @@
     DevBuf akey[2], aval[2], acxy, acell_start, pm2;
     DevBuf atile_raw, atile_h;
     DevBuf inc_head, inc_next, inc_bsum, inc_movers;
+    DevBuf inc_local;
     uint32_t inc_epoch = 0;
     int inc_radix_streak = 0;
     struct Ahead {
diff --git a/adaptive_sph_amd/csrc/sph_internal.hpp b/adaptive_sph_amd/csrc/sph_internal.hpp
--- a/adaptive_sph_amd/csrc/sph_internal.hpp
+++ b/adaptive_sph_amd/csrc/sph_internal.hpp
@@ -64,10 +64,7 @@
     }
 };
 
-struct HeaderOut {
-    float min_x, min_y, max_x, max_y, h_max, h_min, min_cfl;
-    uint32_t pad;
-};
+#include "sph_boundary_fused.hpp"
 
 struct SolverCtrl {
     uint32_t done;
@@ -84,6 +81,58 @@
     uint32_t error;
     uint32_t info;
 };
+
+struct HeaderAheadP {
+    const HeaderOut* partials;
+    uint32_t nparts;
+    const SolverCtrl* ctrl;
+    HeaderOut* out;
+    const DeviceStatus* status;
+    SolverCtrl* h_ctrl;
+    DeviceStatus* h_status;
+    uint32_t seq;
+};
+__device__ __forceinline__ void header_ahead_block(const HeaderAheadP& a)
+{
+    if (a.ctrl->done == 0u) {
+        if (a.h_ctrl && threadIdx.x == 0) {
+            SolverCtrl v = *a.ctrl;
+            v.seq = a.seq - 1u;
+            *a.h_ctrl = v;
+            *a.h_status = *a.status;
+            __threadfence_system();
+            ((volatile SolverCtrl*)a.h_ctrl)->seq = a.seq;
+        }
+        return;
+    }
+    HeaderOut o = header_neutral();
+    for (uint32_t k0 = threadIdx.x; k0 < a.nparts; k0 += 4u * HDR_AHEAD_THREADS) {
+        HeaderOut q[4];
+#pragma unroll
+        for (uint32_t u = 0; u < 4u; u++) q[u] = a.partials[header_ahead_slot(k0, u, a.nparts)];
+#pragma unroll
+        for (uint32_t u = 0; u < 4u; u++) header_merge(o, q[u]);
+    }
+    o.min_x = wave_min(o.min_x); o.min_y = wave_min(o.min_y); o.max_x = wave_max(o.max_x); o.max_y = wave_max(o.max_y);
+    o.h_max = wave_max(o.h_max); o.h_min = wave_min(o.h_min); o.min_cfl = wave_min(o.min_cfl);
+    __shared__ HeaderOut s_hdr[HDR_AHEAD_THREADS / 64u];
+    const uint32_t lane = threadIdx.x & 63u, w = threadIdx.x >> 6;
+    if (lane == 0) s_hdr[w] = o;
+    __syncthreads();
+    if (threadIdx.x == 0) {
+        HeaderOut r = s_hdr[0];
+        for (uint32_t k = 1; k < HDR_AHEAD_THREADS / 64u; k++) header_merge(r, s_hdr[k]);
+        *a.out = r;
+        if (a.h_ctrl) {
+            SolverCtrl v = *a.ctrl;
+            v.seq = a.seq - 1u;
+            *a.h_ctrl = v;
+            *a.h_status = *a.status;
+            __threadfence_system();
+            ((volatile SolverCtrl*)a.h_ctrl)->seq = a.seq;
+        }
+    }
+}
 
 struct CellKeyGen {
     const float4* pm;
@@ -113,9 +162,13 @@
     uint8_t* szc_out;
 };
 size_t incremental_sort_block_sums(uint32_t ncells);
+struct IncFusedP {
+    uint32_t* local;
+    HeaderAheadP hdr;
+};
 void incremental_cell_sort_reorder(hipStream_t s, Profiler* prof, uint32_t n, const float4* pm_new, const IncClassifyP& q, bool classified,
                                    const uint32_t* cell_start_cur, uint32_t* key_out, uint32_t* cell_start_out, const ReorderIO& io, uint32_t* bsum, uint32_t* movers,
-                                   uint32_t* movers_host);
+                                   uint32_t* movers_host, const IncFusedP* fused = nullptr);
 
 void incremental_cell_sort_perm(hipStream_t s, Profiler* prof, uint32_t n, uint32_t n_prev, const CellKeyGen& kg, const IncClassifyP& q, const uint32_t* cell_start_cur,
                                 uint32_t* key_out, uint32_t* perm_out, uint32_t* cell_start_out, uint32_t* bsum, uint32_t* movers, uint32_t* movers_host);
@@ -266,6 +319,7 @@
 void launch_classify(hipStream_t s, Profiler* prof, uint32_t n, const float4* pm, const float* level, uint8_t* size_class, const uint8_t* owned,
                      const uint32_t* orig, DeviceStatus* status, const sph_params* p);
 void launch_header_ahead(sph_ctx* c, uint32_t nblocks, HeaderOut* out_dev, bool publish = false);
+HeaderAheadP header_ahead_args(sph_ctx* c, uint32_t nblocks, HeaderOut* out_dev, bool publish);
 void launch_iisph2_scale(hipStream_t s, Profiler* prof, const SweepArgs& a);
 void launch_check_aii(hipStream_t s, Profiler* prof, const SweepArgs& a);
 void launch_vel_add_pacc(hipStream_t s, Profiler* prof, const SweepArgs& a);
diff --git a/adaptive_sph_amd/csrc/sph_sort.hip b/adaptive_sph_amd/csrc/sph_sort.hip
--- a/adaptive_sph_amd/csrc/sph_sort.hip
+++ b/adaptive_sph_amd/csrc/sph_sort.hip
@@ -253,13 +253,17 @@
     inc_register(q, i, k, i >= n_prev || k != inc_key_of_cur_cell(q.cur, q.nxt, q.cxy_cur[i]));
 }
 
-#define INC_CELLS 1024
+template <bool FUSED>
 __global__ __launch_bounds__(INC_CELLS) void k_inc_count(IncGrid G, const uint32_t* __restrict__ cell_start_cur, const uint8_t* __restrict__ mv,
                                                           const uint32_t* __restrict__ next, const unsigned long long* __restrict__ head, uint32_t epoch,
-                                                          uint32_t* __restrict__ count , uint32_t* __restrict__ bsum,
-                                                          uint32_t* __restrict__ movers)
+                                                          uint32_t* __restrict__ count ,
+                                                          uint32_t* __restrict__ bsum, uint32_t* __restrict__ movers, HeaderAheadP hdr)
 {
     __shared__ uint32_t ws[INC_CELLS / 64], wm[INC_CELLS / 64];
+    if (FUSED && blockIdx.x + 1u == gridDim.x) {
+        header_ahead_block(hdr);
+        return;
+    }
     const uint32_t c = blockIdx.x * (uint32_t)INC_CELLS + threadIdx.x;
     uint32_t cnt = 0, listed = 0;
     if (c < G.nxt.ncells) {
@@ -270,18 +274,33 @@
         if ((uint32_t)(h >> 32) == epoch)
             for (uint32_t m = (uint32_t)h; m; m = next[m - 1u]) listed++;
         cnt += listed;
-        count[c] = cnt;
-    }
+        if (!FUSED) count[c] = cnt;
+    }
+    const uint32_t lane = threadIdx.x & 63u, w = threadIdx.x >> 6;
     uint32_t x = cnt, y = listed;
-    for (int o = 32; o > 0; o >>= 1) {
-        x += (uint32_t)__shfl_xor((int)x, o, 64);
-        y += (uint32_t)__shfl_xor((int)y, o, 64);
-    }
-    if ((threadIdx.x & 63) == 0) {
-        ws[threadIdx.x >> 6] = x;
-        wm[threadIdx.x >> 6] = y;
-    }
-    __syncthreads();
+    if (FUSED) {
+#pragma unroll
+        for (int o = 1; o < 64; o <<= 1) {
+            const uint32_t u = __shfl_up(x, o, 64);
+            if (lane >= (uint32_t)o) x += u;
+        }
+        for (int o = 32; o > 0; o >>= 1) y += (uint32_t)__shfl_xor((int)y, o, 64);
+    } else {
+        for (int o = 32; o > 0; o >>= 1) {
+            x += (uint32_t)__shfl_xor((int)x, o, 64);
+            y += (uint32_t)__shfl_xor((int)y, o, 64);
+        }
+    }
+    if (lane == 63u) {
+        ws[w] = x;
+        wm[w] = y;
+    }
+    __syncthreads();
+    if (FUSED && c < G.nxt.ncells) {
+        uint32_t base = 0;
+        for (uint32_t k = 0; k < w; k++) base += ws[k];
+        count[c] = base + x - cnt;
+    }
     if (threadIdx.x == 0) {
         uint32_t t = 0, m = 0;
         for (int k = 0; k < INC_CELLS / 64; k++) {
@@ -332,14 +351,43 @@
     }
 }
 
-template <bool PERM>
+template <bool PERM, bool FUSED>
 __global__ __launch_bounds__(256) void k_inc_place_reorder(uint32_t n, IncGrid G, const uint32_t* __restrict__ cell_start_cur, const uint32_t* __restrict__ cell_start_nxt,
                                                             const uint32_t* __restrict__ nk, const uint8_t* __restrict__ mv, const uint32_t* __restrict__ next,
                                                             const unsigned long long* __restrict__ head, uint32_t epoch, const uint32_t* __restrict__ cxy_cur,
-                                                            uint32_t* __restrict__ key_out, ReorderIO io, uint32_t* __restrict__ perm_out)
-{
-    const uint32_t i = blockIdx.x * 256 + threadIdx.x;
-    if (i >= n) return;
+                                                            uint32_t* __restrict__ key_out, ReorderIO io, uint32_t* __restrict__ perm_out,
+                                                            const uint32_t* __restrict__ bsum, uint32_t* __restrict__ cell_start_fin, uint32_t* __restrict__ movers,
+                                                            uint32_t* __restrict__ movers_host)
+{
+    __shared__ uint32_t s_w[4];
+    const uint32_t fin_blocks = FUSED ? inc_count_blocks(G.nxt.ncells) : 0u;
+    const uint32_t tid = threadIdx.x, lane = tid & 63u, w = tid >> 6;
+    if (FUSED && blockIdx.x < fin_blocks) {
+        const uint32_t ncells = G.nxt.ncells, blk = blockIdx.x, c0 = blk * (uint32_t)INC_CELLS + 4u * tid;
+        uint32_t pre = 0;
+        for (uint32_t k = tid; k < blk; k += 256u) pre += bsum[k];
+        for (int o = 32; o > 0; o >>= 1) pre += (uint32_t)__shfl_xor((int)pre, o, 64);
+        if (lane == 0) s_w[w] = pre;
+        __syncthreads();
+        pre = s_w[0] + s_w[1] + s_w[2] + s_w[3];
+        if (c0 + 3u < ncells) {
+            const uint4 l = *(const uint4*)(cell_start_nxt + c0);
+            *(uint4*)(cell_start_fin + c0) = make_uint4(l.x + pre, l.y + pre, l.z + pre, l.w + pre);
+        } else
+            for (uint32_t c = c0; c < ncells; c++) cell_start_fin[c] = cell_start_nxt[c] + pre;
+        if (tid == 0) {
+            if (blk + 1u == fin_blocks) cell_start_fin[ncells] = pre + bsum[blk];
+            if (blk == 0) {
+                *movers_host = *movers;
+                *movers = 0u;
+            }
+        }
+        return;
+    }
+    const uint32_t i_raw = (blockIdx.x - fin_blocks) * 256 + tid;
+    if (!FUSED && i_raw >= n) return;
+    const bool past = FUSED && i_raw >= n;
+    const uint32_t i = past ? n - 1u : i_raw;
     const uint32_t flag = mv[i];
     if (PERM && flag == 2u) return;
     const uint32_t c = nk[i];
@@ -357,7 +405,34 @@
         lvlold = io.lvlold_in[i];
     }
     const unsigned long long h = head[c];
-    const uint32_t first = cell_start_nxt[c];
+    uint32_t first = cell_start_nxt[c];
+    if (FUSED) {
+        const uint32_t cb = c >> INC_CELLS_LOG2;
+        uint32_t carry = 0, mine = 0;
+        for (uint32_t k0 = 0; k0 < fin_blocks; k0 += 256u) {
+            const uint32_t k = k0 + 4u * lane;
+            uint4 v = make_uint4(0u, 0u, 0u, 0u);
+            if (k + 3u < fin_blocks) v = *(const uint4*)(bsum + k);
+            else {
+                if (k < fin_blocks) v.x = bsum[k];
+                if (k + 1u < fin_blocks) v.y = bsum[k + 1u];
+                if (k + 2u < fin_blocks) v.z = bsum[k + 2u];
+            }
+            const uint32_t own4 = v.x + v.y + v.z + v.w;
+            uint32_t z = own4;
+#pragma unroll
+            for (int o = 1; o < 64; o <<= 1) {
+                const uint32_t u = __shfl_up(z, o, 64);
+                if (lane >= (uint32_t)o) z += u;
+            }
+            const uint32_t excl = carry + z - own4;
+            const uint32_t e = cb - k0, src = (e >> 2) & 63u, sub = e & 3u;
+            const uint32_t ex = __shfl(excl, (int)src, 64), x0 = __shfl(v.x, (int)src, 64), x1 = __shfl(v.y, (int)src, 64), x2 = __shfl(v.z, (int)src, 64);
+            if (e < 256u) mine = ex + (sub > 0u ? x0 : 0u) + (sub > 1u ? x1 : 0u) + (sub > 2u ? x2 : 0u);
+            carry += __shfl(z, 63, 64);
+        }
+        first += mine;
+    }
     uint32_t b, e, r = 0;
     if (!mover) {
         const uint32_t k = (own & 0xffffu) + (own >> 16) * (uint32_t)G.cur.sx;
@@ -372,6 +447,7 @@
     if ((uint32_t)(h >> 32) == epoch)
         for (uint32_t m = (uint32_t)h; m; m = next[m - 1u]) r += (m - 1u < i) ? 1u : 0u;
     const uint32_t dst = first + r;
+    if (past) return;
     key_out[dst] = c;
     if (PERM) {
         perm_out[dst] = i;
@@ -389,21 +465,35 @@
     io.cxy_out[dst] = (c - cy * (uint32_t)G.nxt.sx) | (cy << 16);
 }
 
-size_t incremental_sort_block_sums(uint32_t ncells) { return ((size_t)ncells + INC_CELLS - 1) / INC_CELLS; }
+size_t incremental_sort_block_sums(uint32_t ncells) { return inc_count_blocks(ncells); }
 
 void incremental_cell_sort_reorder(hipStream_t s, Profiler* prof, uint32_t n, const float4* pm_new, const IncClassifyP& q, bool classified,
                                    const uint32_t* cell_start_cur, uint32_t* key_out, uint32_t* cell_start_out, const ReorderIO& io, uint32_t* bsum, uint32_t* movers,
-                                   uint32_t* movers_host)
+                                   uint32_t* movers_host, const IncFusedP* fused)
 {
     const IncGrid G{q.cur, q.nxt};
     const uint32_t ncells = q.nxt.ncells, cblocks = (uint32_t)incremental_sort_block_sums(ncells);
+    if (fused && classified) {
+        {
+            ProfScope ps(prof, "inc_count", s);
+            hipLaunchKernelGGL(k_inc_count<true>, dim3(cblocks + 1u), dim3(INC_CELLS), 0, s, G, cell_start_cur, q.mv, q.next, q.head, q.epoch, fused->local, bsum, movers,
+                               fused->hdr);
+        }
+        {
+            ProfScope ps(prof, "inc_reorder", s);
+            hipLaunchKernelGGL((k_inc_place_reorder<false, true>), dim3((n + 255) / 256 + cblocks), dim3(256), 0, s, n, G, cell_start_cur, (const uint32_t*)fused->local,
+                               q.nk, q.mv, q.next, q.head, q.epoch, q.cxy_cur, key_out, io, (uint32_t*)nullptr, (const uint32_t*)bsum, cell_start_out, movers, movers_host);
+        }
+        return;
+    }
     if (!classified) {
         ProfScope ps(prof, "inc_classify", s);
         hipLaunchKernelGGL(k_inc_classify, dim3((n + 255) / 256), dim3(256), 0, s, n, pm_new, q);
     }
     {
         ProfScope ps(prof, "inc_count", s);
-        hipLaunchKernelGGL(k_inc_count, dim3(cblocks), dim3(INC_CELLS), 0, s, G, cell_start_cur, q.mv, q.next, q.head, q.epoch, cell_start_out, bsum, movers);
+        hipLaunchKernelGGL(k_inc_count<false>, dim3(cblocks), dim3(INC_CELLS), 0, s, G, cell_start_cur, q.mv, q.next, q.head, q.epoch, cell_start_out, bsum, movers,
+                           HeaderAheadP{});
     }
     {
         ProfScope ps(prof, "inc_scan", s);
@@ -411,8 +501,8 @@
     }
     {
         ProfScope ps(prof, "inc_reorder", s);
-        hipLaunchKernelGGL(k_inc_place_reorder<false>, dim3((n + 255) / 256), dim3(256), 0, s, n, G, cell_start_cur, cell_start_out, q.nk, q.mv, q.next, q.head,
-                           q.epoch, q.cxy_cur, key_out, io, (uint32_t*)nullptr);
+        hipLaunchKernelGGL((k_inc_place_reorder<false, false>), dim3((n + 255) / 256), dim3(256), 0, s, n, G, cell_start_cur, cell_start_out, q.nk, q.mv, q.next, q.head,
+                           q.epoch, q.cxy_cur, key_out, io, (uint32_t*)nullptr, (const uint32_t*)nullptr, (uint32_t*)nullptr, (uint32_t*)nullptr, (uint32_t*)nullptr);
     }
 }
 
@@ -427,7 +517,8 @@
     }
     {
         ProfScope ps(prof, "inc_count", s);
-        hipLaunchKernelGGL(k_inc_count, dim3(cblocks), dim3(INC_CELLS), 0, s, G, cell_start_cur, q.mv, q.next, q.head, q.epoch, cell_start_out, bsum, movers);
+        hipLaunchKernelGGL(k_inc_count<false>, dim3(cblocks), dim3(INC_CELLS), 0, s, G, cell_start_cur, q.mv, q.next, q.head, q.epoch, cell_start_out, bsum, movers,
+                           HeaderAheadP{});
     }
     {
         ProfScope ps(prof, "inc_scan", s);
@@ -435,8 +526,8 @@
     }
     {
         ProfScope ps(prof, "inc_place", s);
-        hipLaunchKernelGGL(k_inc_place_reorder<true>, dim3((n + 255) / 256), dim3(256), 0, s, n, G, cell_start_cur, cell_start_out, q.nk, q.mv, q.next, q.head, q.epoch,
-                           q.cxy_cur, key_out, ReorderIO{}, perm_out);
+        hipLaunchKernelGGL((k_inc_place_reorder<true, false>), dim3((n + 255) / 256), dim3(256), 0, s, n, G, cell_start_cur, cell_start_out, q.nk, q.mv, q.next, q.head,
+                           q.epoch, q.cxy_cur, key_out, ReorderIO{}, perm_out, (const uint32_t*)nullptr, (uint32_t*)nullptr, (uint32_t*)nullptr, (uint32_t*)nullptr);
     }
 }
 
diff --git a/adaptive_sph_amd/csrc/sph_step.hip b/adaptive_sph_amd/csrc/sph_step.hip
--- a/adaptive_sph_amd/csrc/sph_step.hip
+++ b/adaptive_sph_amd/csrc/sph_step.hip
@@ -307,6 +307,7 @@
     bool density_solver;
     int tot_slot = 0;
     uint32_t k = 1, upto = 2;
+    bool header_in_build = false;
     void extend() { upto = k + std::max(1u, k / 4u); }
 };
 static int solve_sweep_a(Group& G, std::vector<Member>& M, const SolveQ& q, uint32_t k)
@@ -411,7 +412,8 @@
         launch_solver_tail(m.c->stream, &m.c->prof, m.a, q.tail, m.c->pm[m.c->pcur ^ 1].as<float4>(), -1, q.residual_density,
                            q.max_avg_error, q.max_iters, hand_host, gate_out);
         if (q.tail == 1  && source_term_on_records(m.a)) m.a.xv_ok = true;
-        if (q.tail >= 2  && m.a.hdr_partials) launch_header_ahead(m.c, (m.n + 255u) / 256u, m.c->hdr_host_dev, publish_next && !multi);
+        if (q.tail >= 2  && m.a.hdr_partials && !q.header_in_build)
+            launch_header_ahead(m.c, (m.n + 255u) / 256u, m.c->hdr_host_dev, publish_next && !multi);
     }
     return SPH_OK;
 }
@@ -499,11 +501,13 @@
 
 static int pressure_iterations(Group& G, std::vector<Member>& M, float max_avg_error, int residual_density, uint32_t max_iters,
                                uint32_t predicted_iters, int tail, bool density_solver, bool final_solve,
-                               const std::function<int()>* behind_tail = nullptr )
+                               const std::function<int()>* behind_tail = nullptr ,
+                               bool header_in_build = false )
 {
     int rc;
     const int multi = G.multi() ? 1 : 0;
     SolveQ q{max_avg_error, residual_density, max_iters, tail, density_solver};
+    q.header_in_build = header_in_build && behind_tail != nullptr;
     if ((multi || M[0].n > 0) && M[0].c->paced_step) {
         sph_ctx* c0 = M[0].c;
         const uint32_t head = density_solver ? pace_prediction(c0, M[0].n, c0->last_dens_iters, c0->prev_dens_iters) : pace_prediction(c0, M[0].n, c0->last_div_iters, c0->prev_div_iters);
@@ -551,7 +555,7 @@
     launch_cell_start(c->stream, &c->prof, v.key[0].as<uint32_t>(), n, kg.g.ncells, v.cell_start->as<uint32_t>(), c->cs_scratch.p, n > 0);
 }
 
-static int ensure_inc_sort_scratch(sph_ctx* c, uint32_t ncells)
+static int ensure_inc_sort_scratch(sph_ctx* c, uint32_t ncells, bool fused = false)
 {
     const size_t head_before = c->inc_head.bytes;
     HIPCHK(c, c->inc_head.ensure((size_t)ncells * 8));
@@ -561,6 +565,9 @@
     if (!c->inc_movers.p) {
         HIPCHK(c, c->inc_movers.ensure(4));
         HIPCHK(c, hipMemsetAsync(c->inc_movers.p, 0, 4, c->stream));
+    }
+    if (fused) {
+        HIPCHK(c, c->inc_local.ensure(((size_t)ncells + 1) * 4));
     }
     if (++c->inc_epoch == 0u) c->inc_epoch = 1u;
     return SPH_OK;
@@ -1242,7 +1249,7 @@
     enum { T_NONE = 0, T_VEL = 1, T_VX = 2, T_HYBRID = 3 };
     g_trace.mark(3);
     struct AheadPlan {
-        bool on = false, incremental = false;
+        bool on = false, incremental = false, fused = false;
         GridP g{};
         int tile_ts = 0, tile_tsx = 0, tile_tsy = 0;
         IncClassifyP q{};
@@ -1278,7 +1285,8 @@
         if (!(c->opt.inc_sort && c->grid_valid && c->fgrid.cs == cs && c->fgrid.ncells > 0 && inc_sort_fits(g.ncells, n) &&
               inc_sort_worthwhile(c->inc_count_valid, *c->movers_host, inc_sort_mover_limit(n, c->opt.inc_sort), c->inc_radix_streak)))
             return SPH_OK;
-        if ((rc = ensure_inc_sort_scratch(c, g.ncells))) return rc;
+        plan.fused = c->opt.boundary_fused != 0 && !level_on && M[0].a.hdr_partials != nullptr;
+        if ((rc = ensure_inc_sort_scratch(c, g.ncells, plan.fused))) return rc;
         plan.incremental = true;
         plan.q = IncClassifyP{c->fgrid, g, c->cxy.as<uint32_t>(), c->akey[1].as<uint32_t>(), c->aval[1].as<uint8_t>(), c->inc_next.as<uint32_t>(),
                               c->inc_head.as<unsigned long long>(), c->inc_epoch};
@@ -1296,9 +1304,13 @@
         hipStream_t s = c->stream;
         const float4* integrated = c->pm[c->pcur ^ 1].as<float4>();
         if (plan.incremental) {
+            IncFusedP fused{};
+            if (plan.fused) {
+                fused = IncFusedP{c->inc_local.as<uint32_t>(), header_ahead_args(c, (n + 255u) / 256u, c->hdr_host_dev, true)};
+            }
             incremental_cell_sort_reorder(s, &c->prof, n, integrated, plan.q,  true, c->cell_start.as<uint32_t>(), c->akey[0].as<uint32_t>(),
                                           c->acell_start.as<uint32_t>(), reorder_io(c, integrated, c->pm2.as<float4>(), c->acxy.as<uint32_t>(), false),
-                                          c->inc_bsum.as<uint32_t>(), c->inc_movers.as<uint32_t>(), (uint32_t*)(c->ctrl_host_dev + 2) + 1);
+                                          c->inc_bsum.as<uint32_t>(), c->inc_movers.as<uint32_t>(), (uint32_t*)(c->ctrl_host_dev + 2) + 1, plan.fused ? &fused : nullptr);
             c->inc_count_valid = true;
         } else {
             const CellKeyGen kg{integrated, g, nullptr, 0u, (uint32_t)SC_GONE_FROM, 1};
@@ -1326,7 +1338,7 @@
         rec(4);
         begin_solve(1, 1);
         if ((rc = plan_ahead_build())) return rc;
-        if ((rc = pressure_iterations(G, M, p->iisph_max_avg_density_error, 1, p->max_iters, c0->last_dens_iters, T_VX, true, !level_on, &queue_ahead_build))) return rc;
+        if ((rc = pressure_iterations(G, M, p->iisph_max_avg_density_error, 1, p->max_iters, c0->last_dens_iters, T_VX, true, !level_on, &queue_ahead_build, plan.fused))) return rc;
         rec(5);
         break;
     case SPH_SOLVER_IISPH2:
@@ -1355,7 +1367,7 @@
         rec(2);
         begin_solve(0, 0);
         if ((rc = plan_ahead_build())) return rc;
-        if ((rc = pressure_iterations(G, M, p->hybrid_dfsph_max_avg_divergence_error, 0, p->max_iters, c0->last_div_iters, T_VX, false, !level_on, &queue_ahead_build))) return rc;
+        if ((rc = pressure_iterations(G, M, p->hybrid_dfsph_max_avg_divergence_error, 0, p->max_iters, c0->last_div_iters, T_VX, false, !level_on, &queue_ahead_build, plan.fused))) return rc;
         rec(3);
         break;
     default: {
@@ -1377,6 +1389,7 @@
             rec(4);
             begin_solve(p->hybrid_dfsph_density_source_term == SPH_ONLY_DENSITY ? 2 : 1, 1);
             if ((rc = plan_ahead_build())) return rc;
+            qs.header_in_build = plan.fused;
             if ((rc = solve_paced(G, M, qs, pace_prediction(c0, M[0].n, c0->last_dens_iters, c0->prev_dens_iters)))) return rc;
             if ((rc = solve_queue(G, M, qs, false, true))) return rc;
             if ((rc = queue_ahead_build())) return rc;
```

New measurement: 2.477 billion particle-steps/s (median of 6 runs). 1.02x the previous value.
